# zubair-irshad/HunyuanWorld-Mirror

Hardware: AMD Instinct MI355X
Metric: views/sec (higher is better)
Workload: dtype bf16; 1 GPU; 8-view 518x518 bf16, no priors, camera+depth+pointmap+normal heads, 8 views/GPU, full 1.23B-param arch; views_per_gpu=8, global_views=8, parallelism=view-shard x1, collective=none (1 GPU)

## Files before the change

hunyuanworld-mirror_amd/_lib.py:

```python
from __future__ import annotations

import ctypes as C
import os

import torch

_HERE = os.path.dirname(os.path.abspath(__file__))
LIB_PATH = os.environ.get("WM_HIP_LIB") or os.path.join(_HERE, "libwm_hip.so")

WM_DT = {"bf16": 0, "f16": 1, "fp16": 1, "float16": 1, "bfloat16": 0}
EPI_F32, EPI_T16, EPI_GELU_T16, EPI_RESID = 0, 1, 2, 3


class wm_config(C.Structure):
    _fields_ = [
        ("img_size", C.c_int32), ("patch_size", C.c_int32), ("embed_dim", C.c_int32), ("gs_dim", C.c_int32),
        ("enable_cond", C.c_int32), ("enable_cam", C.c_int32), ("enable_pts", C.c_int32), ("enable_depth", C.c_int32),
        ("enable_norm", C.c_int32), ("enable_gs", C.c_int32),
        ("depth", C.c_int32), ("num_heads", C.c_int32), ("mlp_ratio", C.c_int32), ("num_register_tokens", C.c_int32),
        ("intermediate_idxs", C.c_int32 * 4),
        ("rope_freq", C.c_float),
        ("dino_depth", C.c_int32), ("dino_heads", C.c_int32),
        ("cam_trunk_depth", C.c_int32), ("cam_heads", C.c_int32), ("cam_steps", C.c_int32),
        ("dpt_features", C.c_int32),
        ("dpt_out_channels", C.c_int32 * 4),
        ("backbone_dtype", C.c_int32), ("head_dtype", C.c_int32),
    ]


_FP = C.c_void_p


class wm_outputs(C.Structure):
    _fields_ = [(n, _FP) for n in (
        "camera_params", "camera_poses", "camera_intrs", "depth", "depth_conf", "pts3d", "pts3d_conf",
        "normals", "normals_conf", "gs_depth", "gs_depth_conf", "splat_means", "splat_quats", "splat_scales",
        "splat_opacities", "splat_sh", "splat_weights")] + [("taps", _FP * 4)]


EXPORTS = [
    "wm_create", "wm_destroy", "wm_last_error", "wm_set_weight", "wm_finalize_weights", "wm_host_resample_pos",
    "wm_workspace_bytes", "wm_reserve", "wm_set_workspace", "wm_missing_name", "wm_share_weights", "wm_forward", "wm_forward_sharded", "wm_rccl_unique_id", "wm_comm_init_rccl",
    "wm_local_group_create", "wm_local_group_destroy", "wm_comm_init_local", "wm_allgather", "wm_profile_enable", "wm_profile_read",
    "wm_op_gemm", "wm_op_gemm_resid_ln", "wm_op_gemm_qkv", "wm_op_attention", "wm_op_layernorm", "wm_op_qkv_post", "wm_op_conv", "wm_op_bilinear",
    "wm_op_linear_f32", "wm_host_to_16", "wm_set_tuning", "wm_op_attention_split", "wm_op_attention_ex", "wm_op_attention_flag_count", "wm_op_gs_splat", "wm_op_conv3x3_up", "wm_depth_to_world", "wm_confidence_mask", "wm_confidence_mask_workspace_bytes", "wm_preprocess_image", "wm_preprocess_image_size",
    "wm_preprocess_image_workspace_bytes", "wm_rasterize_splats", "wm_rasterize_workspace_bytes", "wm_prune_gs", "wm_prune_gs_workspace_bytes", "wm_op_up_conv_n32", "wm_op_conv3x3_gemm16", "wm_op_conv_ex", "wm_op_upconv3x3_tap", "wm_op_tconv", "wm_op_upconv_gather",
    "wm_depth_edge", "wm_normals_edge", "wm_point_filter_mask_workspace_bytes", "wm_point_filter_mask",
    "wm_op_im2col", "wm_op_im2col7", "wm_op_dino_tokens", "wm_op_vgt_special", "wm_op_gemm_rowmap", "wm_op_gemm_convt", "wm_op_layernorm_rows",
    "wm_op_bilinear_add", "wm_op_bilinear16", "wm_op_copy2d", "wm_op_small_attention", "wm_op_adaln", "wm_op_cam_update", "wm_op_cam_matrices",
    "wm_op_linear_f32_ex",
]

_lib = None


def lib() -> C.CDLL:
    global _lib
    if _lib is not None:
        return _lib
    if not os.path.exists(LIB_PATH):
        raise RuntimeError(
            f"{LIB_PATH} not found: build it with `python -c 'import __graft_entry__ as g; g.build()'` "
            "(hipcc --offload-arch=gfx950). There is no CPU fallback for the product path.")
    L = C.CDLL(LIB_PATH, mode=C.RTLD_GLOBAL)
    vp, i32, f32 = C.c_void_p, C.c_int, C.c_float
    L.wm_create.argtypes = [C.POINTER(wm_config), i32, C.POINTER(vp)]
    L.wm_destroy.argtypes = [vp]
    L.wm_destroy.restype = None
    L.wm_last_error.argtypes = [vp]
    L.wm_last_error.restype = C.c_char_p
    L.wm_set_weight.argtypes = [vp, C.c_char_p, vp, C.POINTER(C.c_int64), i32]
    L.wm_finalize_weights.argtypes = [vp, C.POINTER(i32)]
    L.wm_host_resample_pos.argtypes = [vp, i32, i32, i32, i32, vp]
    L.wm_host_resample_pos.restype = None
    L.wm_workspace_bytes.argtypes = [vp, i32, i32, i32, i32]
    L.wm_workspace_bytes.restype = C.c_size_t
    L.wm_reserve.argtypes = [vp, i32, i32, i32, i32]
    L.wm_set_workspace.argtypes = [vp, vp, C.c_size_t]
    L.wm_share_weights.argtypes = [vp, vp]
    L.wm_missing_name.argtypes = [vp, i32]
    L.wm_missing_name.restype = C.c_char_p
    L.wm_forward.argtypes = [vp, vp, i32, i32, i32, vp, vp, vp, C.POINTER(C.c_int32), C.POINTER(wm_outputs), vp]
    L.wm_forward_sharded.argtypes = [vp, vp, i32, i32, i32, i32, i32, vp, vp, vp, C.POINTER(C.c_int32),
                                     C.POINTER(wm_outputs), vp]
    L.wm_rccl_unique_id.argtypes = [vp]
    L.wm_comm_init_rccl.argtypes = [vp, vp, i32, i32]
    L.wm_local_group_create.argtypes = [i32]
    L.wm_local_group_create.restype = vp
    L.wm_local_group_destroy.argtypes = [vp]
    L.wm_local_group_destroy.restype = None
    L.wm_comm_init_local.argtypes = [vp, vp, i32]
    L.wm_allgather.argtypes = [vp, vp, vp, C.c_size_t, vp]
    L.wm_profile_enable.argtypes = [vp, i32]
    L.wm_profile_read.argtypes = [vp, i32, C.POINTER(C.c_double), C.POINTER(C.c_int64)]
    L.wm_op_gemm.argtypes = [i32, i32, vp, vp, vp, vp, vp, i32, i32, i32, vp]
    L.wm_op_gemm_resid_ln.argtypes = [i32, vp, vp, vp, vp, vp, vp, vp, f32, vp, vp, vp, i32, i32, i32, C.POINTER(i32), vp]
    L.wm_op_gemm_qkv.argtypes = [i32, vp, vp, vp, vp, vp, vp, vp, vp, vp, vp, vp, vp, i32, i32, i32, i32, i32, i32, f32, vp]
    L.wm_op_attention.argtypes = [i32, vp, vp, vp, vp, i32, i32, i32, i32, i32, vp]
    L.wm_op_attention_split.argtypes = [i32, vp, vp, vp, vp, i32, i32, i32, i32, i32, i32, vp, vp, vp]
    L.wm_op_attention_ex.argtypes = [i32, vp, vp, vp, vp, i32, i32, i32, i32, i32, i32, vp, vp, vp, vp]
    L.wm_op_attention_flag_count.argtypes = [i32, i32, i32]
    L.wm_op_attention_flag_count.restype = C.c_size_t
    L.wm_op_layernorm.argtypes = [vp, vp, vp, vp, i32, i32, f32, i32, i32, vp]
    L.wm_op_qkv_post.argtypes = [i32, vp, vp, vp, vp, vp, vp, vp, vp, vp, vp, i32, i32, i32, i32, i32, f32, vp]
    L.wm_op_conv.argtypes = [i32, vp, vp, vp, vp, vp, vp, i32, i32, i32, i32, i32, i32, i32, i32, i32, i32, vp]
    L.wm_op_bilinear.argtypes = [vp, vp, i32, i32, i32, i32, i32, i32, vp]
    L.wm_op_linear_f32.argtypes = [vp, vp, vp, vp, i32, i32, i32, i32, i32, i32, vp]
    L.wm_host_to_16.argtypes = [vp, vp, C.c_size_t, i32]
    L.wm_host_to_16.restype = None
    L.wm_depth_to_world.argtypes = [vp, vp, vp, vp, vp, vp, i32, i32, i32, f32, vp]
    L.wm_depth_to_world.restype = i32
    L.wm_confidence_mask_workspace_bytes.argtypes = [C.c_size_t]
    L.wm_confidence_mask_workspace_bytes.restype = C.c_size_t
    L.wm_confidence_mask.argtypes = [vp, C.c_size_t, f32, vp, vp, C.c_size_t, vp]
    L.wm_confidence_mask.restype = i32
    L.wm_depth_edge.argtypes = [vp, vp, i32, i32, i32, i32, i32, f32, i32, f32, vp, vp]
    L.wm_depth_edge.restype = i32
    L.wm_normals_edge.argtypes = [vp, vp, i32, i32, i32, i32, C.c_double, vp, vp]
    L.wm_normals_edge.restype = i32
    L.wm_point_filter_mask_workspace_bytes.argtypes = [i32, i32, i32]
    L.wm_point_filter_mask_workspace_bytes.restype = C.c_size_t
    L.wm_point_filter_mask.argtypes = [vp, vp, vp, i32, i32, i32, i32, C.c_double, i32, C.c_double, f32, vp, vp, vp, C.c_size_t, vp]
    L.wm_point_filter_mask.restype = i32
    L.wm_op_up_conv_n32.argtypes = [i32, vp, vp, vp, vp, i32, i32, i32, i32, i32, i32, vp, vp, i32, vp, vp]
    L.wm_op_up_conv_n32.restype = i32
    L.wm_op_conv3x3_gemm16.argtypes = [i32, vp, vp, vp, vp, i32, vp, vp, i32, i32, i32, i32, i32, i32, i32, vp, vp]
    L.wm_op_conv3x3_gemm16.restype = i32
    L.wm_op_conv_ex.argtypes = [i32, vp, i32, vp, vp, vp, vp, vp, i32, i32, i32, i32, i32, i32, i32, i32, i32, vp]
    L.wm_op_conv_ex.restype = i32
    L.wm_op_upconv3x3_tap.argtypes = [i32, vp, vp, vp, vp, i32, i32, i32, i32, i32, i32, i32, vp, vp, vp]
    L.wm_op_upconv3x3_tap.restype = i32
    L.wm_op_tconv.argtypes = [i32, vp, vp, vp, vp, vp, i32, i32, i32, i32, i32, i32, vp, vp]
    L.wm_op_tconv.restype = i32
    L.wm_op_upconv_gather.argtypes = [vp, vp, vp, i32, i32, i32, i32, i32, i32, vp]
    L.wm_op_upconv_gather.restype = i32
    L.wm_prune_gs_workspace_bytes.argtypes = [C.c_size_t]
    L.wm_prune_gs_workspace_bytes.restype = C.c_size_t
    L.wm_prune_gs.argtypes = [vp, vp, vp, vp, vp, vp, i32, f32, vp, vp, vp, vp, vp, C.POINTER(i32), vp, C.c_size_t, vp]
    L.wm_prune_gs.restype = i32
    L.wm_rasterize_workspace_bytes.argtypes = [i32, i32, i32, i32, C.c_size_t]
    L.wm_rasterize_workspace_bytes.restype = C.c_size_t
    L.wm_rasterize_splats.argtypes = [vp, vp, vp, vp, vp, i32, i32, vp, vp, i32, i32, i32, vp, vp, vp, vp, vp, C.c_size_t, C.c_size_t,
                                      C.POINTER(C.c_ulonglong), vp]
    L.wm_rasterize_splats.restype = i32
    L.wm_preprocess_image_size.argtypes = [i32, i32, i32, i32, C.POINTER(i32), C.POINTER(i32)]
    L.wm_preprocess_image_size.restype = i32
    L.wm_preprocess_image_workspace_bytes.argtypes = [i32, i32, i32, i32]
    L.wm_preprocess_image_workspace_bytes.restype = C.c_size_t
    L.wm_preprocess_image.argtypes = [vp, i32, i32, i32, i32, vp, vp, C.c_size_t, vp]
    L.wm_preprocess_image.restype = i32
# ... 41 lines not shown
```

hunyuanworld-mirror_amd/csrc/gemm.hip:

```cpp
#include "wm_common.h"
#include "wm_kernels.h"

#include <cstdlib>
#include <type_traits>

int wm_tuning[WM_TUNE_COUNT] = {-1, -1, -1, -1, -1, -1, -1, -1, -1, -1, -1, -1, -1, -1, -1, -1, -1, -1, -1, -1, -1, -1, -1, -1, -1, -1, -1, -1, -1};

namespace {

#ifndef WM_GEMM_PRIO
#define WM_GEMM_PRIO 0
#endif
constexpr int PRIO = WM_GEMM_PRIO;
constexpr int BK = 64;

typedef __attribute__((address_space(3))) void* lds_vp;
typedef const __attribute__((address_space(1))) void* glb_vp;

__device__ __forceinline__ void stage_piece32(const u16* __restrict__ g, int ld, int row0, int nrows, int k0, char* lds_tile,
                                              int piece, int lane) {
  const int r = piece * 16 + (lane >> 2);
  const int c = (lane & 3) ^ ((r >> 2) & 3);
  int gr = row0 + r;
  gr = gr < nrows ? gr : nrows - 1;
  __builtin_amdgcn_global_load_lds((glb_vp)(g + (size_t)gr * ld + k0 + c * 8), (lds_vp)(lds_tile + piece * 1024), 16, 0, 0);
}
__device__ __forceinline__ s16x8 lds_frag32(const char* tile, int row, int chunk) {
  return *(const s16x8*)(tile + row * 64 + ((chunk ^ ((row >> 2) & 3)) << 4));
}

__device__ __forceinline__ void stage_piece(const u16* __restrict__ g, int ld, int row0, int nrows, int k0, char* lds_tile,
                                            int piece, int lane) {
  const int r = piece * 8 + (lane >> 3);
  const int c = (lane & 7) ^ ((r >> 1) & 7);
  int gr = row0 + r;
  gr = gr < nrows ? gr : nrows - 1;
  __builtin_amdgcn_global_load_lds((glb_vp)(g + (size_t)gr * ld + k0 + c * 8), (lds_vp)(lds_tile + piece * 1024), 16, 0, 0);
}

__device__ __forceinline__ s16x8 lds_frag(const char* tile, int row, int chunk) {
  return *(const s16x8*)(tile + row * 128 + ((chunk ^ ((row >> 1) & 7)) << 4));
}

__device__ __forceinline__ void tile_of(int lid, int ntm, int ntn, int G, int& band, int& nt) {
  if (G <= 1 || ntn <= 4) { band = lid / ntn; nt = lid - band * ntn; return; }
  const int per = G * ntn, sg = lid / per, r = lid - sg * per;
  const int here = ntm - sg * G < G ? ntm - sg * G : G;
  nt = r / here;
  band = sg * G + (r - nt * here);
}

template <int N> __device__ __forceinline__ void wait_vmcnt() { asm volatile("s_waitcnt vmcnt(%0)" ::"n"(N) : "memory"); }

template <int T, int EPI, int WM, int WN, int TM, int TN, int NSTAGE, int ILV, int KT = 64>
__global__ __launch_bounds__(WM * WN * 64) void gemm_nt_kernel(const WmGemmArgs p) {
  constexpr int BK = KT;
  constexpr int NW = WM * WN, BM = WM * TM * 32, BN = WN * TN * 32;
  constexpr int A_BYTES = BM * BK * 2, B_BYTES = BN * BK * 2, STAGE = A_BYTES + B_BYTES;
  constexpr int PA = BM * BK * 2 / 1024, PB = BN * BK * 2 / 1024;
// ... 232 lines not shown
            if (!ok[g]) continue;
            const float4 gm = *(const float4*)(p.gamma + cb + 8 * g);
            const float4 nv = make_float4(old[g].x + gm.x * v[g].x, old[g].y + gm.y * v[g].y, old[g].z + gm.z * v[g].z, old[g].w + gm.w * v[g].w);
            *(float4*)((float*)p.C + orow * p.ldc + cb + 8 * g) = nv;
            if (p.C2) *(float4*)(p.C2 + orow * p.ldc2 + cb + 8 * g) = nv;
          }
        } else if constexpr (EPI == WM_EPI_ROWMAP_ADD) {
#pragma unroll
          for (int g = 0; g < 4; ++g) {
            if (!ok[g]) continue;
            const int col = cb + 8 * g;
            float4 x = v[g];
            if (p.relu) x = make_float4(fmaxf(x.x, 0.f), fmaxf(x.y, 0.f), fmaxf(x.z, 0.f), fmaxf(x.w, 0.f));
            if (p.add) {
              const float4 ad = *(const float4*)(p.add + (size_t)q * p.N + col);
              x.x += ad.x; x.y += ad.y; x.z += ad.z; x.w += ad.w;
            }
            const size_t o = orow * p.ldc + col;
            if (p.out16) {
              uint2 u;
              u.x = (uint32_t)f2t<T>(x.x) | ((uint32_t)f2t<T>(x.y) << 16);
              u.y = (uint32_t)f2t<T>(x.z) | ((uint32_t)f2t<T>(x.w) << 16);
              *(uint2*)((u16*)p.C + o) = u;
            } else {
              float* c = (float*)p.C + o;
              if (p.accumulate) {
                const float4 od = *(const float4*)c;
                x.x += od.x; x.y += od.y; x.z += od.z; x.w += od.w;
              }
              *(float4*)c = x;
            }
          }
        }
      }
    }
  }
}

template <int T, int EPI, int WM, int WN, int TM, int TN, int NSTAGE, int ILV, int KT = 64>
hipError_t launch_cfg(const WmGemmArgs& a, hipStream_t s) {
  constexpr int BM = WM * TM * 32, BN = WN * TN * 32;
  constexpr size_t shm = (size_t)NSTAGE * (BM + BN) * KT * 2;
  const int ntn = (a.N + BN - 1) / BN, ntm = (a.M + BM - 1) / BM;
  static bool attr = false;
  if (!attr) {
    (void)hipFuncSetAttribute((const void*)gemm_nt_kernel<T, EPI, WM, WN, TM, TN, NSTAGE, ILV, KT>, hipFuncAttributeMaxDynamicSharedMemorySize, (int)shm);
    attr = true;
  }
  hipLaunchKernelGGL((gemm_nt_kernel<T, EPI, WM, WN, TM, TN, NSTAGE, ILV, KT>), dim3(ntm * ntn), dim3(WM * WN * 64), shm, s, a);
  return hipGetLastError();
}


template <int T, int EPI, int SM, int SN>
__device__ __forceinline__ void epilogue16(const WmGemmArgs& p, f32x4 (&acc)[SM][SN], int rowb, int colb, int lane, int mlim) {
  const int l15 = lane & 15, lq = lane >> 4;
  if constexpr (EPI == WM_EPI_QKV) {
    static_assert(EPI != WM_EPI_QKV || SN == 4, "QKV epilogue needs 64 columns per wave");
    const WmQkvArgs& q = p.qkv;
    const int D = q.H * 64;
    const int col0 = colb;
    const int which = col0 / D, head = (col0 - which * D) >> 6;
    if (col0 >= p.N) return;
    const float* nw = which == 0 ? q.qn_w : q.kn_w;
    const float* nb = which == 0 ? q.qn_b : q.kn_b;
    const bool do_norm = which < 2 && nw != nullptr, do_rope = which < 2 && q.rope_cos != nullptr;
    u16* dst = (u16*)(which == 0 ? q.q : which == 1 ? q.k : q.v);
    const float sc = which == 0 ? q.q_scale : 1.0f;
    float4 bs4[4], w4[4], b4[4];
#pragma unroll
    for (int j = 0; j < 4; ++j) {
      bs4[j] = p.bias ? *(const float4*)(p.bias + col0 + 16 * j + 4 * lq) : make_float4(0, 0, 0, 0);
      w4[j] = do_norm ? *(const float4*)(nw + 16 * j + 4 * lq) : make_float4(1, 1, 1, 1);
      b4[j] = do_norm ? *(const float4*)(nb + 16 * j + 4 * lq) : make_float4(0, 0, 0, 0);
    }
    auto rope_rows = [&](int i, float4 (&cs)[2], float4 (&sn)[2]) {
      const int row = rowb + i * 16 + l15;
      const int rr = row < mlim ? row : 0;
      const int t = rr - (int)(((float)rr + 0.5f) * q.inv_tpv) * q.tokens_per_view;
      int py = 0, px = 0;
      if (t >= q.patch_start) {
        const int idx = t - q.patch_start;
        py = (int)(((float)idx + 0.5f) * q.inv_gw) + 1;
        px = idx - (py - 1) * q.grid_w + 1;
      }
      cs[0] = *(const float4*)(q.rope_cos + py * 16 + 4 * lq); sn[0] = *(const float4*)(q.rope_sin + py * 16 + 4 * lq);
      cs[1] = *(const float4*)(q.rope_cos + px * 16 + 4 * lq); sn[1] = *(const float4*)(q.rope_sin + px * 16 + 4 * lq);
    };
    float4 csn[2][2], snn[2][2];
    if (do_rope) rope_rows(0, csn[0], snn[0]);
#pragma unroll
    for (int i = 0; i < SM; ++i) {
      if (rowb + i * 16 >= mlim) break;
      const int row = rowb + i * 16 + l15;
      const bool row_ok = row < mlim;
      if (do_rope && i + 1 < SM) rope_rows(i + 1, csn[(i + 1) & 1], snn[(i + 1) & 1]);
      float v[4][4];
#pragma unroll
      for (int j = 0; j < 4; ++j) {
        v[j][0] = acc[i][j][0] + bs4[j].x; v[j][1] = acc[i][j][1] + bs4[j].y; v[j][2] = acc[i][j][2] + bs4[j].z; v[j][3] = acc[i][j][3] + bs4[j].w;
      }
      if (do_norm) {
        float sm = 0.f;
#pragma unroll
        for (int j = 0; j < 4; ++j)
#pragma unroll
          for (int e = 0; e < 4; ++e) sm += v[j][e];
        sm += __shfl_xor(sm, 16);
        const float mean = xhalf_sum(sm) * (1.0f / 64.0f);
        float ss = 0.f;
#pragma unroll
        for (int j = 0; j < 4; ++j)
#pragma unroll
          for (int e = 0; e < 4; ++e) { v[j][e] -= mean; ss += v[j][e] * v[j][e]; }
        ss += __shfl_xor(ss, 16);
        const float rstd = 1.0f / sqrtf(xhalf_sum(ss) * (1.0f / 64.0f) + 1e-5f);
#pragma unroll
        for (int j = 0; j < 4; ++j) {
          v[j][0] = v[j][0] * rstd * w4[j].x + b4[j].x; v[j][1] = v[j][1] * rstd * w4[j].y + b4[j].y;
          v[j][2] = v[j][2] * rstd * w4[j].z + b4[j].z; v[j][3] = v[j][3] * rstd * w4[j].w + b4[j].w;
        }
      }
      if (do_rope) {
#pragma unroll
        for (int hh = 0; hh < 2; ++hh) {
          const float4 cs = csn[i & 1][hh], sn = snn[i & 1][hh];
          const float c4[4] = {cs.x, cs.y, cs.z, cs.w}, s4[4] = {sn.x, sn.y, sn.z, sn.w};
#pragma unroll
          for (int e = 0; e < 4; ++e) {
            const float lo = v[2 * hh][e], hi = v[2 * hh + 1][e];
            v[2 * hh][e] = lo * c4[e] - hi * s4[e];
            v[2 * hh + 1][e] = hi * c4[e] + lo * s4[e];
          }
        }
      }
      uint2 u[4];
#pragma unroll
      for (int j = 0; j < 4; ++j) {
        u[j].x = (uint32_t)f2t<T>(v[j][0] * sc) | ((uint32_t)f2t<T>(v[j][1] * sc) << 16);
        u[j].y = (uint32_t)f2t<T>(v[j][2] * sc) | ((uint32_t)f2t<T>(v[j][3] * sc) << 16);
      }
#pragma unroll
      for (int jp = 0; jp < 2; ++jp) {
        swap16(u[2 * jp].x, u[2 * jp + 1].x);
        swap16(u[2 * jp].y, u[2 * jp + 1].y);
      }
      if (row_ok) {
        u16* o = dst + ((size_t)head * q.head_stride + row) * 64 + 16 * (lq & 1) + 4 * (lq & 2);
#pragma unroll
        for (int jp = 0; jp < 2; ++jp) *(uint4*)(o + 32 * jp) = make_uint4(u[2 * jp].x, u[2 * jp].y, u[2 * jp + 1].x, u[2 * jp + 1].y);
      }
    }
    return;
  } else {
    float4 bs4[SN], gm4[SN];
#pragma unroll
    for (int j = 0; j < SN; ++j) {
      const int col = colb + j * 16 + 4 * lq;
      bs4[j] = (p.bias && col < p.N) ? *(const float4*)(p.bias + col) : make_float4(0, 0, 0, 0);
      if constexpr (EPI == WM_EPI_RESID) gm4[j] = col < p.N ? *(const float4*)(p.gamma + col) : make_float4(0, 0, 0, 0);
    }
    if constexpr ((EPI == WM_EPI_T16 || EPI == WM_EPI_GELU_T16) && SN % 2 == 0) {
      if ((p.N & 7) == 0 && (p.ldc & 7) == 0 && ((uintptr_t)p.C & 15) == 0) {
#pragma unroll
        for (int i = 0; i < SM; ++i) {
          if (rowb + i * 16 >= mlim) break;
          const int row = rowb + i * 16 + l15;
#pragma unroll
          for (int jp = 0; jp < SN / 2; ++jp) {
            uint2 u[2];
#pragma unroll
            for (int h = 0; h < 2; ++h) {
              const int j = 2 * jp + h;
              float4 x = make_float4(acc[i][j][0] + bs4[j].x, acc[i][j][1] + bs4[j].y, acc[i][j][2] + bs4[j].z, acc[i][j][3] + bs4[j].w);
              if constexpr (EPI == WM_EPI_GELU_T16) x = gelu_erf4(x);
              u[h].x = (uint32_t)f2t<T>(x.x) | ((uint32_t)f2t<T>(x.y) << 16);
              u[h].y = (uint32_t)f2t<T>(x.z) | ((uint32_t)f2t<T>(x.w) << 16);
            }
            swap16(u[0].x, u[1].x);
            swap16(u[0].y, u[1].y);
            const int col = colb + (2 * jp + (lq & 1)) * 16 + 4 * (lq & 2);
            if (row < mlim && col < p.N) *(uint4*)((u16*)p.C + (size_t)row * p.ldc + col) = make_uint4(u[0].x, u[0].y, u[1].x, u[1].y);
          }
        }
        return;
      }
    }
    if constexpr (EPI == WM_EPI_RESID) {
      float4 old[2][SN];
      auto load_old = [&](int i, float4 (&o)[SN]) {
        const int row = rowb + i * 16 + l15;
#pragma unroll
        for (int j = 0; j < SN; ++j) {
          const int col = colb + j * 16 + 4 * lq;
          o[j] = (row < mlim && col < p.N) ? *(const float4*)((const float*)p.C + (size_t)row * p.ldc + col) : make_float4(0, 0, 0, 0);
        }
      };
      load_old(0, old[0]);
#pragma unroll
      for (int i = 0; i < SM; ++i) {
        if (rowb + i * 16 >= mlim) break;
        if (i + 1 < SM) load_old(i + 1, old[(i + 1) & 1]);
        const int row = rowb + i * 16 + l15;
#pragma unroll
        for (int j = 0; j < SN; ++j) {
          const int col = colb + j * 16 + 4 * lq;
          const float4 o = old[i & 1][j], gm = gm4[j], bs = bs4[j];
          if (row < mlim && col < p.N) {
            const float4 nv = make_float4(o.x + gm.x * (acc[i][j][0] + bs.x), o.y + gm.y * (acc[i][j][1] + bs.y), o.z + gm.z * (acc[i][j][2] + bs.z), o.w + gm.w * (acc[i][j][3] + bs.w));
            *(float4*)((float*)p.C + (size_t)row * p.ldc + col) = nv;
            if (p.C2) *(float4*)(p.C2 + (size_t)row * p.ldc2 + col) = nv;
          }
        }
      }
      return;
    }
    if constexpr (EPI == WM_EPI_CONV) {
      auto out_row = [&](int row) -> size_t {
        if (p.tc_k <= 0) return (size_t)row;
        const int hw = p.cv_h * p.cv_w, n = row / hw, rem = row - n * hw, ti = rem / p.cv_w, tj = rem - ti * p.cv_w;
        const int ph = colb / 256, a = ph / p.tc_k, b = ph - a * p.tc_k;
        return ((size_t)(n * p.cv_h + ti) * p.tc_k + a) * (size_t)(p.cv_w * p.tc_k) + (size_t)(tj * p.tc_k + b);
      };
      const int cshift = p.tc_k > 0 ? (colb / 256) * 256 : 0;
      float4 rs[2][SN], r2[2][SN];
      auto load_res = [&](int i, float4 (&a)[SN], float4 (&b)[SN]) {
        const int row = rowb + i * 16 + l15;
// ... 8 lines not shown
      load_res(0, rs[0], r2[0]);
#pragma unroll
      for (int i = 0; i < SM; ++i) {
        if (rowb + i * 16 >= mlim) break;
        if (i + 1 < SM) load_res(i + 1, rs[(i + 1) & 1], r2[(i + 1) & 1]);
        const int row = rowb + i * 16 + l15;
        float4 y[SN];
#pragma unroll
        for (int j = 0; j < SN; ++j) {
          float4 a = rs[i & 1][j];
          if (p.cv_resid_relu) a = make_float4(fmaxf(a.x, 0.f), fmaxf(a.y, 0.f), fmaxf(a.z, 0.f), fmaxf(a.w, 0.f));
          const float4 b = r2[i & 1][j], bs = bs4[j];
          y[j] = make_float4(acc[i][j][0] + bs.x + a.x + b.x, acc[i][j][1] + bs.y + a.y + b.y, acc[i][j][2] + bs.z + a.z + b.z, acc[i][j][3] + bs.w + a.w + b.w);
          if (p.relu) y[j] = make_float4(fmaxf(y[j].x, 0.f), fmaxf(y[j].y, 0.f), fmaxf(y[j].z, 0.f), fmaxf(y[j].w, 0.f));
        }
        if (p.out16) {
          if constexpr (SN % 2 == 0) {
#pragma unroll
            for (int jp = 0; jp < SN / 2; ++jp) {
              uint2 u[2];
#pragma unroll
              for (int h = 0; h < 2; ++h) {
                const float4 x = y[2 * jp + h];
                u[h].x = (uint32_t)f2t<T>(x.x) | ((uint32_t)f2t<T>(x.y) << 16);
                u[h].y = (uint32_t)f2t<T>(x.z) | ((uint32_t)f2t<T>(x.w) << 16);
              }
              swap16(u[0].x, u[1].x);
              swap16(u[0].y, u[1].y);
              const int col = colb + (2 * jp + (lq & 1)) * 16 + 4 * (lq & 2);
              if (row < mlim && col < p.N) *(uint4*)((u16*)p.C + out_row(row) * p.ldc + col - cshift) = make_uint4(u[0].x, u[0].y, u[1].x, u[1].y);
            }
          }
        } else {
#pragma unroll
          for (int j = 0; j < SN; ++j) {
            const int col = colb + j * 16 + 4 * lq;
            if (row < mlim && col < p.N) *(float4*)((float*)p.C + out_row(row) * p.ldc + col - cshift) = y[j];
          }
        }
      }
      return;
    }
#pragma unroll
    for (int i = 0; i < SM; ++i) {
      if (rowb + i * 16 >= mlim) break;
      const int row = rowb + i * 16 + l15;
      if (row >= mlim) continue;
#pragma unroll
      for (int j = 0; j < SN; ++j) {
        const int col = colb + j * 16 + 4 * lq;
        if (col >= p.N) continue;
        const float4 bs = bs4[j];
        float4 x = make_float4(acc[i][j][0] + bs.x, acc[i][j][1] + bs.y, acc[i][j][2] + bs.z, acc[i][j][3] + bs.w);
        const size_t o = (size_t)row * p.ldc + col;
        if constexpr (EPI == WM_EPI_F32) {
          *(float4*)((float*)p.C + o) = x;
        } else if constexpr (EPI == WM_EPI_T16 || EPI == WM_EPI_GELU_T16) {
          if constexpr (EPI == WM_EPI_GELU_T16) x = gelu_erf4(x);
          uint2 u;
          u.x = (uint32_t)f2t<T>(x.x) | ((uint32_t)f2t<T>(x.y) << 16);
          u.y = (uint32_t)f2t<T>(x.z) | ((uint32_t)f2t<T>(x.w) << 16);
          *(uint2*)((u16*)p.C + o) = u;
        }
      }
    }
  }
}

template <int T, int EPI, int WM, int WN, int TM, int TN, int NSTAGE>
__global__ __launch_bounds__(WM * WN * 64) void gemm_nt16_kernel(const WmGemmArgs p) {
  constexpr int NW = WM * WN, BM = WM * TM * 32, BN = WN * TN * 32;
  constexpr int SM = TM * 2, SN = TN * 2;
  constexpr int A_BYTES = BM * BK * 2, B_BYTES = BN * BK * 2, STAGE = A_BYTES + B_BYTES;
  constexpr int PA = BM / 8, PB = BN / 8, PPW = (PA + PB) / NW;
  static_assert((PA + PB) % NW == 0, "pieces must divide over waves");
  extern __shared__ __attribute__((aligned(16))) char smem[];
  const int tid = threadIdx.x, lane = tid & 63, wave = __builtin_amdgcn_readfirstlane(tid >> 6);
  const int wm = wave / WN, wn = wave % WN;
  const int ntn = (p.N + BN - 1) / BN, ntm = (p.M + BM - 1) / BM;
  const int lid = xcd_remap(blockIdx.x, ntm * ntn);
  const int m0 = (lid / ntn) * BM, n0 = (lid % ntn) * BN;
  const u16* A = (const u16*)p.A;
  const u16* W = (const u16*)p.W;
  auto stage = [&](int kt, int s) {
    char* base = smem + s * STAGE;
#pragma unroll
    for (int i = 0; i < PPW; ++i) {
      const int pc = wave * PPW + i;
      if (pc < PA) stage_piece(A, p.lda, m0, p.M, kt * BK, base, pc, lane);
      else stage_piece(W, p.ldw, n0, p.N, kt * BK, base + A_BYTES, pc - PA, lane);
    }
  };
  f32x4 acc[SM][SN];
#pragma unroll
  for (int i = 0; i < SM; ++i)
#pragma unroll
    for (int j = 0; j < SN; ++j) acc[i][j] = f32x4{0.f, 0.f, 0.f, 0.f};
  const int nk = p.K / BK;
#pragma unroll
  for (int s = 0; s < NSTAGE - 1; ++s)
    if (s < nk) stage(s, s);
  const int l15 = lane & 15, lq = lane >> 4;
  for (int t = 0; t < nk; ++t) {
    const int ahead = min(nk - 1 - t, NSTAGE - 2);
    if (ahead >= 2) wait_vmcnt<2 * PPW>();
    else if (ahead == 1) wait_vmcnt<PPW>();
// ... 242 lines not shown
      if (__hip_atomic_load((wm_gi32*)(p.ln_sync + band * 2), WM_RLX_AGENT) >= 4) { ok = 1; break; }
      if (++spins > WM_LN_SPIN_LIMIT) break;
      __builtin_amdgcn_s_sleep(1);
    }
    if (!ok) __hip_atomic_store((wm_gi32*)(p.ln_fallback + band), 1, WM_RLX_AGENT);
    *lflag = ok;
  }
  __syncthreads();
  ok = *lflag;
  if (ok) {
    float4 w4[4], b4[4];
#pragma unroll
    for (int j = 0; j < 4; ++j) {
      w4[j] = *(const float4*)(p.ln_w + colb + j * 16 + 4 * lq);
      b4[j] = *(const float4*)(p.ln_b + colb + j * 16 + 4 * lq);
    }
#pragma unroll
    for (int i = 0; i < SM; ++i) {
      if (rowb + i * 16 >= mlim) break;
      const int row = rowb + i * 16 + l15;
      const int rr = row < mlim ? row : mlim - 1;
      float m[4], q[4];
#pragma unroll
      for (int k = 0; k < 4; ++k) {
        const unsigned long long bits = __hip_atomic_load((wm_gu64*)(p.ln_stats + ((size_t)rr * 4 + k) * 2), WM_RLX_AGENT);
        m[k] = __builtin_bit_cast(float, (unsigned)bits); q[k] = __builtin_bit_cast(float, (unsigned)(bits >> 32));
      }
      float mean, M2;
      ln_combine4(m, q, 256.0f, mean, M2);
      const float rstd = 1.0f / sqrtf(__fadd_rn(__fmul_rn(M2, 1.0f / 1024.0f), p.ln_eps));
      uint2 u[4];
#pragma unroll
      for (int j = 0; j < 4; ++j) {
        const float y0 = ln_norm(acc[i][j][0], mean, rstd, w4[j].x, b4[j].x), y1 = ln_norm(acc[i][j][1], mean, rstd, w4[j].y, b4[j].y);
        const float y2 = ln_norm(acc[i][j][2], mean, rstd, w4[j].z, b4[j].z), y3 = ln_norm(acc[i][j][3], mean, rstd, w4[j].w, b4[j].w);
        u[j].x = (uint32_t)f2t<T>(y0) | ((uint32_t)f2t<T>(y1) << 16);
        u[j].y = (uint32_t)f2t<T>(y2) | ((uint32_t)f2t<T>(y3) << 16);
      }
#pragma unroll
      for (int jp = 0; jp < 2; ++jp) {
        swap16(u[2 * jp].x, u[2 * jp + 1].x);
        swap16(u[2 * jp].y, u[2 * jp + 1].y);
        const int col = colb + (2 * jp + (lq & 1)) * 16 + 4 * (lq & 2);
        if (row < mlim) *(uint4*)((u16*)p.ln_out + (size_t)row * p.ln_ld + col) = make_uint4(u[2 * jp].x, u[2 * jp].y, u[2 * jp + 1].x, u[2 * jp + 1].y);
      }
    }
  }
  __syncthreads();
  if (tid == 0) {
    const int d = __hip_atomic_fetch_add((wm_gi32*)(p.ln_sync + band * 2 + 1), 1, WM_RLX_AGENT);
    if (d == 3) {
      __hip_atomic_store((wm_gi32*)(p.ln_sync + band * 2), 0, WM_RLX_AGENT);
      __hip_atomic_store((wm_gi32*)(p.ln_sync + band * 2 + 1), 0, WM_RLX_AGENT);
    }
  }
}

#ifdef WM_GEMM_STAMPS
__device__ int wm_ln_fallback_count;
#endif
template <int T>
__global__ __launch_bounds__(256) void gemm_ln_fallback_kernel(const WmGemmArgs p, int bands, int full_units) {
  const int band = blockIdx.x;
  if (__hip_atomic_load((wm_gi32*)(p.ln_fallback + band), WM_RLX_AGENT) == 0) return;
  int u0, S;
  if (p.sched_bands > 0) {
    u0 = (int)((long long)band * p.sched_units / bands);
    S = (int)((long long)(band + 1) * p.sched_units / bands) - u0;
  } else {
    u0 = band * full_units; S = full_units;
  }
  const int lane = threadIdx.x & 63, wave = threadIdx.x >> 6;
#ifdef WM_GEMM_STAMPS
  if (threadIdx.x == 0) atomicAdd(&wm_ln_fallback_count, 1);
#endif
  const int r1 = (u0 + S) * 16 < p.M ? (u0 + S) * 16 : p.M;
  for (int row = u0 * 16 + wave; row < r1; row += 4) {
    float m[4], q[4];
#pragma unroll
    for (int k = 0; k < 4; ++k) {
      const unsigned long long bits = __hip_atomic_load((wm_gu64*)(p.ln_stats + ((size_t)row * 4 + k) * 2), WM_RLX_AGENT);
      m[k] = __builtin_bit_cast(float, (unsigned)bits); q[k] = __builtin_bit_cast(float, (unsigned)(bits >> 32));
    }
    float mean, M2;
    ln_combine4(m, q, 256.0f, mean, M2);
    const float rstd = 1.0f / sqrtf(__fadd_rn(__fmul_rn(M2, 1.0f / 1024.0f), p.ln_eps));
#pragma unroll
    for (int i = 0; i < 4; ++i) {
      const int c = (i * 64 + lane) * 4;
      const float4 v = *(const float4*)((const float*)p.C + (size_t)row * p.ldc + c);
      const float4 w = *(const float4*)(p.ln_w + c), b = *(const float4*)(p.ln_b + c);
      uint2 u;
      u.x = (uint32_t)f2t<T>(ln_norm(v.x, mean, rstd, w.x, b.x)) | ((uint32_t)f2t<T>(ln_norm(v.y, mean, rstd, w.y, b.y)) << 16);
      u.y = (uint32_t)f2t<T>(ln_norm(v.z, mean, rstd, w.z, b.z)) | ((uint32_t)f2t<T>(ln_norm(v.w, mean, rstd, w.w, b.w)) << 16);
      *(uint2*)((u16*)p.ln_out + (size_t)row * p.ln_ld + c) = u;
    }
  }
  __syncthreads();
  if (threadIdx.x == 0) __hip_atomic_store((wm_gi32*)(p.ln_fallback + band), 0, WM_RLX_AGENT);
}

#ifdef WM_GEMM_STAMPS
__device__ unsigned long long wm_gemm_stamp_buf[8 * 8192];
#endif

template <int T, int EPI, int PRIO, int DBG = 0, int QI = 4, int VER = 2>
// ... 49 lines not shown
    const int lim = (isA ? p.M : p.N) - 1;
    gr = gr < lim ? gr : lim;
    gp[i] = (isA ? (const u16*)p.A + (size_t)gr * p.lda : (const u16*)p.W + (size_t)gr * p.ldw) + c * 8;
    loff[i] = (isA ? 0 : A_BYTES) + pl * 1024;
    if constexpr (CONV) {
      if (isA) {
        const int ai = i < 2 ? i : i - 4;
        const int hw = p.cv_h * p.cv_w, n = gr / hw, rem = gr - n * hw, y = rem / p.cv_w, x = rem - y * p.cv_w;
        cv_pix[ai] = gr;
        cv_fl[ai] = (y == 0 ? 1 : 0) | (y == p.cv_h - 1 ? 2 : 0) | (x == 0 ? 4 : 0) | (x == p.cv_w - 1 ? 8 : 0);
        cv_c8[ai] = c * 8;
      }
    }
  }
  auto dma = [&](int buf, int i0, int i1, bool in_loop = false) {
    if ((DBG == 6 || (DBG >= 16 && (DBG & 1))) && in_loop) return;
#pragma unroll
    for (int i = i0; i < i1; ++i) {
      if ((i == 1 || i == 7) && !two) continue;
      if constexpr (CONV) {
        if (i < 2 || i >= 6) {
          const int ai = i < 2 ? i : i - 4;
          const int tap = cv_tap[ai], cc = cv_cc[ai];
          int dy, dx;
          if (p.tc_k > 0) { const unsigned nb = tc_word >> (4 * tap); dy = (int)(nb & 3) - 1; dx = (int)((nb >> 2) & 3) - 1; }
          else { const int ty = tap / 3; dy = ty - 1; dx = tap - ty * 3 - 1; }
          const int mask = (dy < 0 ? 1 : 0) | (dy > 0 ? 2 : 0) | (dx < 0 ? 4 : 0) | (dx > 0 ? 8 : 0);
          const u16* inside = (const u16*)p.A + ((long long)(cv_pix[ai] + dy * p.cv_w + dx) * p.cv_cin + cc * 64 + cv_c8[ai]);
          const u16* src = (cv_fl[ai] & mask) ? (const u16*)p.cv_zero + cv_c8[ai] : inside;
          __builtin_amdgcn_global_load_lds((glb_vp)src, (lds_vp)(smem + buf * STAGE + loff[i]), 16, 0, 0);
          if (++cv_cc[ai] == cv_nch) { cv_cc[ai] = 0; ++cv_tap[ai]; }
          continue;
        }
      }
      __builtin_amdgcn_global_load_lds((glb_vp)gp[i], (lds_vp)(smem + buf * STAGE + loff[i]), 16, 0, 0);
      gp[i] += 64;
    }
  };
  auto wait2 = [&](auto n2c, auto n1c) {
    if (two) wait_vmcnt<decltype(n2c)::value>(); else wait_vmcnt<decltype(n1c)::value>();
  };
#define WM_W2(a_, b_) wait2(std::integral_constant<int, a_>{}, std::integral_constant<int, b_>{})
  const int sw = (l15 >> 1) & 7;
  const int foff0 = l15 * 128 + ((lq ^ sw) << 4), foff1 = l15 * 128 + (((4 + lq) ^ sw) << 4);
  const int a_base = wr * WROWS * 128, b_base = A_BYTES + wc * 64 * 128;

  f32x4 acc[SM][SN];
#pragma unroll
  for (int i = 0; i < SM; ++i)
#pragma unroll
    for (int j = 0; j < SN; ++j) acc[i][j] = f32x4{0.f, 0.f, 0.f, 0.f};
  s16x8 a[QI][2], b0[2][2], b1[2][2];

  const int nk = CONV && p.tc_k > 0 ? (int)(tc_word >> 16) * cv_nch : p.K / 64;
  dma(0, 0, 8);
  if (nk > 1) dma(1, 0, 8);
  if constexpr (VER == 3) {
    if (nk > 1) WM_W2(10, 7); else WM_W2(2, 1);
  } else {
    if (nk > 1) WM_W2(12, 9); else WM_W2(4, 3);
  }
  __builtin_amdgcn_s_barrier();
  if (VER == 2 && wr == 1) __builtin_amdgcn_s_barrier();

#ifdef WM_GEMM_STAMPS
  const unsigned long long st_loop0 = __builtin_amdgcn_s_memrealtime(), st_cyc0 = __builtin_amdgcn_s_memtime();
#endif
  if constexpr (VER == 3) {
    constexpr int NAY = QI == 4 ? 2 : 1;
    constexpr int CY = 2 * NAY + 4, C0Y = NAY + 2;
    auto lgk0 = [&]() { asm volatile("s_waitcnt lgkmcnt(0)" ::: "memory"); };
    auto bar = [&]() { __builtin_amdgcn_s_barrier(); __builtin_amdgcn_sched_barrier(0); };
    auto mfma_on = [&]() { __builtin_amdgcn_sched_barrier(0); if (PRIO) __builtin_amdgcn_s_setprio(1); };
    auto mfma_off = [&]() { if (PRIO) __builtin_amdgcn_s_setprio(0); __builtin_amdgcn_sched_barrier(0); };
    auto kloop3 = [&](auto nbc) __attribute__((always_inline)) {
      constexpr int NB = decltype(nbc)::value;
      auto rd_a = [&](int t, int q0, int n) {
        const char* tile = smem + (t & 1) * STAGE;
#pragma unroll
        for (int i = 0; i < n; ++i) {
          a[i][0] = *(const s16x8*)(tile + a_base + (q0 + i) * 2048 + foff0);
          a[i][1] = *(const s16x8*)(tile + a_base + (q0 + i) * 2048 + foff1);
        }
      };
      auto rd_b = [&](int t, int j0, s16x8 (&b)[2][2]) {
        const char* tile = smem + (t & 1) * STAGE;
#pragma unroll
        for (int j = 0; j < 2; ++j) {
          b[j][0] = *(const s16x8*)(tile + b_base + (j0 + j) * 2048 + foff0);
          b[j][1] = *(const s16x8*)(tile + b_base + (j0 + j) * 2048 + foff1);
        }
      };
      auto L0 = [&](int t) {
        rd_b(t, 0, b0); rd_a(t, 0, QI);
        if (t >= 1 && t + 1 < nk) dma((t + 1) & 1, 6, 8, true);
      };
      auto L1 = [&](int t) { rd_b(t, 2, b1); };
      auto L2 = [&](int t) {
        rd_a(t, QI, NB);
        if (t + 2 < nk) dma(t & 1, 0, 4, true);
      };
      auto L3 = [&](int t) {
        if (t + 2 < nk) dma(t & 1, 4, 6, true);
      };
      auto mm = [&](int r0, int n, int c0, s16x8 (&b)[2][2]) {
#pragma unroll
        for (int kh = 0; kh < 2; ++kh)
#pragma unroll
          for (int i = 0; i < n; ++i)
#pragma unroll
            for (int j = 0; j < 2; ++j) acc[r0 + i][c0 + j] = mfma16<T>(b[j][kh], a[i][kh], acc[r0 + i][c0 + j]);
      };
      auto M0 = [&](int) { mfma_on(); mm(0, QI, 0, b0); mfma_off(); };
      auto M1 = [&](int) { mfma_on(); mm(0, QI, 2, b1); mfma_off(); };
      auto M2 = [&](int) { mfma_on(); mm(QI, NB, 2, b1); mfma_off(); };
// ... 104 lines not shown
    else if (do_pf) wait_vmcnt<PF>(); else wait_vmcnt<0>();
    stage_end();
#pragma unroll
    for (int kh = 0; kh < 2; ++kh)
#pragma unroll
      for (int i = 0; i < QI; ++i)
#pragma unroll
        for (int j = 0; j < 2; ++j) acc[i][2 + j] = mfma16<T>(b1[j][kh], a[i][kh], acc[i][2 + j]);
    mfma_end();
    if (!NO_RD) {
#pragma unroll
    for (int i = 0; i < NB; ++i) {
      a[i][0] = *(const s16x8*)(tile + a_base + (QI + i) * 2048 + foff0);
      a[i][1] = *(const s16x8*)(tile + a_base + (QI + i) * 2048 + foff1);
    }
    }
    if (n2) dma(buf, 4, 6, true);
    stage_end();
#pragma unroll
    for (int kh = 0; kh < 2; ++kh)
#pragma unroll
      for (int i = 0; i < NB; ++i)
#pragma unroll
        for (int j = 0; j < 2; ++j) acc[QI + i][2 + j] = mfma16<T>(b1[j][kh], a[i][kh], acc[QI + i][2 + j]);
    mfma_end();
    if (n2) { dma(buf, 6, 8, true); WM_W2(12, 9); } else if (n1) { if (do_pf) WM_W2(4 + PF, 3 + PF); else WM_W2(4, 3); }
    stage_end();
#pragma unroll
    for (int kh = 0; kh < 2; ++kh)
#pragma unroll
      for (int i = 0; i < NB; ++i)
#pragma unroll
        for (int j = 0; j < 2; ++j) acc[QI + i][j] = mfma16<T>(b0[j][kh], a[i][kh], acc[QI + i][j]);
    mfma_end();
  }
  };
  if (nB == QI) kloop(std::integral_constant<int, QI>{});
  else if (nB == QI - 1) kloop(std::integral_constant<int, QI - 1>{});
  else kloop(std::integral_constant<int, QI - 2>{});
  }
#undef WM_W2
#ifdef WM_GEMM_STAMPS
  const unsigned long long st_loop1 = __builtin_amdgcn_s_memrealtime(), st_cyc1 = __builtin_amdgcn_s_memtime();
#endif
  if (VER == 2 && wr == 0) __builtin_amdgcn_s_barrier();
  if (DBG == 5 && acc[0][0][0] != 1.2345e-30f) return;
  {
    const int rowb = m0 + (wr ? 16 * S0 : 0), rend = rowb + 16 * Sw;
    if constexpr (EPI == WM_EPI_RESID && DBG == 0 && QI == 3) {
      if (p.ln_out) {
        epilogue_resid_ln<T, SM>(p, acc, smem, tid, lane, wr, wc, band, nt, rowb, n0 + wc * 64, wr ? 16 * S0 : 0, rend < p.M ? rend : p.M);
        return;
      }
    }
    epilogue16<T, EPI, SM, SN>(p, acc, rowb, n0 + wc * 64, lane, rend < p.M ? rend : p.M);
  }
#ifdef WM_GEMM_STAMPS
  asm volatile("s_waitcnt vmcnt(0)" ::: "memory");
  if (wave == 0 && blockIdx.x < 8192) {
    const unsigned long long st_exit = __builtin_amdgcn_s_memrealtime();
    const unsigned hw = __builtin_amdgcn_s_getreg((31 << 11) | 4), xcc = __builtin_amdgcn_s_getreg((31 << 11) | 20);
    if (lane == 0) {
      unsigned long long* o = wm_gemm_stamp_buf + (size_t)blockIdx.x * 8;
      o[0] = st_entry; o[1] = st_loop0; o[2] = st_loop1; o[3] = st_exit; o[4] = st_cyc1 - st_cyc0;
      o[5] = ((unsigned long long)xcc << 32) | hw; o[6] = ((unsigned long long)m0 << 32) | (unsigned)n0; o[7] = 1;
    }
  }
#endif
}

template <int T, int EPI, int DBG = 0, int QI = 4, int VER = 2>
hipError_t launch_pp2(const WmGemmArgs& a, hipStream_t s) {
  constexpr int BM = 64 * QI;
  constexpr size_t shm = (size_t)2 * (BM + 256) * 128 + (EPI == WM_EPI_RESID ? 2048 : 0);
  const int ntn = (a.N + 255) / 256, ntm = a.sched_bands > 0 ? a.sched_bands : (a.M + BM - 1) / BM;
  static bool attr = false;
  if (!attr) {
    (void)hipFuncSetAttribute((const void*)gemm_pp2_kernel<T, EPI, 1, DBG, QI, VER>, hipFuncAttributeMaxDynamicSharedMemorySize, (int)shm);
    attr = true;
  }
  hipLaunchKernelGGL((gemm_pp2_kernel<T, EPI, 1, DBG, QI, VER>), dim3(ntm * ntn), dim3(512), shm, s, a);
  return hipGetLastError();
}

template <int T, int EPI, int QI, int DBG = 0>
hipError_t launch_pp(const WmGemmArgs& a, hipStream_t s) {
  constexpr int BM = 64 * QI, BN = 256;
  constexpr size_t shm = (size_t)2 * (BM + BN) * 128;
  const int ntn = (a.N + BN - 1) / BN, ntm = (a.M + BM - 1) / BM;
  static bool attr = false;
  if (!attr) {
    (void)hipFuncSetAttribute((const void*)gemm_pp_kernel<T, EPI, QI, 1, DBG>, hipFuncAttributeMaxDynamicSharedMemorySize, (int)shm);
    attr = true;
  }
  hipLaunchKernelGGL((gemm_pp_kernel<T, EPI, QI, 1, DBG>), dim3(ntm * ntn), dim3(512), shm, s, a);
  return hipGetLastError();
}

template <int T, int EPI>
hipError_t launch_pp_E(const WmGemmArgs& a, int cfg, hipStream_t s) {
  const int ver = EPI == WM_EPI_CONV ? 2 : wm_tuning[WM_TUNE_GEMM_PP];
  if constexpr (EPI == WM_EPI_CONV) {
    return cfg == 4 ? launch_pp2<T, EPI>(a, s) : launch_pp2<T, EPI, 0, 3>(a, s);
  } else {
    if (ver == 4) return cfg == 4 ? launch_pp2<T, EPI, 0, 4, 3>(a, s) : launch_pp2<T, EPI, 0, 3, 3>(a, s);
    if (ver != 3) return cfg == 4 ? launch_pp2<T, EPI>(a, s) : launch_pp2<T, EPI, 0, 3>(a, s);
    return cfg == 5 ? launch_pp<T, EPI, 3>(a, s) : launch_pp<T, EPI, 4>(a, s);
  }
// ... 90 lines not shown
  return best;
}

void pick_sched(const WmGemmArgs& a, int ncu, int forced_cfg, int& cfg, int& bands) {
  const int U = (a.M + 15) / 16, ntn = (a.N + 255) / 256;
  const float kf = (float)a.K / 1024.0f;
  float best = 1e30f;
  int best_cfg = cfg, best_b = 0;
  for (int c = 4; c <= 5; ++c) {
    if (forced_cfg >= 0 && c != forced_cfg) continue;
    const int full = c == 4 ? 16 : 12;
    const float unit = c == 4 ? 1.43f : 1.5f;
    const int bmin = (U + full - 1) / full;
    for (int k = 0; k < 6; ++k) {
      int B;
      if (k == 0) B = bmin;
      else {
        const long r0 = ((long)bmin * ntn + ncu - 1) / ncu;
        B = (int)(((r0 + k - 1) * ncu) / ntn);
      }
      if (B < bmin) continue;
      if (B > U) B = U;
      const int smax = (U + B - 1) / B;
      if (U / B < full - 4) continue;
      const long rounds = ((long)B * ntn + ncu - 1) / ncu;
      const float loop = kf * (full * unit - 0.5f * (float)(full - smax));
      const float cost = (float)rounds * (1.6f + loop + 0.35f * (float)smax);
      if (cost < best) { best = cost; best_cfg = c; best_b = B; }
    }
  }
  cfg = best_cfg;
  bands = best_b;
}

}

static int wm_ncu() {
  static const int ncu = [] { hipDeviceProp_t pr; int d = 0; (void)hipGetDevice(&d); return hipGetDeviceProperties(&pr, d) == hipSuccess ? pr.multiProcessorCount : 256; }();
  return ncu;
}
static void plan_gemm(const WmGemmArgs& a, int& cfg, int& sched_b, bool& pp2_out);

bool wm_gemm_fuses_ln(const WmGemmArgs& a) {
  if (!a.ln_out || a.epi != WM_EPI_RESID || a.N != 1024 || !a.ln_w || !a.ln_b || !a.ln_stats || !a.ln_sync || !a.ln_fallback || !a.gamma) return false;
  if (wm_tuning[WM_TUNE_LN_FUSE] != 1 || (a.ln_ld & 7) || (a.ldc & 3)) return false;
  int cfg, sched_b; bool pp2;
  plan_gemm(a, cfg, sched_b, pp2);
  if (!pp2 || cfg != 5) return false;
  const int bm = cfg == 4 ? 256 : 192;
  const long bands = sched_b > 0 ? sched_b : (a.M + bm - 1) / bm;
  return bands * 4 <= wm_ncu();
}

hipError_t wm_launch_gemm_ln_fallback(const WmGemmArgs& a, hipStream_t s) {
  if (!wm_gemm_fuses_ln(a)) return hipSuccess;
  int cfg, sched_b; bool pp2;
  plan_gemm(a, cfg, sched_b, pp2);
  const int bm = cfg == 4 ? 256 : 192;
  const int bands = sched_b > 0 ? sched_b : (a.M + bm - 1) / bm;
  WmGemmArgs b = a;
  b.sched_bands = sched_b; b.sched_units = (a.M + 15) / 16;
  if (a.dtype == WM_T_BF16) hipLaunchKernelGGL((gemm_ln_fallback_kernel<WM_T_BF16>), dim3(bands), dim3(256), 0, s, b, bands, bm / 16);
  else hipLaunchKernelGGL((gemm_ln_fallback_kernel<WM_T_F16>), dim3(bands), dim3(256), 0, s, b, bands, bm / 16);
  return hipGetLastError();
}

static void plan_gemm(const WmGemmArgs& a, int& cfg, int& sched_b, bool& pp2_out) {
  cfg = pick_cfg(a);
  sched_b = 0;
  {
    const int ncu = wm_ncu();
    const int pp = wm_tuning[WM_TUNE_GEMM_PP];
    const bool pp2 = (cfg == 4 || cfg == 5) && (pp < 0 || pp == 1 || pp == 2 || pp == 4 || a.epi == WM_EPI_CONV) && (a.epi == WM_EPI_F32 || a.epi == WM_EPI_T16 || a.epi == WM_EPI_GELU_T16 || a.epi == WM_EPI_RESID || a.epi == WM_EPI_QKV || a.epi == WM_EPI_CONV);
    const int ts = wm_tuning[WM_TUNE_GEMM_SCHED];
    if (pp2 && ts != 0) {
      const long legacy_tiles = (long)((a.M + (cfg == 4 ? 255 : 191)) / (cfg == 4 ? 256 : 192)) * ((a.N + 255) / 256);
      if (ts > 0) sched_b = ts;
      else if (legacy_tiles <= 3L * ncu && a.M <= 16384) pick_sched(a, ncu, wm_tuning[WM_TUNE_GEMM_CFG], cfg, sched_b);
      const int U = (a.M + 15) / 16, full = cfg == 4 ? 16 : 12;
      if (sched_b > U) sched_b = U;
      if (sched_b <= 0 || (U + sched_b - 1) / sched_b > full || U / sched_b < full - 4) sched_b = 0;
    }
    pp2_out = pp2 && wm_tuning[WM_TUNE_GEMM_PP] != 0;
    static const int pp_env = [] { const char* e = wm_env("WM_GEMM_PP"); return e ? atoi(e) : 1; }();
    if (wm_tuning[WM_TUNE_GEMM_PP] < 0 && !pp_env) pp2_out = false;
    if (a.epi == WM_EPI_CONV) pp2_out = true;
  }
}

hipError_t wm_launch_gemm(const WmGemmArgs& a, hipStream_t s) {
  if (a.M <= 0 || a.N <= 0) return hipSuccess;
  if (a.K <= 0 || a.K % 64 != 0 || a.N % 4 != 0) return hipErrorInvalidValue;
  if ((a.lda & 7) || (a.ldw & 7)) return hipErrorInvalidValue;
  if (a.epi == WM_EPI_CONVT && (a.ct_cout & 3)) return hipErrorInvalidValue;
  if (a.epi != WM_EPI_CONVT && a.epi != WM_EPI_QKV && (a.ldc & 3)) return hipErrorInvalidValue;
  if (a.epi == WM_EPI_QKV && (a.N % 64 || a.N != 3 * a.qkv.H * 64)) return hipErrorInvalidValue;
  if (a.epi == WM_EPI_CONV && a.tc_k <= 0 && (a.cv_h <= 0 || a.cv_w <= 0 || a.cv_cin % 64 || a.K != 9 * a.cv_cin || a.M % (a.cv_h * a.cv_w) || !a.cv_zero || (a.N & 7))) return hipErrorInvalidValue;
  if (a.epi == WM_EPI_CONV && a.tc_k > 0 && (a.cv_h <= 0 || a.cv_w <= 0 || a.cv_cin % 64 || a.K != 4 * a.cv_cin || a.M % (a.cv_h * a.cv_w) || !a.cv_zero || a.tc_k > 4 ||
                                             a.N != a.tc_k * a.tc_k * 256 || a.ldc != 256 || a.cv_resid || a.cv_resid2))
    return hipErrorInvalidValue;
  int cfg, sched_b;
  bool is_pp2;
  plan_gemm(a, cfg, sched_b, is_pp2);
  const bool fuse_ln = wm_gemm_fuses_ln(a);
  const int gb = wm_tuning[WM_TUNE_GEMM_GROUP] >= 0 ? wm_tuning[WM_TUNE_GEMM_GROUP] : 6;
  if (a.epi == WM_EPI_QKV) {
    if (a.qkv.tokens_per_view <= 0 || a.qkv.grid_w <= 0 || a.M >= (1 << 20) || a.qkv.tokens_per_view >= (1 << 16)) return hipErrorInvalidValue;
    WmGemmArgs b = a;
    b.group_bands = gb;
    b.sched_bands = sched_b; b.sched_units = (a.M + 15) / 16;
    b.qkv.inv_tpv = 1.0f / (float)a.qkv.tokens_per_view;
    b.qkv.inv_gw = 1.0f / (float)a.qkv.grid_w;
    return b.dtype == WM_T_BF16 ? launch_T<WM_T_BF16>(b, cfg, s) : launch_T<WM_T_F16>(b, cfg, s);
  }
  WmGemmArgs c = a;
  c.group_bands = gb;
  c.sched_bands = sched_b; c.sched_units = (a.M + 15) / 16;
  c.pf_c = a.epi == WM_EPI_RESID && wm_tuning[WM_TUNE_RESID_PREFETCH] == 1 ? 1 : 0;
  if (!fuse_ln) c.ln_out = nullptr;
  return c.dtype == WM_T_BF16 ? launch_T<WM_T_BF16>(c, cfg, s) : launch_T<WM_T_F16>(c, cfg, s);
}

#ifdef WM_GEMM_STAMPS
extern "C" int wm_debug_gemm_stamps(unsigned long long* host_out, int nblocks) {
  if (nblocks > 8192) nblocks = 8192;
  return hipMemcpyFromSymbol(host_out, HIP_SYMBOL(wm_gemm_stamp_buf), (size_t)nblocks * 8 * sizeof(unsigned long long)) == hipSuccess ? 0 : 1;
}
extern "C" int wm_debug_ln_fallback_count() {
  int v = -1, z = 0;
  if (hipMemcpyFromSymbol(&v, HIP_SYMBOL(wm_ln_fallback_count), 4) != hipSuccess) return -1;
  (void)hipMemcpyToSymbol(HIP_SYMBOL(wm_ln_fallback_count), &z, 4);
  return v;
}
extern "C" int wm_debug_gemm_stamps_clear() {
  void* d = nullptr;
  if (hipGetSymbolAddress(&d, HIP_SYMBOL(wm_gemm_stamp_buf)) != hipSuccess) return 1;
  return hipMemset(d, 0, sizeof(unsigned long long) * 8 * 8192) == hipSuccess ? 0 : 1;
}
#endif
```

hunyuanworld-mirror_amd/csrc/wm_kernels.h:

```cpp
#pragma once
#include <hip/hip_runtime.h>
#include <stdint.h>
#include <stddef.h>

#include <cstdlib>
inline const char* wm_env(const char* name) {
#ifdef WM_DIAG_ENV
  return getenv(name);
#else
  (void)name;
  return nullptr;
#endif
}


enum {
  WM_EPI_F32 = 0,
  WM_EPI_T16 = 1,
  WM_EPI_GELU_T16 = 2,
  WM_EPI_RESID = 3,
  WM_EPI_ROWMAP_ADD = 4,
  WM_EPI_CONVT = 5,
  WM_EPI_QKV = 6,
  WM_EPI_CONV = 7,
};

struct WmQkvArgs {
  const float* qkv; void* q; void* k; void* v;
  const float* qn_w; const float* qn_b; const float* kn_w; const float* kn_b;
  const float* rope_cos; const float* rope_sin;
  int M, H, head_stride;
  int tokens_per_view, patch_start, grid_w;
  float inv_tpv, inv_gw;
  float q_scale; int dtype;
};

struct WmGemmArgs {
  const void* A; const void* W; void* C;
  const float* bias; const float* gamma; const float* add;
  float* C2; int ldc2;
  int M, N, K, lda, ldw, ldc;
  int dtype, epi;
  int group_bands;
  int pf_c;
  int sched_bands, sched_units;
  int rows_per_group, out_group, out_off, accumulate, out16, relu;
  int ct_k, ct_cout, ct_gh, ct_gw;
  WmQkvArgs qkv;
  int cv_h, cv_w, cv_cin;
  const void* cv_zero;
  const float* cv_resid; const float* cv_resid2;
  int cv_resid_relu;
  int tc_k;
  unsigned tc_list[16];
  void* ln_out; int ln_ld;
  const float* ln_w; const float* ln_b; float ln_eps;
  float* ln_stats;
  int* ln_sync;
  int* ln_fallback;
};
hipError_t wm_launch_gemm(const WmGemmArgs& a, hipStream_t s);
bool wm_gemm_fuses_ln(const WmGemmArgs& a);
hipError_t wm_launch_gemm_ln_fallback(const WmGemmArgs& a, hipStream_t s);

#define WM_ATTN_MAX_SPLITS_C 8
struct WmAttnArgs {
  const void* Q; const void* K; const void* V;
  void* O;
  int H;
  int q_rows;
  int seq_len;
  int q_head_stride;
  int kv_head_stride;
  int kv_chunks;
  long long kv_chunk_stride;
  int kv_rows_per_chunk;
  int dtype;
  int kv_splits, max_splits;
  int full_units;
  float* part_o; float* part_ml;
  int* unit_flags;
  const int* only_if;
  int* unit_hint;
  int* unit_stat;
  int force_partial, part_slot0;
};
hipError_t wm_launch_attention_combine(const WmAttnArgs& a, int slots, hipStream_t s);
hipError_t wm_launch_attention(const WmAttnArgs& a, hipStream_t s);
int wm_attention_variant(const WmAttnArgs& a);
void wm_attention_geometry(const WmAttnArgs& a, int* unit_rows, int* blocks_per_cu);
hipError_t wm_launch_attention_v3(const WmAttnArgs& a, int grid, int* flags, int minw, hipStream_t s);
hipError_t wm_launch_attention_v4(const WmAttnArgs& a, int grid, int* flags, hipStream_t s);
inline size_t wm_attention_max_blocks(int q_rows, int seq_len, int H) {
  const size_t nseq = (size_t)(q_rows / (seq_len > 0 ? seq_len : 1));
  return ((size_t)(seq_len + 127) / 128 + 1) * nseq * (size_t)H * WM_ATTN_MAX_SPLITS_C;
}
constexpr int WM_ATTN_MAX_SPLITS = 8;
constexpr int WM_ATTN_HINT_TTL = 15;

struct WmLnArgs {
  const float* x; void* y; const float* w; const float* b;
  int D, ld_in, ld_out; float eps;
  int groups, rows_per_group, in_group, in_off, out_group, out_off;
  int out_f32, dtype;
};
hipError_t wm_launch_layernorm(const WmLnArgs& a, hipStream_t s);

hipError_t wm_launch_qkv_post(const WmQkvArgs& a, hipStream_t s);

hipError_t wm_launch_im2col(const float* img, void* out, int N, int C, int H, int W, int ps, int Kpad,
                            int normalize, int dtype, hipStream_t s);
hipError_t wm_launch_im2col7(const float* img, void* out, int N, int H, int W, int Kpad, int dtype, hipStream_t s);
hipError_t wm_launch_gs_splat(const float* gp, const float* img, const float* depth, const float* cam, float* means, float* quats,
                              float* scales, float* opac, float* sh, float* wts, int N, int H, int W, hipStream_t s);
// ... 35 lines not shown
  const float* resid2;
  float* y;
  int N, Hi, Wi, Cin, Ho, Wo, Cout, ksize, stride, pad;
  int relu_in, resid_relu, relu_out, dtype;
  int up_hs, up_ws;
  const float* up_addx; const float* up_addy;
  int out16;
  int in16;
  int dbg;
};
bool wm_conv3x3_applicable(const WmConvArgs& a);
bool wm_conv_force_generic();
bool wm_conv3x3_out16_ok(const WmConvArgs& a);
struct WmConvN32Args {
  const uint16_t* x; const uint16_t* w; const float* bias; float* y; const uint16_t* zero;
  int N, H, W, Cin, relu_out, dtype;
  const float* tail_w; const float* tail_b; float* tail_attr; float* tail_conf; int tail_C, tail_act;
};
hipError_t wm_launch_conv3x3_n32_in16(const WmConvN32Args& a, hipStream_t s);
hipError_t wm_launch_bilinear16(const float* in, void* out16, int N, int Hi, int Wi, int Ho, int Wo, int C, const float* addx,
                                const float* addy, int dtype, hipStream_t s);
hipError_t wm_launch_conv(const WmConvArgs& a, hipStream_t s);
hipError_t wm_launch_f32_to_16_2d(const float* src, int ld_src, void* dst16, int ld_dst, int rows, int cols, int dtype, hipStream_t s);
hipError_t wm_launch_tconv_border(float* out, const float* bmiss, int N, int H, int W, int F, hipStream_t s);
hipError_t wm_launch_repack_tap_major(const void* w16, void* wt16, int Co, int C, hipStream_t s);
hipError_t wm_launch_upconv_gather(const void* y16, const float* bias, float* out, int N, int Hi, int Wi, int Ho, int Wo, int Co, hipStream_t s);

hipError_t wm_launch_linear_f32(const float* X, const float* W, const float* b, float* Y, int M, int N, int K,
                                int ldx, int ldy, int pre_act, int post_act, const float* gamma, int accumulate,
                                hipStream_t s);
hipError_t wm_launch_small_attention(const float* qkv, float* out, int S, int heads, int hd, hipStream_t s);
hipError_t wm_launch_adaln(const float* tok, const float* mod, float* h, int S, int D, float eps, hipStream_t s);
hipError_t wm_launch_cam_update(float* pred, const float* delta, float* out, int S, int first, hipStream_t s);
hipError_t wm_launch_cam_matrices(const float* params, float* poses, float* intrs, int S, int H, int W, hipStream_t s);

struct WmRasterArgs {
  const float* means; const float* quats; const float* scales; const float* opacities;
  const float* colors; int is_sh;
  int N;
  const float* viewmats; const float* Ks; int C;
  int width, height;
  float* out_rgb; float* out_depth; float* out_alpha;
  int* radii_out;
  void* workspace; size_t workspace_bytes; size_t max_isects;
};
size_t wm_raster_workspace_bytes(int N, int C, int width, int height, size_t max_isects);
hipError_t wm_launch_rasterize(const WmRasterArgs& a, hipStream_t s, unsigned long long* n_isects_out);

size_t wm_prune_workspace_bytes(size_t N);
hipError_t wm_launch_prune_gs(const float* means, const float* quats, const float* scales, const float* opac, const float* sh,
                              const float* weights, int N, float voxel, float* o_means, float* o_quats, float* o_scales, float* o_opac,
                              float* o_sh, int* K_out, void* workspace, size_t ws_bytes, hipStream_t s);

enum { WM_TUNE_GEMM_CFG = 0, WM_TUNE_GEMM_PP, WM_TUNE_GEMM_MFMA16, WM_TUNE_ATTN_QB, WM_TUNE_OP_LDPAD, WM_TUNE_ATTN_SPLITS, WM_TUNE_CONV_FUSE_UP, WM_TUNE_CONV_NARROW, WM_TUNE_CONV_BN, WM_TUNE_CONV_RS, WM_TUNE_LIN_MFMA, WM_TUNE_CONV_TPX, WM_TUNE_ATTN_TAIL, WM_TUNE_GEMM_GROUP, WM_TUNE_COMM_OVERLAP, WM_TUNE_HEADS_CONC, WM_TUNE_RCU_MID16, WM_TUNE_GEMM_SCHED, WM_TUNE_FORCE_GATHER, WM_TUNE_ATTN_OP_POLICY, WM_TUNE_COMM_P2P, WM_TUNE_LN_RPW, WM_TUNE_LN_FUSE, WM_TUNE_HEADS_MAIN, WM_TUNE_CONV_GEMM, WM_TUNE_RESID_PREFETCH, WM_TUNE_UP1_GATHER, WM_TUNE_TCONV, WM_TUNE_UP1_COMP, WM_TUNE_COUNT };
extern int wm_tuning[WM_TUNE_COUNT];
```

hunyuanworld-mirror_amd/csrc/wm_model.cpp:

```cpp
#include <hip/hip_runtime.h>
#include <rccl/rccl.h>
#include <pthread.h>

#include <algorithm>
#include <cmath>
#include <cstdio>
#include <cstdlib>
#include <cstring>
#include <map>
#include <string>
#include <unordered_map>
#include <vector>

#include "../../include/wm_hip.h"
#include "wm_kernels.h"

namespace {

inline int ru(int x, int m) { return (x + m - 1) / m * m; }

inline uint16_t h_f2bf(float f) {
  uint32_t u;
  memcpy(&u, &f, 4);
  if ((u & 0x7fffffffu) > 0x7f800000u) return (uint16_t)((u >> 16) | 0x40);
  return (uint16_t)((u + 0x7fffu + ((u >> 16) & 1u)) >> 16);
}
inline uint16_t h_f2h(float f) {
  _Float16 h = (_Float16)f;
  uint16_t r;
  memcpy(&r, &h, 2);
  return r;
}
inline uint16_t h_to16(float f, int dt) { return dt == WM_DT_BF16 ? h_f2bf(f) : h_f2h(f); }

struct Weight {
  std::vector<int64_t> shape;
  float* f32 = nullptr;
  void* w16 = nullptr;
  int k16 = 0;
  bool tap_major = false;
  std::vector<float> host;
  bool set = false;
  bool owned = true;
};

struct TconvPack {
  void* w16 = nullptr;
  float* bias_rep = nullptr;
  float* bmiss = nullptr;
  unsigned list[16] = {0};
  int k = 0, cin = 0;
};
static void free_tconv(TconvPack& t) {
  if (t.w16) (void)hipFree(t.w16);
  if (t.bias_rep) (void)hipFree(t.bias_rep);
  if (t.bmiss) (void)hipFree(t.bmiss);
  t = TconvPack();
}

static hipError_t build_tconv(int dt, int k, int Cin, int Cm, int F_, const float* wct, const float* bct, const float* wrn, TconvPack& out, hipStream_t s);
struct Up1Comp {
  void* w16 = nullptr;
  float* bias = nullptr;
  int co = 0;
};
static void free_up1comp(Up1Comp& u) {
  if (u.w16) (void)hipFree(u.w16);
  if (u.bias) (void)hipFree(u.bias);
  u = Up1Comp();
}
static hipError_t build_up1comp(int dt, int F_, int Co, const float* woc1, const float* wout, const float* bout, Up1Comp& out, hipStream_t s);

struct EvPair { hipEvent_t a, b; };

struct Comm {
  int kind = 0;
  int rank = 0, world = 1;
  ncclComm_t nccl = nullptr;
  wm_local_group* grp = nullptr;
};

}

struct wm_local_group {
  int world;
  pthread_barrier_t bar;
  std::vector<void*> recv;
};

struct wm_handle {
  wm_config cfg;
  int device = 0;
  std::string err;
  std::unordered_map<std::string, Weight> w;
  std::map<std::string, std::vector<int64_t>> spec;
  bool finalized = false;
  Comm comm;
  char* arena = nullptr;
  size_t arena_bytes = 0;
  bool arena_owned = true;
  int plan_n = -1, plan_nt = -1, plan_H = -1, plan_W = -1;
  std::map<std::string, TconvPack> tconv;
  bool tconv_valid = false;
  std::map<std::string, Up1Comp> up1comp;
  std::vector<std::string> missing;
  std::map<std::string, void*> buf;
  hipStream_t hstream[4] = {nullptr, nullptr, nullptr, nullptr};
  hipEvent_t hfork = nullptr, hjoin[4] = {nullptr, nullptr, nullptr, nullptr};
  hipStream_t cstream = nullptr;
  hipEvent_t cfork = nullptr, cjoin = nullptr;
  hipStream_t camstream = nullptr;
  hipEvent_t camjoin = nullptr;
  int* att_stat_host = nullptr;
  int att_stat_n = 0;
  std::vector<int> att_seen, att_general_ttl;
  bool prof = false;
  static constexpr int NKIND = 13;
  std::vector<EvPair> ev[NKIND];
  size_t ev_used[NKIND] = {};
};

namespace {

wm_status fail(wm_handle* h, wm_status st, const std::string& msg) {
  if (h) h->err = msg;
  return st;
}
#define HIPCHK(h, e)                                                                                   \
  do {                                                                                                 \
    hipError_t _e = (e);                                                                               \
    if (_e != hipSuccess)                                                                              \
      return fail(h, WM_ERR_HIP, std::string(hipGetErrorString(_e)) + " at " + __FILE__ + ":" + std::to_string(__LINE__)); \
  } while (0)

bool ends_with(const std::string& s, const char* suf) {
  const size_t n = strlen(suf);
  return s.size() >= n && s.compare(s.size() - n, n, suf) == 0;
}
bool starts_with(const std::string& s, const char* p) { return s.compare(0, strlen(p), p) == 0; }

enum WKind { WK_F32, WK_LIN16_BACKBONE, WK_LIN16_HEAD, WK_CONV16_HEAD, WK_CONVT16_HEAD };

WKind classify(const std::string& n, int ndim) {
  const bool vgt = starts_with(n, "visual_geometry_transformer.");
  if (vgt && ndim >= 2) {
    if (ends_with(n, "attn.qkv.weight") || ends_with(n, "attn.proj.weight") || ends_with(n, "mlp.fc1.weight") ||
        ends_with(n, "mlp.fc2.weight") || ends_with(n, "patch_embed.proj.weight") || ends_with(n, "depth_embed.proj.2.fc1.weight") ||
        ends_with(n, "depth_embed.proj.2.fc2.weight"))
      return WK_LIN16_BACKBONE;
    return WK_F32;
  }
  const bool head = starts_with(n, "pts_head.") || starts_with(n, "depth_head.") || starts_with(n, "norm_head.") || starts_with(n, "gs_head.");
  if (head && ndim == 4 && ends_with(n, ".weight")) {
    if (ends_with(n, "scratch.output_conv2.2.weight")) return WK_F32;
    if (n.find("input_merger") != std::string::npos) return WK_LIN16_HEAD;
    if (n.find("resize_layers.0.") != std::string::npos || n.find("resize_layers.1.") != std::string::npos) return WK_CONVT16_HEAD;
// ... 237 lines not shown
  if (x < 1.0) return ((a + 2.0) * x - (a + 3.0)) * x * x + 1.0;
  if (x < 2.0) return (((x - 5.0) * x + 8.0) * x - 4.0) * a;
  return 0.0;
}
void aa_weights(int in, int out, std::vector<int>& xmin, std::vector<int>& xsize, std::vector<float>& wts, int& maxk) {
  const double scale = (double)in / out;
  const double support = scale >= 1.0 ? 2.0 * scale : 2.0;
  const double invscale = scale >= 1.0 ? 1.0 / scale : 1.0;
  maxk = (int)std::ceil(support) * 2 + 1;
  xmin.resize(out); xsize.resize(out); wts.assign((size_t)out * maxk, 0.f);
  for (int i = 0; i < out; ++i) {
    const double center = scale * (i + 0.5);
    const int lo = std::max(0, (int)(center - support + 0.5));
    const int hi = std::min(in, (int)(center + support + 0.5));
    xmin[i] = lo; xsize[i] = hi - lo;
    double tot = 0;
    std::vector<double> w(hi - lo);
    for (int j = 0; j < hi - lo; ++j) { w[j] = cubic_aa((j + lo - center + 0.5) * invscale); tot += w[j]; }
    for (int j = 0; j < hi - lo; ++j) wts[(size_t)i * maxk + j] = (float)(w[j] / tot);
  }
}

}

extern "C" void wm_host_resample_pos(const float* in, int gs, int D, int gh, int gw, float* out) {
  std::vector<int> xm, xs, ym, ys;
  std::vector<float> xw, yw;
  int kx, ky;
  aa_weights(gs, gw, xm, xs, xw, kx);
  aa_weights(gs, gh, ym, ys, yw, ky);
  std::vector<float> tmp((size_t)gs * gw * D);
  for (int y = 0; y < gs; ++y)
    for (int x = 0; x < gw; ++x) {
      float* o = &tmp[((size_t)y * gw + x) * D];
      for (int c = 0; c < D; ++c) o[c] = 0.f;
      for (int j = 0; j < xs[x]; ++j) {
        const float w = xw[(size_t)x * kx + j];
        const float* s = in + ((size_t)y * gs + xm[x] + j) * D;
        for (int c = 0; c < D; ++c) o[c] += w * s[c];
      }
    }
  for (int y = 0; y < gh; ++y)
    for (int x = 0; x < gw; ++x) {
      float* o = out + ((size_t)y * gw + x) * D;
      for (int c = 0; c < D; ++c) o[c] = 0.f;
      for (int j = 0; j < ys[y]; ++j) {
        const float w = yw[(size_t)y * ky + j];
        const float* s = &tmp[((size_t)(ym[y] + j) * gw + x) * D];
        for (int c = 0; c < D; ++c) o[c] += w * s[c];
      }
    }
}

extern "C" int wm_set_tuning(const char* key, int value) {
  static const char* keys[WM_TUNE_COUNT] = {"gemm_cfg", "gemm_pp", "gemm_mfma16", "attn_qb", "op_ldpad", "attn_splits", "conv_fuse_up", "conv_narrow", "conv_bn", "conv_rs", "lin_mfma", "conv_tpx", "attn_tail", "gemm_group", "comm_overlap", "heads_concurrent", "rcu_mid16", "gemm_sched", "force_gather", "attn_op_policy", "comm_p2p", "ln_rpw", "ln_fuse", "heads_main", "conv_gemm", "resid_prefetch", "up1_gather", "tconv", "up1_comp"};
  for (int i = 0; i < WM_TUNE_COUNT; ++i)
    if (key && strcmp(key, keys[i]) == 0) { wm_tuning[i] = value; return 0; }
  return -1;
}

extern "C" void wm_host_to_16(const float* in, uint16_t* out, size_t n, int dtype) {
  for (size_t i = 0; i < n; ++i) out[i] = h_to16(in[i], dtype);
}

extern "C" wm_status wm_create(const wm_config* cfg, int device, wm_handle** out) {
  if (!cfg || !out) return WM_ERR_INVALID;
  wm_handle* h = new wm_handle();
  h->cfg = *cfg;
  h->device = device;
  *out = h;
  if (cfg->embed_dim / cfg->num_heads != 64 || cfg->embed_dim / cfg->dino_heads != 64)
    return fail(h, WM_ERR_INVALID, "backbone head_dim must be 64 (reference: 1024/16)");
  if (cfg->embed_dim % 64) return fail(h, WM_ERR_INVALID, "embed_dim must be a multiple of 64");
  if (hipSetDevice(device) != hipSuccess) return fail(h, WM_ERR_HIP, "hipSetDevice failed");
  return WM_OK;
}

extern "C" void wm_destroy(wm_handle* h) {
  if (!h) return;
  (void)hipSetDevice(h->device);
  for (auto& kv : h->tconv) free_tconv(kv.second);
  for (auto& kv : h->up1comp) free_up1comp(kv.second);
  for (auto& kv : h->w) {
    if (!kv.second.owned) continue;
    if (kv.second.f32) (void)hipFree(kv.second.f32);
    if (kv.second.w16) (void)hipFree(kv.second.w16);
  }
  if (h->arena && h->arena_owned) (void)hipFree(h->arena);
  for (int i = 0; i < 4; ++i) {
    if (h->hstream[i]) (void)hipStreamDestroy(h->hstream[i]);
    if (h->hjoin[i]) (void)hipEventDestroy(h->hjoin[i]);
  }
  if (h->att_stat_host) (void)hipHostFree(h->att_stat_host);
  if (h->hfork) (void)hipEventDestroy(h->hfork);
  if (h->camstream) (void)hipStreamDestroy(h->camstream);
  if (h->camjoin) (void)hipEventDestroy(h->camjoin);
  if (h->cstream) (void)hipStreamDestroy(h->cstream);
  if (h->cfork) (void)hipEventDestroy(h->cfork);
  if (h->cjoin) (void)hipEventDestroy(h->cjoin);
  for (int k = 0; k < wm_handle::NKIND; ++k)
    for (auto& e : h->ev[k]) { (void)hipEventDestroy(e.a); (void)hipEventDestroy(e.b); }
  if (h->comm.kind == 1 && h->comm.nccl) ncclCommDestroy(h->comm.nccl);
  delete h;
}

extern "C" const char* wm_last_error(const wm_handle* h) { return h ? h->err.c_str() : "null handle"; }

extern "C" wm_status wm_set_weight(wm_handle* h, const char* name, const float* host, const int64_t* shape, int ndim) {
  if (!h || !name || !host || !shape) return WM_ERR_INVALID;
  HIPCHK(h, hipSetDevice(h->device));
  const std::string n(name);
  auto& spec = h->spec;
  if (spec.empty())
    for (auto& kv : param_spec(h->cfg)) spec[kv.first] = kv.second;
  auto it = spec.find(n);
  if (it == spec.end()) return WM_OK;
  std::vector<int64_t> sh(shape, shape + ndim);
  if (sh != it->second) return fail(h, WM_ERR_INVALID, "shape mismatch for " + n);
  size_t numel = 1;
  for (auto s : sh) numel *= (size_t)s;
  Weight& w = h->w[n];
  h->plan_n = -1;
  h->tconv_valid = false;
  if (w.owned) {
    if (w.f32) (void)hipFree(w.f32);
    if (w.w16) (void)hipFree(w.w16);
  }
  w.f32 = nullptr; w.w16 = nullptr; w.owned = true; w.tap_major = false;
  w.shape = sh;
  w.set = true;
  const WKind k = classify(n, ndim);
  if (k == WK_F32) {
    HIPCHK(h, hipMalloc((void**)&w.f32, std::max<size_t>(numel, 4) * 4));
    HIPCHK(h, hipMemcpy(w.f32, host, numel * 4, hipMemcpyHostToDevice));
    if (ends_with(n, "pos_embed") || ends_with(n, "init_token")) w.host.assign(host, host + numel);
    if (n.find(".resize_layers.0.bias") != std::string::npos || n.find(".resize_layers.1.bias") != std::string::npos ||
        ends_with(n, ".scratch.refinenet1.out_conv.bias"))
      w.host.assign(host, host + numel);
    return WM_OK;
  }
  if (n.find(".resize_layers.0.weight") != std::string::npos || n.find(".resize_layers.1.weight") != std::string::npos ||
      ends_with(n, ".scratch.layer1_rn.weight") || ends_with(n, ".scratch.layer2_rn.weight") ||
      ends_with(n, ".scratch.refinenet1.out_conv.weight") || ends_with(n, ".scratch.output_conv1.weight"))
    w.host.assign(host, host + numel);
  const int dt = k == WK_LIN16_BACKBONE ? h->cfg.backbone_dtype : h->cfg.head_dtype;
  std::vector<uint16_t> r;
  if (k == WK_LIN16_BACKBONE || k == WK_LIN16_HEAD) {
    const int N = (int)sh[0];
    const int K = (int)(numel / N);
    const int Kp = ru(K, 64);
    r.assign((size_t)N * Kp, 0);
    for (int i = 0; i < N; ++i)
      for (int j = 0; j < K; ++j) r[(size_t)i * Kp + j] = h_to16(host[(size_t)i * K + j], dt);
    w.k16 = Kp;
  } else if (k == WK_CONV16_HEAD) {
    const int Co = (int)sh[0], Ci = (int)sh[1], kh = (int)sh[2], kw = (int)sh[3];
    r.resize(numel);
    for (int o = 0; o < Co; ++o)
      for (int c = 0; c < Ci; ++c)
        for (int y = 0; y < kh; ++y)
          for (int x = 0; x < kw; ++x)
            r[(((size_t)o * kh + y) * kw + x) * Ci + c] = h_to16(host[(((size_t)o * Ci + c) * kh + y) * kw + x], dt);
    w.k16 = kh * kw * Ci;
    if (kh == 3 && kw == 3 && ends_with(n, "output_conv1.weight")) {
      r.resize(2 * numel);
      for (int o = 0; o < Co; ++o)
        for (int t = 0; t < 9; ++t)
          for (int c = 0; c < Ci; ++c) r[numel + ((size_t)t * Co + o) * Ci + c] = r[((size_t)o * 9 + t) * Ci + c];
      w.tap_major = true;
    }
  } else {
    const int Ci = (int)sh[0], Co = (int)sh[1], kk = (int)sh[2];
    r.resize(numel);
    for (int c = 0; c < Ci; ++c)
      for (int o = 0; o < Co; ++o)
        for (int i = 0; i < kk; ++i)
          for (int j = 0; j < kk; ++j)
            r[((size_t)(i * kk + j) * Co + o) * Ci + c] = h_to16(host[(((size_t)c * Co + o) * kk + i) * kk + j], dt);
    w.k16 = Ci;
  }
  HIPCHK(h, hipMalloc(&w.w16, r.size() * 2));
  HIPCHK(h, hipMemcpy(w.w16, r.data(), r.size() * 2, hipMemcpyHostToDevice));
  return WM_OK;
}

static float init_value_of(const std::string& n) {
  const bool norm = n.find(".norm1.") != std::string::npos || n.find(".norm2.") != std::string::npos || n.find(".norm.") != std::string::npos ||
                    n.find("q_norm.") != std::string::npos || n.find("k_norm.") != std::string::npos || n.find("token_norm.") != std::string::npos ||
                    n.find("out_norm.") != std::string::npos;
  if (norm) return ends_with(n, ".weight") ? 1.0f : 0.0f;
  if (ends_with(n, ".gamma")) return n.find(".patch_embed.") != std::string::npos ? 1.0f : 0.01f;
  return 0.0f;
}

extern "C" wm_status wm_finalize_weights(wm_handle* h, int* missing) {
  if (!h) return WM_ERR_INVALID;
  HIPCHK(h, hipSetDevice(h->device));
  h->missing.clear();
  for (auto& kv : param_spec(h->cfg)) {
    auto it = h->w.find(kv.first);
    if (it != h->w.end() && it->second.set) continue;
    h->missing.push_back(kv.first);
    size_t numel = 1;
    for (auto s : kv.second) numel *= (size_t)s;
    std::vector<float> z(numel, init_value_of(kv.first));
    wm_status st = wm_set_weight(h, kv.first.c_str(), z.data(), kv.second.data(), (int)kv.second.size());
    if (st != WM_OK) return st;
    h->w[kv.first].set = false;
  }
  if (missing) *missing = (int)h->missing.size();
  h->finalized = true;
  return WM_OK;
}

extern "C" wm_status wm_share_weights(wm_handle* dst, const wm_handle* src) {
  if (!dst || !src || dst == src) return WM_ERR_INVALID;
  if (!src->finalized) return fail(dst, WM_ERR_STATE, "source weights not finalized");
  if (memcmp(&dst->cfg, &src->cfg, sizeof(wm_config)) != 0 || dst->device != src->device)
    return fail(dst, WM_ERR_INVALID, "wm_share_weights: configuration or device differs");
  for (auto& kv : dst->w) {
    if (!kv.second.owned) continue;
    if (kv.second.f32) (void)hipFree(kv.second.f32);
    if (kv.second.w16) (void)hipFree(kv.second.w16);
  }
  dst->w = src->w;
  for (auto& kv : dst->w) kv.second.owned = false;
  dst->spec = src->spec;
  dst->missing = src->missing;
  dst->finalized = true;
  dst->plan_n = -1;
  dst->tconv_valid = false;
  return WM_OK;
}

extern "C" const char* wm_missing_name(const wm_handle* h, int i) {
  return (h && i >= 0 && (size_t)i < h->missing.size()) ? h->missing[i].c_str() : nullptr;
}

extern "C" size_t wm_workspace_bytes(const wm_handle* h, int n_local, int n_total, int H, int W) {
  if (!h) return 0;
  const Dims d = make_dims(h, n_local, n_total, H, W);
  size_t tot = 0;
  for (auto& kv : arena_layout(h, d)) tot += kv.second;
  return tot;
}

namespace {

wm_status plan(wm_handle* h, const Dims& d) {
  if (h->plan_n == d.n && h->plan_nt == d.nt && h->plan_H == d.H && h->plan_W == d.W) return WM_OK;
  const wm_config& c = h->cfg;
  auto L = arena_layout(h, d);
  size_t tot = 0;
  for (auto& kv : L) tot += kv.second;
  HIPCHK(h, hipDeviceSynchronize());
  if (tot > h->arena_bytes) {
    if (!h->arena_owned)
      return fail(h, WM_ERR_STATE, "caller workspace too small: " + std::to_string(h->arena_bytes) + " < " + std::to_string(tot) + " bytes (wm_workspace_bytes)");
    if (h->arena) HIPCHK(h, hipFree(h->arena));
    h->arena = nullptr;
    h->arena_bytes = 0;
    HIPCHK(h, hipMalloc((void**)&h->arena, tot));
    h->arena_bytes = tot;
  }
  h->buf.clear();
  size_t off = 0;
  for (auto& kv : L) { h->buf[kv.first] = h->arena + off; off += kv.second; }

  {
    const int np = std::max(d.gh, d.gw) + 1;
    std::vector<float> cs((size_t)np * 16), sn((size_t)np * 16);
    for (int p = 0; p < np; ++p)
      for (int i = 0; i < 16; ++i) {
        const float expo = (float)(2 * i) / 32.0f;
        const float inv = 1.0f / std::pow(c.rope_freq, expo);
        const float ang = (float)p * inv;
        cs[(size_t)p * 16 + i] = std::cos(ang);
        sn[(size_t)p * 16 + i] = std::sin(ang);
      }
    HIPCHK(h, hipMemcpy(h->buf["rope_cos"], cs.data(), cs.size() * 4, hipMemcpyHostToDevice));
    HIPCHK(h, hipMemcpy(h->buf["rope_sin"], sn.data(), sn.size() * 4, hipMemcpyHostToDevice));
  }
  {
    const int n = (c.dino_depth + 2 * c.depth) * 3;
    if (h->att_stat_n != n) {
      if (h->att_stat_host) HIPCHK(h, hipHostFree(h->att_stat_host));
      h->att_stat_host = nullptr;
      HIPCHK(h, hipHostMalloc((void**)&h->att_stat_host, (size_t)n * 4, hipHostMallocDefault));
      h->att_stat_n = n;
    }
    memset(h->att_stat_host, 0, (size_t)n * 4);
    h->att_seen.assign(n, 0);
    h->att_general_ttl.assign(n, 0);
    HIPCHK(h, hipMemset(h->buf["ATT_STAT"], 0, (size_t)n * 4));
  }
  HIPCHK(h, hipMemset(h->buf["LN_SYNC"], 0, ((size_t)d.Mx / 16 + 2) * 3 * 4));
  HIPCHK(h, hipMemset(h->buf["ATT_HINT"], 0, (size_t)(c.dino_depth + 2 * c.depth) * 3 * wm_attention_max_blocks((int)d.Mx, d.P < d.Td ? d.P : d.Td, d.heads) * 4));
  {
    const Weight* pe = W(h, "visual_geometry_transformer.patch_embed.pos_embed");
    if (!pe || pe->host.empty()) return fail(h, WM_ERR_STATE, "pos_embed not set");
    const int g = c.img_size / c.patch_size, D = d.D;
    if (d.gh == g && d.gw == g) {
      HIPCHK(h, hipMemcpy(h->buf["dino_pos"], pe->host.data(), (size_t)(1 + d.hw) * D * 4, hipMemcpyHostToDevice));
    } else {
      std::vector<float> r((size_t)(1 + d.hw) * D);
      memcpy(r.data(), pe->host.data(), (size_t)D * 4);
      wm_host_resample_pos(pe->host.data() + D, g, D, d.gh, d.gw, r.data() + D);
      HIPCHK(h, hipMemcpy(h->buf["dino_pos"], r.data(), r.size() * 4, hipMemcpyHostToDevice));
    }
  }
  {
    const double aspect = (double)d.W / (double)d.H;
    std::vector<float> tx, ty;
    for (int i = 0; i < 4; ++i) {
      const int C = c.dpt_out_channels[i];
      uv_tables(d.gw, d.gh, C, aspect, tx, ty);
      std::vector<float> full((size_t)d.hw * C);
      for (int y = 0; y < d.gh; ++y)
        for (int x = 0; x < d.gw; ++x)
          for (int k = 0; k < C; ++k)
            full[((size_t)y * d.gw + x) * C + k] = k < C / 2 ? tx[(size_t)x * (C / 2) + k] : ty[(size_t)y * (C / 2) + k - C / 2];
      HIPCHK(h, hipMemcpy(h->buf["dpt_pos" + std::to_string(i)], full.data(), full.size() * 4, hipMemcpyHostToDevice));
    }
    uv_tables(d.W, d.H, c.dpt_features / 2, aspect, tx, ty);
    HIPCHK(h, hipMemcpy(h->buf["dpt_posx"], tx.data(), tx.size() * 4, hipMemcpyHostToDevice));
    HIPCHK(h, hipMemcpy(h->buf["dpt_posy"], ty.data(), ty.size() * 4, hipMemcpyHostToDevice));
    if (c.enable_gs) {
      uv_tables(d.W, d.H, c.gs_dim / 2, aspect, tx, ty);
      HIPCHK(h, hipMemcpy(h->buf["gs_posx"], tx.data(), tx.size() * 4, hipMemcpyHostToDevice));
      HIPCHK(h, hipMemcpy(h->buf["gs_posy"], ty.data(), ty.size() * 4, hipMemcpyHostToDevice));
    }
  }
  if (!h->tconv_valid) {
    for (auto& kv : h->tconv) free_tconv(kv.second);
  for (auto& kv : h->up1comp) free_up1comp(kv.second);
    h->tconv.clear();
    std::vector<std::string> heads;
    if (c.enable_pts) heads.push_back("pts_head.");
    if (c.enable_depth) heads.push_back("depth_head.");
    if (c.enable_norm) heads.push_back("norm_head.");
    if (c.dpt_features == 256)
      for (const std::string& p : heads)
        for (int i = 0; i < 2; ++i) {
          const Weight* wct = W(h, p + "resize_layers." + std::to_string(i) + ".weight");
          const Weight* bct = W(h, p + "resize_layers." + std::to_string(i) + ".bias");
          const Weight* wrn = W(h, p + "scratch.layer" + std::to_string(i + 1) + "_rn.weight");
          const int k = i == 0 ? 4 : 2, oc = c.dpt_out_channels[i];
          if (!wct || !bct || !wrn || wct->host.empty() || bct->host.empty() || wrn->host.empty() || oc % 64) continue;
          if (wct->host.size() != (size_t)oc * oc * k * k || bct->host.size() != (size_t)oc || wrn->host.size() != (size_t)256 * oc * 9) continue;
          HIPCHK(h, build_tconv(c.head_dtype, k, oc, oc, 256, wct->host.data(), bct->host.data(), wrn->host.data(), h->tconv[p + std::to_string(i)], nullptr));
        }
    h->up1comp.clear();
    if (c.head_dtype == WM_DT_F16)
      for (const std::string& p : heads) {
        const Weight* w1 = W(h, p + "scratch.output_conv1.weight");
        const Weight* wo = W(h, p + "scratch.refinenet1.out_conv.weight");
        const Weight* bo = W(h, p + "scratch.refinenet1.out_conv.bias");
        const int F_ = c.dpt_features;
        if (!w1 || !wo || !bo || w1->host.empty() || wo->host.empty() || bo->host.empty() || F_ % 64 || w1->shape.size() != 4) continue;
        const int Co = (int)w1->shape[0];
        if ((Co != 128 && Co != 64 && Co != 32) || w1->host.size() != (size_t)Co * F_ * 9 || wo->host.size() != (size_t)F_ * F_ || bo->host.size() != (size_t)F_) continue;
        HIPCHK(h, build_up1comp(c.head_dtype, F_, Co, w1->host.data(), wo->host.data(), bo->host.data(), h->up1comp[p], nullptr));
      }
    h->tconv_valid = true;
  }
  if (c.enable_cam) {
    const Weight* it = W(h, "cam_head.init_token");
    std::vector<float> v((size_t)d.nt * 12, 0.f);
    if (it && !it->host.empty())
      for (int i = 0; i < d.nt; ++i)
        for (int k = 0; k < 9; ++k) v[(size_t)i * 12 + k] = it->host[k];
    HIPCHK(h, hipMemcpy(h->buf["cam_init"], v.data(), v.size() * 4, hipMemcpyHostToDevice));
  }
  h->plan_n = d.n; h->plan_nt = d.nt; h->plan_H = d.H; h->plan_W = d.W;
  return WM_OK;
}

struct ProfScope {
  wm_handle* h; int kind; hipStream_t s; EvPair* e = nullptr;
  ProfScope(wm_handle* h_, int k, hipStream_t s_) : h(h_), kind(k), s(s_) {
    if (!h->prof) return;
    auto& v = h->ev[kind];
    if (h->ev_used[kind] == v.size()) {
      EvPair p;
// ... 15 lines not shown
      for (int r = 0; r < cm.world; ++r) {
        if (r == cm.rank) continue;
        if (ncclSend(send, bytes, ncclInt8, r, cm.nccl, s) != ncclSuccess) return fail(h, WM_ERR_COMM, "ncclSend failed");
        if (ncclRecv((char*)recv + (size_t)r * bytes, bytes, ncclInt8, r, cm.nccl, s) != ncclSuccess) return fail(h, WM_ERR_COMM, "ncclRecv failed");
      }
      if (ncclGroupEnd() != ncclSuccess) return fail(h, WM_ERR_COMM, "ncclGroupEnd failed");
      HIPCHK(h, hipMemcpyAsync((char*)recv + (size_t)cm.rank * bytes, send, bytes, hipMemcpyDeviceToDevice, s));
      return WM_OK;
    }
    if (ncclAllGather(send, recv, bytes, ncclInt8, cm.nccl, s) != ncclSuccess) return fail(h, WM_ERR_COMM, "ncclAllGather failed");
    return WM_OK;
  }
  if (cm.kind == 2) {
    wm_local_group* g = cm.grp;
    g->recv[cm.rank] = recv;
    HIPCHK(h, hipStreamSynchronize(s));
    pthread_barrier_wait(&g->bar);
    for (int r = 0; r < g->world; ++r)
      HIPCHK(h, hipMemcpyAsync((char*)g->recv[r] + (size_t)cm.rank * bytes, send, bytes, hipMemcpyDeviceToDevice, s));
    HIPCHK(h, hipStreamSynchronize(s));
    pthread_barrier_wait(&g->bar);
    return WM_OK;
  }
  return fail(h, WM_ERR_COMM, "sharded forward without a communicator");
}

struct Ctx {
  wm_handle* h; Dims d; hipStream_t s; int bdt, hdt;
  int attn_site = 0;
};

#define LCHK(c, e)                                                                                            \
  do {                                                                                                        \
    hipError_t _e = (e);                                                                                      \
    if (_e != hipSuccess)                                                                                     \
      return fail((c).h, WM_ERR_HIP, std::string(hipGetErrorString(_e)) + " at " + __FILE__ + ":" + std::to_string(__LINE__)); \
  } while (0)

wm_status gemm(Ctx& c, int dt, int epi, const void* A, int lda, const void* Wp, int ldw, void* C, int ldc, const float* bias,
               const float* gamma, int M, int N, int K, WmGemmArgs* extra = nullptr, int prof_kind = -1, bool* ln_fused = nullptr) {
  WmGemmArgs a;
  if (extra) a = *extra; else memset(&a, 0, sizeof(a));
  a.A = A; a.W = Wp; a.C = C; a.bias = bias; a.gamma = gamma;
  a.M = M; a.N = N; a.K = K; a.lda = lda; a.ldw = ldw; a.ldc = ldc; a.dtype = dt; a.epi = epi;
  ProfScope ps(c.h, prof_kind >= 0 ? prof_kind : epi == WM_EPI_QKV ? 5 : epi == WM_EPI_RESID ? 6 : epi == WM_EPI_GELU_T16 ? 7 : 2, c.s);
  const bool fuse = a.ln_out != nullptr && wm_gemm_fuses_ln(a);
  if (!fuse) a.ln_out = nullptr;
  if (ln_fused) *ln_fused = fuse;
  LCHK(c, wm_launch_gemm(a, c.s));
  if (fuse) LCHK(c, wm_launch_gemm_ln_fallback(a, c.s));
  return WM_OK;
}

wm_status layernorm(Ctx& c, const float* x, int ld_in, void* y, int ld_out, const float* w, const float* b, int D, float eps,
                    int groups, int rpg, int in_group, int in_off, int out_group, int out_off, int out_f32, int dt) {
  WmLnArgs a;
  a.x = x; a.y = y; a.w = w; a.b = b; a.D = D; a.ld_in = ld_in; a.ld_out = ld_out; a.eps = eps;
  a.groups = groups; a.rows_per_group = rpg; a.in_group = in_group; a.in_off = in_off; a.out_group = out_group; a.out_off = out_off;
  a.out_f32 = out_f32; a.dtype = dt;
  LCHK(c, wm_launch_layernorm(a, c.s));
  return WM_OK;
}

wm_status backbone_block(Ctx& c, const std::string& p, float* X, int M, int seq_len, int heads, float eps, bool qk_norm,
                         bool rope, int tokens_per_view, int patch_start, bool is_global, float* tap_half = nullptr,
                         bool ln1_done = false, const std::string& next_norm1 = std::string(), bool* ln1_ready = nullptr) {
  wm_handle* h = c.h;
  const Dims& d = c.d;
  const int D = d.D, dt = c.bdt;
  uint16_t* A16 = B<uint16_t>(h, "A16");
  char* QKV16 = B<char>(h, "QKV16");
  const size_t hsz = (size_t)M * D * 2;
  void* Q16 = QKV16; void* K16 = QKV16 + hsz; void* V16 = QKV16 + 2 * hsz;
  void* O16 = B<void>(h, "O16");
  void* H16 = B<void>(h, "H16");
  wm_status st;
  if (ln1_ready) *ln1_ready = false;
  if (!ln1_done) {
    st = layernorm(c, X, D, A16, D, F(h, p + "norm1.weight"), F(h, p + "norm1.bias"), D, eps, 1, M, 0, 0, 0, 0, 0, dt);
    if (st) return st;
  }
  auto fuse_args = [&](WmGemmArgs& ex, const float* w, const float* b) {
    ex.ln_out = A16; ex.ln_ld = D; ex.ln_w = w; ex.ln_b = b; ex.ln_eps = eps;
    ex.ln_stats = B<float>(h, "LN_STATS");
    int* sync = B<int>(h, "LN_SYNC");
    ex.ln_sync = sync; ex.ln_fallback = sync + ((size_t)d.Mx / 16 + 2) * 2;
  };
  {
    WmGemmArgs ex;
    memset(&ex, 0, sizeof(ex));
    WmQkvArgs& a = ex.qkv;
    a.q = Q16; a.k = K16; a.v = V16;
    if (qk_norm) {
      a.qn_w = F(h, p + "attn.q_norm.weight"); a.qn_b = F(h, p + "attn.q_norm.bias");
      a.kn_w = F(h, p + "attn.k_norm.weight"); a.kn_b = F(h, p + "attn.k_norm.bias");
    }
    if (rope) { a.rope_cos = B<float>(h, "rope_cos"); a.rope_sin = B<float>(h, "rope_sin"); }
    a.M = M; a.H = heads; a.head_stride = M; a.tokens_per_view = tokens_per_view; a.patch_start = patch_start; a.grid_w = d.gw;
    a.q_scale = 0.125f * 1.4426950408889634f; a.dtype = dt;
    st = gemm(c, dt, WM_EPI_QKV, A16, D, W16(h, p + "attn.qkv.weight"), D, nullptr, 0, F(h, p + "attn.qkv.bias"), nullptr, M, 3 * D, D, &ex);
    if (st) return st;
  }
  {
    WmAttnArgs a;
    memset(&a, 0, sizeof(a));
    a.Q = Q16; a.O = O16; a.H = heads; a.q_rows = M; a.q_head_stride = M; a.dtype = dt;
    const bool force_gather = wm_tuning[WM_TUNE_FORCE_GATHER] > 0;
    static const bool overlap_env = [] { const char* e = wm_env("WM_COMM_OVERLAP"); return e && atoi(e) != 0; }();
    a.part_o = B<float>(h, "ATT_PO"); a.part_ml = B<float>(h, "ATT_ML"); a.max_splits = WM_ATTN_MAX_SPLITS;
    a.unit_flags = B<int>(h, "ATT_FLAGS");
    const size_t hint_n = wm_attention_max_blocks((int)d.Mx, d.P < d.Td ? d.P : d.Td, d.heads);
    const int site = c.attn_site++;
    int* const hint0 = B<int>(h, "ATT_HINT") + (size_t)site * 3 * hint_n;
    int* const stat0 = B<int>(h, "ATT_STAT") + (size_t)site * 3;
    a.unit_hint = hint0; a.unit_stat = stat0;
    bool general_only = false;
    if (site * 3 < h->att_stat_n) {
      const int cur = h->att_stat_host[site * 3], delta = cur - h->att_seen[site * 3];
      h->att_seen[site * 3] = cur;
      const long units = (long)((seq_len + 511) / 512) * (M / (seq_len > 0 ? seq_len : 1)) * heads;
      if (delta > 0 && (long)delta * 4 >= units) h->att_general_ttl[site * 3] = WM_ATTN_HINT_TTL;
      if (h->att_general_ttl[site * 3] > 0) { --h->att_general_ttl[site * 3]; general_only = true; }
    }
    const bool sharded = is_global && (d.world > 1 || (force_gather && h->comm.kind != 0));
    const int ntpc = (M + 63) / 64;
    const bool overlap = wm_tuning[WM_TUNE_COMM_OVERLAP] >= 0 ? wm_tuning[WM_TUNE_COMM_OVERLAP] != 0 : overlap_env;
    bool overlap_ok = sharded && overlap && d.world > 1 && ntpc >= 16;
    if (overlap_ok) {
      WmAttnArgs t = a;
      t.force_partial = 1; t.K = K16; t.V = V16; t.seq_len = M; t.kv_head_stride = M; t.kv_chunks = 1;
      overlap_ok = wm_attention_variant(t) >= 0;
      t.kv_chunks = d.world - 1 > 1 ? d.world - 1 : 2; t.kv_rows_per_chunk = M; t.kv_chunk_stride = (long long)(2 * hsz / 2);
      overlap_ok = overlap_ok && wm_attention_variant(t) >= 0;
    }
    if (overlap_ok) {
      if (!h->cstream) {
        LCHK(c, hipStreamCreateWithFlags(&h->cstream, hipStreamNonBlocking));
        LCHK(c, hipEventCreateWithFlags(&h->cfork, hipEventDisableTiming));
        LCHK(c, hipEventCreateWithFlags(&h->cjoin, hipEventDisableTiming));
      }
      char* KVG = B<char>(h, "KVG");
      const int rank = h->comm.rank, world = d.world;
      LCHK(c, hipEventRecord(h->cfork, c.s));
      static const int ncu = [] { hipDeviceProp_t pr; int dv = 0; (void)hipGetDevice(&dv); return hipGetDeviceProperties(&pr, dv) == hipSuccess ? pr.multiProcessorCount : 256; }();
      auto pick = [&](int chunks, int smax) {
        WmAttnArgs g = a;
        g.force_partial = 1; g.seq_len = M; g.kv_head_stride = M;
        if (chunks <= 1) { g.K = K16; g.V = V16; g.kv_chunks = 1; }
        else { g.K = B<char>(h, "KVG"); g.V = g.K; g.kv_chunks = chunks; g.kv_rows_per_chunk = M; g.kv_chunk_stride = (long long)(2 * hsz / 2); }
        int unit_rows = 256, per_cu = 2;
        wm_attention_geometry(g, &unit_rows, &per_cu);
        const int ntiles = (chunks < 1 ? 1 : chunks) * ntpc;
        const long slots = (long)per_cu * ncu, units = (long)((M + unit_rows - 1) / unit_rows) * heads;
        int best = 1; long best_cost = -1;
        for (int S = 1; S <= smax && S * 8 <= ntiles; ++S) {
          const long cost = ((units * S + slots - 1) / slots) * ((ntiles + S - 1) / S) + 6L * S;
          if (best_cost < 0 || cost < best_cost) { best_cost = cost; best = S; }
        }
        return best;
      };
      const int nb = rank, nc = world - 1 - rank;
      const int sa = pick(1, 2);
      const int sb = nb > 0 ? pick(nb, nc > 0 ? 3 : 6) : 0, sc = nc > 0 ? pick(nc, WM_ATTN_MAX_SPLITS - sa - sb) : 0;
      a.force_partial = 1;
      a.K = K16; a.V = V16; a.seq_len = M; a.kv_head_stride = M; a.kv_chunks = 1; a.kv_chunk_stride = 0; a.kv_rows_per_chunk = 0;
      a.kv_splits = sa; a.part_slot0 = 0;
      {
        ProfScope ps(h, 0, c.s);
        LCHK(c, wm_launch_attention(a, c.s));
      }
      LCHK(c, hipStreamWaitEvent(h->cstream, h->cfork, 0));
      st = comm_allgather(h, K16, KVG, 2 * hsz, h->cstream);
      if (st) return st;
      LCHK(c, hipEventRecord(h->cjoin, h->cstream));
      LCHK(c, hipStreamWaitEvent(c.s, h->cjoin, 0));
      ProfScope ps(h, 0, c.s);
      a.seq_len = M; a.kv_head_stride = M; a.kv_chunk_stride = (long long)(2 * hsz / 2); a.kv_rows_per_chunk = M;
      if (nb > 0) {
        a.K = KVG; a.V = KVG + hsz; a.kv_chunks = nb; a.kv_splits = sb; a.part_slot0 = sa; a.unit_hint = hint0 + hint_n; a.unit_stat = stat0 + 1;
        LCHK(c, wm_launch_attention(a, c.s));
      }
      if (nc > 0) {
        char* base = KVG + (size_t)(rank + 1) * 2 * hsz;
        a.K = base; a.V = base + hsz; a.kv_chunks = nc; a.kv_splits = sc; a.part_slot0 = sa + sb; a.unit_hint = hint0 + 2 * hint_n; a.unit_stat = stat0 + 2;
        LCHK(c, wm_launch_attention(a, c.s));
      }
      LCHK(c, wm_launch_attention_combine(a, sa + sb + sc, c.s));
    } else {
      if (sharded) {
        char* KVG = B<char>(h, "KVG");
        st = comm_allgather(h, K16, KVG, 2 * hsz, c.s);
        if (st) return st;
        a.K = KVG; a.V = KVG + hsz; a.seq_len = M; a.kv_head_stride = M; a.kv_chunks = d.world;
        a.kv_chunk_stride = (long long)(2 * hsz / 2); a.kv_rows_per_chunk = M;
      } else {
        a.K = K16; a.V = V16; a.seq_len = seq_len; a.kv_head_stride = M; a.kv_chunks = 1; a.kv_chunk_stride = 0; a.kv_rows_per_chunk = 0;
      }
      if (general_only) { a.unit_flags = nullptr; a.unit_hint = nullptr; a.unit_stat = nullptr; }
      ProfScope ps(h, is_global ? 0 : 1, c.s);
      LCHK(c, wm_launch_attention(a, c.s));
    }
  }
  {
    WmGemmArgs ex;
    memset(&ex, 0, sizeof(ex));
    fuse_args(ex, F(h, p + "norm2.weight"), F(h, p + "norm2.bias"));
    bool fused = false;
    st = gemm(c, dt, WM_EPI_RESID, O16, D, W16(h, p + "attn.proj.weight"), D, X, D, F(h, p + "attn.proj.bias"), F(h, p + "ls1.gamma"), M, D, D, &ex, -1, &fused);
    if (st) return st;
    if (!fused) {
      st = layernorm(c, X, D, A16, D, F(h, p + "norm2.weight"), F(h, p + "norm2.bias"), D, eps, 1, M, 0, 0, 0, 0, 0, dt);
      if (st) return st;
    }
  }
  const int Hd = c.h->cfg.mlp_ratio * D;
  st = gemm(c, dt, WM_EPI_GELU_T16, A16, D, W16(h, p + "mlp.fc1.weight"), D, H16, Hd, F(h, p + "mlp.fc1.bias"), nullptr, M, Hd, D);
  if (st) return st;
  WmGemmArgs ex;
  memset(&ex, 0, sizeof(ex));
  ex.C2 = tap_half; ex.ldc2 = 2 * D;
  bool fused = false;
  if (!next_norm1.empty()) fuse_args(ex, F(h, next_norm1 + "norm1.weight"), F(h, next_norm1 + "norm1.bias"));
  st = gemm(c, dt, WM_EPI_RESID, H16, Hd, W16(h, p + "mlp.fc2.weight"), Hd, X, D, F(h, p + "mlp.fc2.bias"), F(h, p + "ls2.gamma"), M, D, Hd, &ex, -1, &fused);
  if (ln1_ready) *ln1_ready = fused;
  return st;
}

wm_status linear32(Ctx& c, const float* X, int ldx, const std::string& name, float* Y, int ldy, int M, int pre, int post,
                   const float* gamma = nullptr, int accumulate = 0) {
  const Weight* w = W(c.h, name + ".weight");
  if (!w || !w->f32) return fail(c.h, WM_ERR_STATE, "missing fp32 weight " + name);
  const int N = (int)w->shape[0];
  int K = 1;
  for (size_t i = 1; i < w->shape.size(); ++i) K *= (int)w->shape[i];
  LCHK(c, wm_launch_linear_f32(X, w->f32, F(c.h, name + ".bias"), Y, M, N, K, ldx, ldy, pre, post, gamma, accumulate, c.s));
  return WM_OK;
}

wm_status camera_head(Ctx& c, float* out_params) {
  wm_handle* h = c.h;
  const Dims& d = c.d;
  const wm_config& cf = h->cfg;
  const int D2 = 2 * d.D, S = d.nt;
  const std::string ch = "cam_head.";
  float* tok = B<float>(h, "cam_tok");
  wm_status st;
  float* tok_local = d.world > 1 ? B<float>(h, "cam_tok_local") : tok;
  st = layernorm(c, B<float>(h, "tap3"), D2, tok_local, D2, F(h, ch + "token_norm.weight"), F(h, ch + "token_norm.bias"), D2, 1e-5f,
                 d.n, 1, d.P, 0, 1, 0, 1, 0);
  if (st) return st;
  if (d.world > 1) {
    st = comm_allgather(h, tok_local, tok, (size_t)d.n * D2 * 4, c.s);
    if (st) return st;
  }
  float *e = B<float>(h, "cam_e"), *mod = B<float>(h, "cam_mod"), *hh = B<float>(h, "cam_h"), *a = B<float>(h, "cam_a");
  float *qkv = B<float>(h, "cam_qkv"), *o = B<float>(h, "cam_o"), *f = B<float>(h, "cam_f");
  float *pred = B<float>(h, "cam_pred"), *delta = B<float>(h, "cam_delta"), *init = B<float>(h, "cam_init");
  LCHK(c, hipMemsetAsync(pred, 0, (size_t)S * 12 * 4, c.s));
  LCHK(c, hipMemsetAsync(delta, 0, (size_t)S * 12 * 4, c.s));
  for (int step = 0; step < cf.cam_steps; ++step) {
    st = linear32(c, step == 0 ? init : pred, 12, ch + "param_embed", e, D2, S, 0, 0);
    if (st) return st;
    st = linear32(c, e, D2, ch + "adapt_norm_gen.1", mod, 3 * D2, S, 1, 0);
    if (st) return st;
    LCHK(c, wm_launch_adaln(tok, mod, hh, S, D2, 1e-6f, c.s));
    for (int b = 0; b < cf.cam_trunk_depth; ++b) {
      const std::string p = ch + "refine_net." + std::to_string(b) + ".";
      st = layernorm(c, hh, D2, a, D2, F(h, p + "norm1.weight"), F(h, p + "norm1.bias"), D2, 1e-5f, 1, S, 0, 0, 0, 0, 1, 0);
      if (st) return st;
      st = linear32(c, a, D2, p + "attn.qkv", qkv, 3 * D2, S, 0, 0);
      if (st) return st;
      LCHK(c, wm_launch_small_attention(qkv, o, S, cf.cam_heads, D2 / cf.cam_heads, c.s));
      st = linear32(c, o, D2, p + "attn.proj", hh, D2, S, 0, 0, F(h, p + "ls1.gamma"), 1);
      if (st) return st;
      st = layernorm(c, hh, D2, a, D2, F(h, p + "norm2.weight"), F(h, p + "norm2.bias"), D2, 1e-5f, 1, S, 0, 0, 0, 0, 1, 0);
      if (st) return st;
      st = linear32(c, a, D2, p + "mlp.fc1", f, 4 * D2, S, 0, 2);
// ... 329 lines not shown
      memset(&ex, 0, sizeof(ex));
      ex.rows_per_group = (int)npix; ex.accumulate = 1; ex.relu = 1;
      st = gemm(c, c.hdt, WM_EPI_ROWMAP_ADD, col, 192, W16(h, p + "input_merger.0.weight"), 192, fused, F_ / 2,
                F(h, p + "input_merger.0.bias"), nullptr, (int)npix, F_ / 2, 192, &ex);
      if (st) return st;
      float* X = others[0];
      float* gp = others[2];
      st = conv(c, fused, "gs_renderer.gs_head.0", false, nullptr, false, nullptr, X, n, Ho, Wo, 3, 1, 1, false);
      if (st) return st;
      st = conv(c, X, "gs_renderer.gs_head.2", true, nullptr, false, nullptr, gp, n, Ho, Wo, 1, 1, 0, true);
      if (st) return st;
      LCHK(c, wm_launch_gs_splat(gp, img_c, out_attr + voff, B<float>(h, "cam_params") + (size_t)(first_view + v0) * 9,
                                 out->splat_means + voff * 3, out->splat_quats + voff * 4, out->splat_scales + voff * 3,
                                 out->splat_opacities + voff, out->splat_sh + voff * 3, out->splat_weights + voff, n, Ho, Wo, c.s));
    }
  }
  return WM_OK;
}

wm_status forward_impl(wm_handle* h, const float* img, int n, int first_view, int nt, int H, int W_, const float* pose7,
                       const float* depth, const float* ray4, const int32_t* flags, const wm_outputs* out, hipStream_t s) {
  if (!h || !img || !out) return WM_ERR_INVALID;
  if (!h->finalized) return fail(h, WM_ERR_STATE, "weights not finalized");
  const wm_config& cf = h->cfg;
  if (n <= 0 || nt < n || nt % n) return fail(h, WM_ERR_INVALID, "n_total must be a positive multiple of n_local");
  if (H % cf.patch_size || W_ % cf.patch_size) return fail(h, WM_ERR_INVALID, "H and W must be multiples of patch_size");
  if (nt / n > 1 && (h->comm.kind == 0 || h->comm.world != nt / n)) return fail(h, WM_ERR_COMM, "communicator world size mismatch");
  HIPCHK(h, hipSetDevice(h->device));
  Ctx c{h, make_dims(h, n, nt, H, W_), s, cf.backbone_dtype, cf.head_dtype};
  const Dims& d = c.d;
  if (!(h->plan_n == d.n && h->plan_nt == d.nt && h->plan_H == d.H && h->plan_W == d.W))
    return fail(h, WM_ERR_STATE, "no workspace for this shape: call wm_reserve(h, n_local, n_total, H, W) first (and again after loading weights)");
  wm_status st = WM_OK;
  for (int k = 0; k < wm_handle::NKIND; ++k) h->ev_used[k] = 0;
  ProfScope whole(h, 4, s);
  HIPCHK(h, hipMemsetAsync(B<char>(h, "ZERO256"), 0, 256, s));
  const int D = d.D;
  const std::string v = "visual_geometry_transformer.", dn = v + "patch_embed.";
  float* Xd = B<float>(h, "Xd");
  float* Xv = B<float>(h, "Xv");
  void* A16 = B<void>(h, "A16");

  LCHK(c, wm_launch_im2col(img, A16, n, 3, H, W_, cf.patch_size, d.kpad_patch, 1, c.bdt, s));
  {
    WmGemmArgs ex;
    memset(&ex, 0, sizeof(ex));
    ex.rows_per_group = d.hw; ex.out_group = d.Td; ex.out_off = 1 + d.R; ex.add = B<float>(h, "dino_pos") + D;
    st = gemm(c, c.bdt, WM_EPI_ROWMAP_ADD, A16, d.kpad_patch, W16(h, dn + "patch_embed.proj.weight"), d.kpad_patch, Xd, D,
              F(h, dn + "patch_embed.proj.bias"), nullptr, n * d.hw, D, d.kpad_patch, &ex);
    if (st) return st;
  }
  LCHK(c, wm_launch_dino_tokens(nullptr, F(h, dn + "cls_token"), F(h, dn + "register_tokens"), B<float>(h, "dino_pos"), Xd, n, d.hw, d.R, D, s));
  {
    bool ln1 = false;
    for (int i = 0; i < cf.dino_depth; ++i) {
      const std::string nxt = i + 1 < cf.dino_depth ? dn + "blocks." + std::to_string(i + 1) + "." : std::string();
      st = backbone_block(c, dn + "blocks." + std::to_string(i) + ".", Xd, d.Md, d.Td, cf.dino_heads, 1e-6f, false, false, d.Td, 0, false, nullptr, ln1, nxt, &ln1);
      if (st) return st;
    }
  }
  st = layernorm(c, Xd, D, Xv, D, F(h, dn + "norm.weight"), F(h, dn + "norm.bias"), D, 1e-6f, n, d.hw, d.Td, 1 + d.R, d.P, d.psi, 1, 0);
  if (st) return st;

  const float* pose_tok = nullptr; const float* ray_tok = nullptr;
  if (cf.enable_cond) {
    float* pin = B<float>(h, "pr_in"); float* ph = B<float>(h, "pr_h");
    if (flags && flags[0] == 1 && pose7) {
      LCHK(c, hipMemcpy2DAsync(pin, 8 * 4, pose7, 7 * 4, 7 * 4, n, hipMemcpyDeviceToDevice, s));
      st = linear32(c, pin, 8, v + "pose_embed.0", ph, D, n, 0, 1);
      if (st) return st;
      st = linear32(c, ph, D, v + "pose_embed.2", B<float>(h, "pose_tok"), D, n, 0, 0);
      if (st) return st;
      pose_tok = B<float>(h, "pose_tok");
    }
    if (flags && flags[2] == 1 && ray4) {
      st = linear32(c, ray4, 4, v + "ray_embed.0", ph, D, n, 0, 1);
      if (st) return st;
      st = linear32(c, ph, D, v + "ray_embed.2", B<float>(h, "ray_tok"), D, n, 0, 0);
      if (st) return st;
      ray_tok = B<float>(h, "ray_tok");
    }
    if (flags && flags[1] == 1 && depth) {
      LCHK(c, wm_launch_im2col(depth, A16, n, 1, H, W_, cf.patch_size, d.kpad_depth, 0, c.bdt, s));
      void* H16 = B<void>(h, "H16");
      st = gemm(c, c.bdt, WM_EPI_GELU_T16, A16, d.kpad_depth, W16(h, v + "depth_embed.proj.2.fc1.weight"), d.kpad_depth, H16, 4 * D,
                F(h, v + "depth_embed.proj.2.fc1.bias"), nullptr, n * d.hw, 4 * D, d.kpad_depth);
      if (st) return st;
      WmGemmArgs ex;
      memset(&ex, 0, sizeof(ex));
      ex.rows_per_group = d.hw; ex.out_group = d.P; ex.out_off = d.psi; ex.accumulate = 1;
      st = gemm(c, c.bdt, WM_EPI_ROWMAP_ADD, H16, 4 * D, W16(h, v + "depth_embed.proj.2.fc2.weight"), 4 * D, Xv, D,
                F(h, v + "depth_embed.proj.2.fc2.bias"), nullptr, n * d.hw, D, 4 * D, &ex);
      if (st) return st;
    }
  }
  LCHK(c, wm_launch_vgt_special(Xv, F(h, v + "cam_token"), F(h, v + "reg_token"), pose_tok, ray_tok, n, d.P, d.R, D, cf.enable_cond, first_view, s));

  int tap_i = 0;
  bool vgt_ln1 = false;
  for (int i = 0; i < cf.depth; ++i) {
    const bool is_tap = tap_i < 4 && i == cf.intermediate_idxs[tap_i];
    float* tap = is_tap ? B<float>(h, ("tap" + std::to_string(tap_i)).c_str()) : nullptr;
    const std::string gname = v + "global_blocks." + std::to_string(i) + ".";
    const std::string fnext = i + 1 < cf.depth ? v + "frame_blocks." + std::to_string(i + 1) + "." : std::string();
    st = backbone_block(c, v + "frame_blocks." + std::to_string(i) + ".", Xv, d.Mv, d.P, cf.num_heads, 1e-5f, true, true, d.P, d.psi, false, tap,
                        vgt_ln1, gname, &vgt_ln1);
    if (st) return st;
    st = backbone_block(c, gname, Xv, d.Mv, d.Mv, cf.num_heads, 1e-5f, true, true, d.P, d.psi, true, tap ? tap + D : nullptr, vgt_ln1, fnext, &vgt_ln1);
    if (st) return st;
    if (is_tap) {
      if (out->taps[tap_i]) LCHK(c, hipMemcpyAsync(out->taps[tap_i], tap, (size_t)d.Mv * 2 * D * 4, hipMemcpyDeviceToDevice, s));
      ++tap_i;
    }
  }

  if (h->att_stat_host) LCHK(c, hipMemcpyAsync(h->att_stat_host, B<int>(h, "ATT_STAT"), (size_t)h->att_stat_n * 4, hipMemcpyDeviceToHost, s));

  static const bool conc_env = [] { const char* e = wm_env("WM_HEADS_CONCURRENT"); return !e || atoi(e) != 0; }();
  const bool serial = !(wm_tuning[WM_TUNE_HEADS_CONC] >= 0 ? wm_tuning[WM_TUNE_HEADS_CONC] != 0 : conc_env) || h->prof;
  if (!h->hfork) LCHK(c, hipEventCreateWithFlags(&h->hfork, hipEventDisableTiming));
  if (!serial) LCHK(c, hipEventRecord(h->hfork, s));
  bool cam_async = false;
  if (cf.enable_cam && out->camera_params) {
    Ctx cc = c;
    if (!serial) {
      if (!h->camstream) {
        LCHK(c, hipStreamCreateWithFlags(&h->camstream, hipStreamNonBlocking));
        LCHK(c, hipEventCreateWithFlags(&h->camjoin, hipEventDisableTiming));
      }
      cc.s = h->camstream;
      LCHK(c, hipStreamWaitEvent(cc.s, h->hfork, 0));
      cam_async = true;
    }
    st = camera_head(cc, B<float>(h, "cam_params"));
    if (st) return st;
    LCHK(c, hipMemcpyAsync(out->camera_params, B<float>(h, "cam_params"), (size_t)nt * 9 * 4, hipMemcpyDeviceToDevice, cc.s));
    if (out->camera_poses && out->camera_intrs)
      LCHK(c, wm_launch_cam_matrices(B<float>(h, "cam_params"), out->camera_poses, out->camera_intrs, nt, H, W_, cc.s));
    if (cam_async) LCHK(c, hipEventRecord(h->camjoin, cc.s));
  }
  {
    struct HeadJob { const char* p; int F; int od; int act; bool gs; float* attr; float* conf; };
    std::vector<HeadJob> jobs;
    if (cf.enable_depth && out->depth && out->depth_conf) jobs.push_back({"depth_head.", cf.dpt_features, 2, WM_ACT_EXP, false, out->depth, out->depth_conf});
    if (cf.enable_pts && out->pts3d && out->pts3d_conf) jobs.push_back({"pts_head.", cf.dpt_features, 4, WM_ACT_INV_LOG, false, out->pts3d, out->pts3d_conf});
    if (cf.enable_norm && out->normals && out->normals_conf) jobs.push_back({"norm_head.", cf.dpt_features, 4, WM_ACT_NORM, false, out->normals, out->normals_conf});
    if (cf.enable_gs && out->gs_depth && out->gs_depth_conf) {
      if (out->splat_means && !(out->splat_quats && out->splat_scales && out->splat_opacities && out->splat_sh && out->splat_weights))
        return fail(h, WM_ERR_INVALID, "splat outputs must be given together");
      if (out->splat_means && !(cf.enable_cam && out->camera_params)) return fail(h, WM_ERR_INVALID, "splats need the camera head");
      jobs.push_back({"gs_head.", cf.gs_dim, 2, WM_ACT_EXP, true, out->gs_depth, out->gs_depth_conf});
    }
// ... 101 lines not shown
  if (!h || !g || rank < 0 || rank >= g->world) return WM_ERR_INVALID;
  h->comm.kind = 2; h->comm.rank = rank; h->comm.world = g->world; h->comm.grp = g;
  return WM_OK;
}

extern "C" wm_status wm_allgather(wm_handle* h, const void* send, void* recv, size_t bytes_per_rank, void* stream) {
  if (!h || !send || !recv || bytes_per_rank == 0) return WM_ERR_INVALID;
  return comm_allgather(h, send, recv, bytes_per_rank, (hipStream_t)stream);
}

extern "C" wm_status wm_profile_enable(wm_handle* h, int on) {
  if (!h) return WM_ERR_INVALID;
  h->prof = on != 0;
  return WM_OK;
}
extern "C" wm_status wm_profile_read(wm_handle* h, int kind, double* total_ms, int64_t* launches) {
  if (!h || kind < 0 || kind >= wm_handle::NKIND) return WM_ERR_INVALID;
  double tot = 0;
  for (size_t i = 0; i < h->ev_used[kind]; ++i) {
    float ms = 0;
    HIPCHK(h, hipEventSynchronize(h->ev[kind][i].b));
    HIPCHK(h, hipEventElapsedTime(&ms, h->ev[kind][i].a, h->ev[kind][i].b));
    tot += ms;
  }
  if (total_ms) *total_ms = tot;
  if (launches) *launches = (int64_t)h->ev_used[kind];
  return WM_OK;
}

extern "C" wm_status wm_op_gemm(int dtype, int epi, const void* A, const void* Wp, void* C, const float* bias, const float* gamma,
                                int M, int N, int K, void* stream) {
  WmGemmArgs a;
  memset(&a, 0, sizeof(a));
  a.A = A; a.W = Wp; a.C = C; a.bias = bias; a.gamma = gamma; a.M = M; a.N = N; a.K = K; a.lda = K; a.ldw = K; a.ldc = N;
  if (wm_tuning[WM_TUNE_OP_LDPAD] > 0) a.lda = a.ldw = K + wm_tuning[WM_TUNE_OP_LDPAD];
  a.dtype = dtype; a.epi = epi;
  return wm_launch_gemm(a, (hipStream_t)stream) == hipSuccess ? WM_OK : WM_ERR_HIP;
}
extern "C" wm_status wm_op_gemm_resid_ln(int dtype, const void* A, const void* Wp, float* X, const float* bias, const float* gamma, const float* ln_w,
                                         const float* ln_b, float ln_eps, void* ln_out, float* stats, int* sync, int M, int N, int K, int* fused_out,
                                         void* stream) {
  WmGemmArgs a;
  memset(&a, 0, sizeof(a));
  a.A = A; a.W = Wp; a.C = X; a.bias = bias; a.gamma = gamma; a.M = M; a.N = N; a.K = K; a.lda = K; a.ldw = K; a.ldc = N;
  a.dtype = dtype; a.epi = WM_EPI_RESID;
  a.ln_out = ln_out; a.ln_ld = N; a.ln_w = ln_w; a.ln_b = ln_b; a.ln_eps = ln_eps; a.ln_stats = stats; a.ln_sync = sync;
  a.ln_fallback = sync + ((size_t)M / 16 + 2) * 2;
  const bool fuse = wm_gemm_fuses_ln(a);
  if (fused_out) *fused_out = fuse ? 1 : 0;
  if (!fuse) a.ln_out = nullptr;
  if (wm_launch_gemm(a, (hipStream_t)stream) != hipSuccess) return WM_ERR_HIP;
  if (fuse && wm_launch_gemm_ln_fallback(a, (hipStream_t)stream) != hipSuccess) return WM_ERR_HIP;
  return WM_OK;
}
extern "C" wm_status wm_op_gemm_qkv(int dtype, const void* A, const void* Wp, const float* bias, void* q, void* k, void* v,
                                    const float* qn_w, const float* qn_b, const float* kn_w, const float* kn_b, const float* rope_cos,
                                    const float* rope_sin, int M, int H, int K, int tokens_per_view, int patch_start, int grid_w,
                                    float q_scale, void* stream) {
  WmGemmArgs a;
  memset(&a, 0, sizeof(a));
  a.A = A; a.W = Wp; a.bias = bias; a.M = M; a.N = 3 * H * 64; a.K = K; a.lda = K; a.ldw = K; a.dtype = dtype; a.epi = WM_EPI_QKV;
  a.qkv.q = q; a.qkv.k = k; a.qkv.v = v; a.qkv.qn_w = qn_w; a.qkv.qn_b = qn_b; a.qkv.kn_w = kn_w; a.qkv.kn_b = kn_b;
  a.qkv.rope_cos = rope_cos; a.qkv.rope_sin = rope_sin; a.qkv.M = M; a.qkv.H = H; a.qkv.head_stride = M;
  a.qkv.tokens_per_view = tokens_per_view; a.qkv.patch_start = patch_start; a.qkv.grid_w = grid_w; a.qkv.q_scale = q_scale; a.qkv.dtype = dtype;
  return wm_launch_gemm(a, (hipStream_t)stream) == hipSuccess ? WM_OK : WM_ERR_HIP;
}
extern "C" wm_status wm_op_attention(int dtype, const void* Q, const void* K, const void* V, void* O, int H, int q_rows, int seq_len,
                                     int kv_chunks, int kv_rows_per_chunk, void* stream) {
  WmAttnArgs a;
  memset(&a, 0, sizeof(a));
  a.Q = Q; a.K = K; a.V = V; a.O = O; a.H = H; a.q_rows = q_rows; a.seq_len = seq_len; a.q_head_stride = q_rows;
  a.kv_chunks = kv_chunks; a.dtype = dtype;
  if (kv_chunks > 1) {
    a.kv_head_stride = kv_rows_per_chunk; a.kv_rows_per_chunk = kv_rows_per_chunk; a.kv_chunk_stride = (long long)H * kv_rows_per_chunk * 64;
  } else {
    a.kv_head_stride = q_rows;
  }
  return wm_launch_attention(a, (hipStream_t)stream) == hipSuccess ? WM_OK : WM_ERR_HIP;
}
extern "C" wm_status wm_op_attention_split(int dtype, const void* Q, const void* K, const void* V, void* O, int H, int q_rows, int seq_len,
                                           int kv_chunks, int kv_rows_per_chunk, int kv_splits, float* part_o, float* part_ml, void* stream) {
  WmAttnArgs a;
  memset(&a, 0, sizeof(a));
  a.Q = Q; a.K = K; a.V = V; a.O = O; a.H = H; a.q_rows = q_rows; a.seq_len = seq_len; a.q_head_stride = q_rows;
  a.kv_chunks = kv_chunks; a.dtype = dtype; a.kv_splits = kv_splits; a.max_splits = WM_ATTN_MAX_SPLITS; a.part_o = part_o; a.part_ml = part_ml;
  if (kv_chunks > 1) {
    a.kv_head_stride = kv_rows_per_chunk; a.kv_rows_per_chunk = kv_rows_per_chunk; a.kv_chunk_stride = (long long)H * kv_rows_per_chunk * 64;
  } else {
    a.kv_head_stride = q_rows;
  }
  return wm_launch_attention(a, (hipStream_t)stream) == hipSuccess ? WM_OK : WM_ERR_HIP;
}
extern "C" wm_status wm_op_attention_ex(int dtype, const void* Q, const void* K, const void* V, void* O, int H, int q_rows, int seq_len,
                                        int kv_chunks, int kv_rows_per_chunk, int kv_splits, float* part_o, float* part_ml, int* unit_flags,
                                        void* stream) {
  WmAttnArgs a;
  memset(&a, 0, sizeof(a));
  a.Q = Q; a.K = K; a.V = V; a.O = O; a.H = H; a.q_rows = q_rows; a.seq_len = seq_len; a.q_head_stride = q_rows;
  a.kv_chunks = kv_chunks; a.dtype = dtype; a.kv_splits = kv_splits; a.max_splits = WM_ATTN_MAX_SPLITS; a.part_o = part_o; a.part_ml = part_ml;
  a.unit_flags = unit_flags;
  if (unit_flags) {
    const size_t nb = wm_attention_max_blocks(q_rows, seq_len, H);
    a.unit_hint = unit_flags + nb;
    a.unit_stat = unit_flags + 2 * nb;
    const bool policy = wm_tuning[WM_TUNE_ATTN_OP_POLICY] == 1;
    static int* mirror = nullptr;
// ... 406 lines not shown
```

include/wm_hip.h:

```cpp
#ifndef WM_HIP_H
#define WM_HIP_H
#include <stddef.h>
#include <stdint.h>

#ifdef __cplusplus
extern "C" {
#endif

typedef struct wm_handle wm_handle;

typedef enum { WM_OK = 0, WM_ERR_INVALID = 1, WM_ERR_HIP = 2, WM_ERR_STATE = 3, WM_ERR_COMM = 4 } wm_status;
typedef enum { WM_DT_BF16 = 0, WM_DT_F16 = 1 } wm_dtype;

typedef struct {
  int32_t img_size, patch_size, embed_dim, gs_dim;
  int32_t enable_cond, enable_cam, enable_pts, enable_depth, enable_norm, enable_gs;
  int32_t depth, num_heads, mlp_ratio, num_register_tokens;
  int32_t intermediate_idxs[4];
  float rope_freq;
  int32_t dino_depth, dino_heads;
  int32_t cam_trunk_depth, cam_heads, cam_steps;
  int32_t dpt_features;
  int32_t dpt_out_channels[4];
  int32_t backbone_dtype;
// ... 9 lines not shown
  float* pts3d;
  float* pts3d_conf;
  float* normals;
  float* normals_conf;
  float* gs_depth;
  float* gs_depth_conf;
  float* splat_means;
  float* splat_quats;
  float* splat_scales;
  float* splat_opacities;
  float* splat_sh;
  float* splat_weights;
  float* taps[4];
} wm_outputs;

wm_status wm_create(const wm_config* cfg, int device, wm_handle** out);
void wm_destroy(wm_handle* h);
const char* wm_last_error(const wm_handle* h);
wm_status wm_set_weight(wm_handle* h, const char* name, const float* host, const int64_t* shape, int ndim);
wm_status wm_finalize_weights(wm_handle* h, int* missing);
const char* wm_missing_name(const wm_handle* h, int i);
wm_status wm_share_weights(wm_handle* dst, const wm_handle* src);
void wm_host_resample_pos(const float* in, int gs, int D, int gh, int gw, float* out);

size_t wm_workspace_bytes(const wm_handle* h, int n_local, int n_total, int H, int W);
wm_status wm_reserve(wm_handle* h, int n_local, int n_total, int H, int W);
wm_status wm_set_workspace(wm_handle* h, void* device_ptr, size_t bytes);
wm_status wm_forward(wm_handle* h, const float* img, int N, int H, int W, const float* pose7, const float* depth,
                     const float* ray4, const int32_t cond_flags[3], const wm_outputs* out, void* stream);
wm_status wm_forward_sharded(wm_handle* h, const float* img, int n_local, int first_view, int n_total, int H, int W,
                             const float* pose7, const float* depth, const float* ray4, const int32_t cond_flags[3],
                             const wm_outputs* out, void* stream);

#define WM_RCCL_ID_BYTES 128
wm_status wm_rccl_unique_id(uint8_t id[WM_RCCL_ID_BYTES]);
wm_status wm_comm_init_rccl(wm_handle* h, const uint8_t id[WM_RCCL_ID_BYTES], int rank, int world);
typedef struct wm_local_group wm_local_group;
wm_local_group* wm_local_group_create(int world);
void wm_local_group_destroy(wm_local_group* g);
wm_status wm_comm_init_local(wm_handle* h, wm_local_group* g, int rank);
wm_status wm_allgather(wm_handle* h, const void* send, void* recv, size_t bytes_per_rank, void* stream);

wm_status wm_profile_enable(wm_handle* h, int on);
wm_status wm_profile_read(wm_handle* h, int kind, double* total_ms, int64_t* launches);

wm_status wm_op_gemm(int dtype, int epi, const void* A, const void* W, void* C, const float* bias, const float* gamma,
                     int M, int N, int K, void* stream);
wm_status wm_op_gemm_qkv(int dtype, const void* A, const void* W, const float* bias, void* q, void* k, void* v, const float* qn_w,
                         const float* qn_b, const float* kn_w, const float* kn_b, const float* rope_cos, const float* rope_sin, int M,
                         int H, int K, int tokens_per_view, int patch_start, int grid_w, float q_scale, void* stream);
wm_status wm_op_gemm_resid_ln(int dtype, const void* A, const void* W, float* X, const float* bias, const float* gamma, const float* ln_w,
                              const float* ln_b, float ln_eps, void* ln_out, float* stats, int* sync, int M, int N, int K, int* fused_out,
                              void* stream);
wm_status wm_op_attention(int dtype, const void* Q, const void* K, const void* V, void* O, int H, int q_rows, int seq_len,
                          int kv_chunks, int kv_rows_per_chunk, void* stream);
wm_status wm_op_attention_split(int dtype, const void* Q, const void* K, const void* V, void* O, int H, int q_rows, int seq_len,
                                int kv_chunks, int kv_rows_per_chunk, int kv_splits, float* part_o, float* part_ml, void* stream);
wm_status wm_op_attention_ex(int dtype, const void* Q, const void* K, const void* V, void* O, int H, int q_rows, int seq_len,
                             int kv_chunks, int kv_rows_per_chunk, int kv_splits, float* part_o, float* part_ml, int* unit_flags,
                             void* stream);
size_t wm_op_attention_flag_count(int q_rows, int seq_len, int H);
wm_status wm_op_gs_splat(const float* gp, const float* img, const float* depth, const float* cam, float* means, float* quats,
                         float* scales, float* opac, float* sh, float* wts, int N, int H, int W, void* stream);
wm_status wm_op_layernorm(const float* x, void* y, const float* w, const float* b, int rows, int D, float eps, int out_f32,
                          int dtype, void* stream);
wm_status wm_op_qkv_post(int dtype, const float* qkv, void* q, void* k, void* v, const float* qn_w, const float* qn_b,
                         const float* kn_w, const float* kn_b, const float* rope_cos, const float* rope_sin, int M, int H,
                         int tokens_per_view, int patch_start, int grid_w, float q_scale, void* stream);
wm_status wm_op_conv(int dtype, const float* x, const void* w16, const float* bias, const float* resid, const float* resid2,
                     float* y, int N, int Hi, int Wi, int Cin, int Cout, int ksize, int stride, int pad, int relu_in,
                     int resid_relu, void* stream);
wm_status wm_op_conv3x3_up(int dtype, const float* x, const void* w16, const float* bias, float* y, int N, int Hs, int Ws, int Hi, int Wi,
                           int Cin, int Cout, const float* addx, const float* addy, void* stream);
wm_status wm_op_bilinear(const float* in, float* out, int N, int Hi, int Wi, int Ho, int Wo, int C, void* stream);
wm_status wm_op_linear_f32(const float* X, const float* W, const float* b, float* Y, int M, int N, int K, int ldx, int pre_act,
                           int post_act, void* stream);

wm_status wm_op_im2col(int dtype, const float* img, void* out, int N, int C, int H, int W, int ps, int Kpad, int normalize, void* stream);
wm_status wm_op_im2col7(int dtype, const float* img, void* out, int N, int H, int W, int Kpad, void* stream);
wm_status wm_op_dino_tokens(const float* patch, const float* cls, const float* reg, const float* pos, float* X, int N, int hw, int R, int D,
                            void* stream);
wm_status wm_op_vgt_special(float* X, const float* cam_tok, const float* reg_tok, const float* pose_tok, const float* ray_tok, int N, int P,
                            int R, int D, int cond, int first_view_global, void* stream);
wm_status wm_op_gemm_rowmap(int dtype, const void* A, const void* W, void* C, const float* bias, const float* add, int M, int N, int K,
                            int ldc, int rows_per_group, int out_group, int out_off, int accumulate, int out16, int relu, void* stream);
wm_status wm_op_gemm_convt(int dtype, const void* A, const void* W, float* C, const float* bias, int M, int N, int K, int ct_k, int ct_cout,
                           int ct_gh, int ct_gw, void* stream);
wm_status wm_op_layernorm_rows(const float* x, void* y, const float* w, const float* b, int D, int ld_in, int ld_out, float eps, int groups,
                               int rows_per_group, int in_group, int in_off, int out_group, int out_off, int out_f32, int dtype, void* stream);
wm_status wm_op_bilinear_add(const float* in, float* out, int N, int Hi, int Wi, int Ho, int Wo, int C, const float* addx, const float* addy,
                             void* stream);
wm_status wm_op_bilinear16(int dtype, const float* in, void* out16, int N, int Hi, int Wi, int Ho, int Wo, int C, const float* addx,
                           const float* addy, void* stream);
wm_status wm_op_copy2d(const float* src, float* dst, int rows, int cols, int ld_src, int ld_dst, void* stream);
wm_status wm_op_small_attention(const float* qkv, float* out, int S, int heads, int hd, void* stream);
wm_status wm_op_adaln(const float* tok, const float* mod, float* h, int S, int D, float eps, void* stream);
wm_status wm_op_cam_update(float* pred, const float* delta, float* out, int S, int first, void* stream);
wm_status wm_op_cam_matrices(const float* params, float* poses, float* intrs, int S, int H, int W, void* stream);
wm_status wm_op_linear_f32_ex(const float* X, const float* W, const float* b, float* Y, int M, int N, int K, int ldx, int ldy, int pre_act,
                              int post_act, const float* gamma, int accumulate, void* stream);
wm_status wm_depth_to_world(const float* depth, const float* extrinsic, const float* intrinsic, float* world, float* cam,
                            unsigned char* mask, int B, int H, int W, float eps, void* stream);

wm_status wm_preprocess_image_size(int H, int W, int mode, int output_size, int* out_h, int* out_w);
size_t wm_preprocess_image_workspace_bytes(int H, int W, int mode, int output_size);
wm_status wm_preprocess_image(const unsigned char* rgb, int H, int W, int mode, int output_size, float* out, void* workspace,
// ... 54 lines not shown
```

Before: 160.6 views/s.

## Defer LayerNorm into consumer GEMM epilogues via folded weights and row stats

Adds a deferred-LayerNorm path. The LN scale is folded into the following GEMM's bf16 weights, with per-column sum and bias vectors precomputed. The residual GEMM epilogue writes a bf16 copy of the unnormalized residual plus per-row partial mean/variance stats. The consumer GEMMs (QKV, fc1) then apply mean and rstd in their epilogue, so the standalone layernorm launch and its extra pass over activations are removed. The path is gated behind a new tuning flag, and applying normalization after the matmul on unnormalized bf16 inputs may change numerical accuracy.

```diff
diff --git a/hunyuanworld-mirror_amd/_lib.py b/hunyuanworld-mirror_amd/_lib.py
--- a/hunyuanworld-mirror_amd/_lib.py
+++ b/hunyuanworld-mirror_amd/_lib.py
@@ -49,6 +49,7 @@
     "wm_op_im2col", "wm_op_im2col7", "wm_op_dino_tokens", "wm_op_vgt_special", "wm_op_gemm_rowmap", "wm_op_gemm_convt", "wm_op_layernorm_rows",
     "wm_op_bilinear_add", "wm_op_bilinear16", "wm_op_copy2d", "wm_op_small_attention", "wm_op_adaln", "wm_op_cam_update", "wm_op_cam_matrices",
     "wm_op_linear_f32_ex",
+    "wm_op_fold_ln", "wm_op_gemm_resid_defer", "wm_op_gemm_deferred_ln", "wm_op_gemm_qkv_deferred_ln", "wm_layernorm_launch_count",
 ]
 
 _lib = None
@@ -96,6 +97,12 @@
     L.wm_op_gemm.argtypes = [i32, i32, vp, vp, vp, vp, vp, i32, i32, i32, vp]
     L.wm_op_gemm_resid_ln.argtypes = [i32, vp, vp, vp, vp, vp, vp, vp, f32, vp, vp, vp, i32, i32, i32, C.POINTER(i32), vp]
     L.wm_op_gemm_qkv.argtypes = [i32, vp, vp, vp, vp, vp, vp, vp, vp, vp, vp, vp, vp, i32, i32, i32, i32, i32, i32, f32, vp]
+    L.wm_op_fold_ln.argtypes = [vp, vp, vp, vp, vp, vp, vp, i32, i32, vp]
+    L.wm_op_gemm_resid_defer.argtypes = [i32, vp, vp, vp, vp, vp, vp, vp, vp, i32, i32, i32, C.POINTER(i32), vp]
+    L.wm_op_gemm_deferred_ln.argtypes = [i32, i32, vp, vp, vp, vp, vp, vp, f32, i32, i32, i32, vp]
+    L.wm_op_gemm_qkv_deferred_ln.argtypes = [i32, vp, vp, vp, vp, vp, f32, vp, vp, vp, vp, vp, vp, vp, vp, vp, i32, i32, i32, i32, i32, i32, f32, vp]
+    L.wm_layernorm_launch_count.argtypes = [i32]
+    L.wm_layernorm_launch_count.restype = C.c_longlong
     L.wm_op_attention.argtypes = [i32, vp, vp, vp, vp, i32, i32, i32, i32, i32, vp]
     L.wm_op_attention_split.argtypes = [i32, vp, vp, vp, vp, i32, i32, i32, i32, i32, i32, vp, vp, vp]
     L.wm_op_attention_ex.argtypes = [i32, vp, vp, vp, vp, i32, i32, i32, i32, i32, i32, vp, vp, vp, vp]
diff --git a/hunyuanworld-mirror_amd/csrc/gemm.hip b/hunyuanworld-mirror_amd/csrc/gemm.hip
--- a/hunyuanworld-mirror_amd/csrc/gemm.hip
+++ b/hunyuanworld-mirror_amd/csrc/gemm.hip
@@ -4,7 +4,7 @@
 #include <cstdlib>
 #include <type_traits>
 
-int wm_tuning[WM_TUNE_COUNT] = {-1, -1, -1, -1, -1, -1, -1, -1, -1, -1, -1, -1, -1, -1, -1, -1, -1, -1, -1, -1, -1, -1, -1, -1, -1, -1, -1, -1, -1};
+int wm_tuning[WM_TUNE_COUNT] = {-1, -1, -1, -1, -1, -1, -1, -1, -1, -1, -1, -1, -1, -1, -1, -1, -1, -1, -1, -1, -1, -1, -1, -1, -1, -1, -1, -1, -1, -1};
 
 namespace {
 
@@ -343,9 +343,18 @@
 }
 
 
+__device__ __forceinline__ float ln_lin(float a, float mean, float rstd, float s, float c) {
+  return __builtin_fmaf(rstd, __fsub_rn(a, __fmul_rn(mean, s)), c);
+}
+__device__ __forceinline__ float4 ln_lin4(const f32x4& a, float mean, float rstd, const float4& s, const float4& c) {
+  return make_float4(ln_lin(a[0], mean, rstd, s.x, c.x), ln_lin(a[1], mean, rstd, s.y, c.y), ln_lin(a[2], mean, rstd, s.z, c.z), ln_lin(a[3], mean, rstd, s.w, c.w));
+}
+
 template <int T, int EPI, int SM, int SN>
-__device__ __forceinline__ void epilogue16(const WmGemmArgs& p, f32x4 (&acc)[SM][SN], int rowb, int colb, int lane, int mlim) {
+__device__ __forceinline__ void epilogue16(const WmGemmArgs& p, f32x4 (&acc)[SM][SN], int rowb, int colb, int lane, int mlim,
+                                           const float* lnm = nullptr, const float* lnr = nullptr) {
   const int l15 = lane & 15, lq = lane >> 4;
+  const bool def = lnm != nullptr && p.ln_s != nullptr;
   if constexpr (EPI == WM_EPI_QKV) {
     static_assert(EPI != WM_EPI_QKV || SN == 4, "QKV epilogue needs 64 columns per wave");
     const WmQkvArgs& q = p.qkv;
@@ -358,10 +367,16 @@
     const bool do_norm = which < 2 && nw != nullptr, do_rope = which < 2 && q.rope_cos != nullptr;
     u16* dst = (u16*)(which == 0 ? q.q : which == 1 ? q.k : q.v);
     const float sc = which == 0 ? q.q_scale : 1.0f;
-    float4 bs4[4], w4[4], b4[4];
+    float4 bs4[4], w4[4], b4[4], s4[4];
 #pragma unroll
     for (int j = 0; j < 4; ++j) {
-      bs4[j] = p.bias ? *(const float4*)(p.bias + col0 + 16 * j + 4 * lq) : make_float4(0, 0, 0, 0);
+      if (def) {
+        bs4[j] = *(const float4*)(p.ln_c + col0 + 16 * j + 4 * lq);
+        s4[j] = *(const float4*)(p.ln_s + col0 + 16 * j + 4 * lq);
+      } else {
+        bs4[j] = p.bias ? *(const float4*)(p.bias + col0 + 16 * j + 4 * lq) : make_float4(0, 0, 0, 0);
+        s4[j] = make_float4(0, 0, 0, 0);
+      }
       w4[j] = do_norm ? *(const float4*)(nw + 16 * j + 4 * lq) : make_float4(1, 1, 1, 1);
       b4[j] = do_norm ? *(const float4*)(nb + 16 * j + 4 * lq) : make_float4(0, 0, 0, 0);
     }
@@ -389,7 +404,12 @@
       float v[4][4];
 #pragma unroll
       for (int j = 0; j < 4; ++j) {
-        v[j][0] = acc[i][j][0] + bs4[j].x; v[j][1] = acc[i][j][1] + bs4[j].y; v[j][2] = acc[i][j][2] + bs4[j].z; v[j][3] = acc[i][j][3] + bs4[j].w;
+        if (def) {
+          const float4 x = ln_lin4(acc[i][j], lnm[i], lnr[i], s4[j], bs4[j]);
+          v[j][0] = x.x; v[j][1] = x.y; v[j][2] = x.z; v[j][3] = x.w;
+        } else {
+          v[j][0] = acc[i][j][0] + bs4[j].x; v[j][1] = acc[i][j][1] + bs4[j].y; v[j][2] = acc[i][j][2] + bs4[j].z; v[j][3] = acc[i][j][3] + bs4[j].w;
+        }
       }
       if (do_norm) {
         float sm = 0.f;
@@ -444,11 +464,15 @@
     }
     return;
   } else {
-    float4 bs4[SN], gm4[SN];
+    float4 bs4[SN], gm4[SN], s4[SN];
 #pragma unroll
     for (int j = 0; j < SN; ++j) {
       const int col = colb + j * 16 + 4 * lq;
       bs4[j] = (p.bias && col < p.N) ? *(const float4*)(p.bias + col) : make_float4(0, 0, 0, 0);
+      s4[j] = make_float4(0, 0, 0, 0);
+      if constexpr (EPI == WM_EPI_F32 || EPI == WM_EPI_GELU_T16) {
+        if (def && col < p.N) { bs4[j] = *(const float4*)(p.ln_c + col); s4[j] = *(const float4*)(p.ln_s + col); }
+      }
       if constexpr (EPI == WM_EPI_RESID) gm4[j] = col < p.N ? *(const float4*)(p.gamma + col) : make_float4(0, 0, 0, 0);
     }
     if constexpr ((EPI == WM_EPI_T16 || EPI == WM_EPI_GELU_T16) && SN % 2 == 0) {
@@ -464,6 +488,7 @@
             for (int h = 0; h < 2; ++h) {
               const int j = 2 * jp + h;
               float4 x = make_float4(acc[i][j][0] + bs4[j].x, acc[i][j][1] + bs4[j].y, acc[i][j][2] + bs4[j].z, acc[i][j][3] + bs4[j].w);
+              if (def) x = ln_lin4(acc[i][j], lnm[i], lnr[i], s4[j], bs4[j]);
               if constexpr (EPI == WM_EPI_GELU_T16) x = gelu_erf4(x);
               u[h].x = (uint32_t)f2t<T>(x.x) | ((uint32_t)f2t<T>(x.y) << 16);
               u[h].y = (uint32_t)f2t<T>(x.z) | ((uint32_t)f2t<T>(x.w) << 16);
@@ -578,6 +603,9 @@
         if (col >= p.N) continue;
         const float4 bs = bs4[j];
         float4 x = make_float4(acc[i][j][0] + bs.x, acc[i][j][1] + bs.y, acc[i][j][2] + bs.z, acc[i][j][3] + bs.w);
+        if constexpr (EPI == WM_EPI_F32 || EPI == WM_EPI_GELU_T16) {
+          if (def) x = ln_lin4(acc[i][j], lnm[i], lnr[i], s4[j], bs);
+        }
         const size_t o = (size_t)row * p.ldc + col;
         if constexpr (EPI == WM_EPI_F32) {
           *(float4*)((float*)p.C + o) = x;
@@ -926,6 +954,84 @@
     if (d == 3) {
       __hip_atomic_store((wm_gi32*)(p.ln_sync + band * 2), 0, WM_RLX_AGENT);
       __hip_atomic_store((wm_gi32*)(p.ln_sync + band * 2 + 1), 0, WM_RLX_AGENT);
+    }
+  }
+}
+
+template <int T, int SM>
+__device__ __forceinline__ void epilogue_resid_defer(const WmGemmArgs& p, f32x4 (&acc)[SM][4], char* smem, int lane, int wc, int nt, int rowb, int colb,
+                                                     int rl0, int mlim) {
+  const int l15 = lane & 15, lq = lane >> 4;
+  float4 bs4[4], gm4[4];
+#pragma unroll
+  for (int j = 0; j < 4; ++j) {
+    const int col = colb + j * 16 + 4 * lq;
+    bs4[j] = p.bias ? *(const float4*)(p.bias + col) : make_float4(0, 0, 0, 0);
+    gm4[j] = *(const float4*)(p.gamma + col);
+  }
+  float4 old[2][4];
+  auto load_old = [&](int i, float4 (&o)[4]) {
+    const int row = rowb + i * 16 + l15;
+#pragma unroll
+    for (int j = 0; j < 4; ++j) o[j] = row < mlim ? *(const float4*)((const float*)p.C + (size_t)row * p.ldc + colb + j * 16 + 4 * lq) : make_float4(0, 0, 0, 0);
+  };
+  load_old(0, old[0]);
+#pragma unroll
+  for (int i = 0; i < SM; ++i) {
+    if (rowb + i * 16 >= mlim) break;
+    if (i + 1 < SM) load_old(i + 1, old[(i + 1) & 1]);
+    const int row = rowb + i * 16 + l15;
+    uint2 u[4];
+#pragma unroll
+    for (int j = 0; j < 4; ++j) {
+      const float4 o = old[i & 1][j], gm = gm4[j], bs = bs4[j];
+      acc[i][j] = f32x4{o.x + gm.x * (acc[i][j][0] + bs.x), o.y + gm.y * (acc[i][j][1] + bs.y), o.z + gm.z * (acc[i][j][2] + bs.z), o.w + gm.w * (acc[i][j][3] + bs.w)};
+      u[j].x = (uint32_t)f2t<T>(acc[i][j][0]) | ((uint32_t)f2t<T>(acc[i][j][1]) << 16);
+      u[j].y = (uint32_t)f2t<T>(acc[i][j][2]) | ((uint32_t)f2t<T>(acc[i][j][3]) << 16);
+      if (row < mlim) {
+        const float4 nv = make_float4(acc[i][j][0], acc[i][j][1], acc[i][j][2], acc[i][j][3]);
+        *(float4*)((float*)p.C + (size_t)row * p.ldc + colb + j * 16 + 4 * lq) = nv;
+        if (p.C2) *(float4*)(p.C2 + (size_t)row * p.ldc2 + colb + j * 16 + 4 * lq) = nv;
+      }
+    }
+#pragma unroll
+    for (int jp = 0; jp < 2; ++jp) {
+      swap16(u[2 * jp].x, u[2 * jp + 1].x);
+      swap16(u[2 * jp].y, u[2 * jp + 1].y);
+      const int col = colb + (2 * jp + (lq & 1)) * 16 + 4 * (lq & 2);
+      if (row < mlim) *(uint4*)((u16*)p.a16_out + (size_t)row * p.a16_ld + col) = make_uint4(u[2 * jp].x, u[2 * jp].y, u[2 * jp + 1].x, u[2 * jp + 1].y);
+    }
+  }
+  float2* lst = (float2*)smem;
+  __syncthreads();
+#pragma unroll
+  for (int i = 0; i < SM; ++i) {
+    if (rowb + i * 16 >= mlim) break;
+    float s1 = 0.f;
+#pragma unroll
+    for (int j = 0; j < 4; ++j) s1 += (acc[i][j][0] + acc[i][j][1]) + (acc[i][j][2] + acc[i][j][3]);
+    s1 += __shfl_xor(s1, 16);
+    const float mw = __fmul_rn(xhalf_sum(s1), 1.0f / 64.0f);
+    float s2 = 0.f;
+#pragma unroll
+    for (int j = 0; j < 4; ++j)
+#pragma unroll
+      for (int e = 0; e < 4; ++e) { const float d = acc[i][j][e] - mw; s2 = __builtin_fmaf(d, d, s2); }
+    s2 += __shfl_xor(s2, 16);
+    s2 = xhalf_sum(s2);
+    if (lq == 0) lst[(rl0 + i * 16 + l15) * 4 + wc] = make_float2(mw, s2);
+  }
+  __syncthreads();
+  if (wc == 0 && lq == 0) {
+#pragma unroll
+    for (int i = 0; i < SM; ++i) {
+      if (rowb + i * 16 >= mlim) break;
+      const float4 a0 = *(const float4*)(lst + (rl0 + i * 16 + l15) * 4), a1 = *(const float4*)(lst + (rl0 + i * 16 + l15) * 4 + 2);
+      const float m[4] = {a0.x, a0.z, a1.x, a1.z}, q[4] = {a0.y, a0.w, a1.y, a1.w};
+      float tmean, tm2;
+      ln_combine4(m, q, 64.0f, tmean, tm2);
+      const int row = rowb + i * 16 + l15;
+      if (row < mlim) *(float2*)(p.ln_stats + ((size_t)row * 4 + nt) * 2) = make_float2(tmean, tm2);
     }
   }
 }
@@ -1081,6 +1187,21 @@
     for (int j = 0; j < SN; ++j) acc[i][j] = f32x4{0.f, 0.f, 0.f, 0.f};
   s16x8 a[QI][2], b0[2][2], b1[2][2];
 
+  constexpr bool DEFC = (EPI == WM_EPI_F32 || EPI == WM_EPI_GELU_T16 || EPI == WM_EPI_QKV) && DBG == 0;
+  float lnm[SM], lnr[SM];
+  float4 lnst[DEFC ? SM : 1][2];
+  if constexpr (DEFC) {
+    if (p.ln_s) {
+      const int rowb0 = m0 + (wr ? 16 * S0 : 0);
+#pragma unroll
+      for (int i = 0; i < SM; ++i) {
+        int row = rowb0 + i * 16 + l15;
+        row = row < p.M ? row : p.M - 1;
+        const float4* sp = (const float4*)(p.ln_stats + (size_t)row * 8);
+        lnst[i][0] = sp[0]; lnst[i][1] = sp[1];
+      }
+    }
+  }
   const int nk = CONV && p.tc_k > 0 ? (int)(tc_word >> 16) * cv_nch : p.K / 64;
   dma(0, 0, 8);
   if (nk > 1) dma(1, 0, 8);
@@ -1090,6 +1211,19 @@
     if (nk > 1) WM_W2(12, 9); else WM_W2(4, 3);
   }
   __builtin_amdgcn_s_barrier();
+  if constexpr (DEFC) {
+#pragma unroll
+    for (int i = 0; i < SM; ++i) { lnm[i] = 0.f; lnr[i] = 1.f; }
+    if (p.ln_s) {
+#pragma unroll
+      for (int i = 0; i < SM; ++i) {
+        const float m[4] = {lnst[i][0].x, lnst[i][0].z, lnst[i][1].x, lnst[i][1].z}, q[4] = {lnst[i][0].y, lnst[i][0].w, lnst[i][1].y, lnst[i][1].w};
+        float M2;
+        ln_combine4(m, q, 256.0f, lnm[i], M2);
+        lnr[i] = 1.0f / sqrtf(__fadd_rn(__fmul_rn(M2, 1.0f / 1024.0f), p.ln_eps));
+      }
+    }
+  }
   if (VER == 2 && wr == 1) __builtin_amdgcn_s_barrier();
 
 #ifdef WM_GEMM_STAMPS
@@ -1300,8 +1434,13 @@
         epilogue_resid_ln<T, SM>(p, acc, smem, tid, lane, wr, wc, band, nt, rowb, n0 + wc * 64, wr ? 16 * S0 : 0, rend < p.M ? rend : p.M);
         return;
       }
-    }
-    epilogue16<T, EPI, SM, SN>(p, acc, rowb, n0 + wc * 64, lane, rend < p.M ? rend : p.M);
+      if (p.a16_out) {
+        epilogue_resid_defer<T, SM>(p, acc, smem, lane, wc, nt, rowb, n0 + wc * 64, wr ? 16 * S0 : 0, rend < p.M ? rend : p.M);
+        return;
+      }
+    }
+    if constexpr (DEFC) epilogue16<T, EPI, SM, SN>(p, acc, rowb, n0 + wc * 64, lane, rend < p.M ? rend : p.M, lnm, lnr);
+    else epilogue16<T, EPI, SM, SN>(p, acc, rowb, n0 + wc * 64, lane, rend < p.M ? rend : p.M);
   }
 #ifdef WM_GEMM_STAMPS
   asm volatile("s_waitcnt vmcnt(0)" ::: "memory");
@@ -1498,6 +1637,54 @@
   return bands * 4 <= wm_ncu();
 }
 
+bool wm_gemm_defers_ln(const WmGemmArgs& a) {
+  if (!a.a16_out || a.epi != WM_EPI_RESID || a.dtype != WM_T_BF16 || a.N != 1024 || !a.ln_stats || !a.gamma || (a.a16_ld & 7) || (a.ldc & 3)) return false;
+  if (((uintptr_t)a.a16_out & 15) || ((uintptr_t)a.ln_stats & 15)) return false;
+  if (wm_tuning[WM_TUNE_LN_DEFER] != 1 || wm_tuning[WM_TUNE_LN_FUSE] == 1) return false;
+  int cfg, sched_b; bool pp2;
+  plan_gemm(a, cfg, sched_b, pp2);
+  return pp2 && cfg == 5;
+}
+
+bool wm_gemm_takes_deferred_ln(const WmGemmArgs& a) {
+  if (a.epi != WM_EPI_F32 && a.epi != WM_EPI_GELU_T16 && a.epi != WM_EPI_QKV) return false;
+  if (a.dtype != WM_T_BF16 || a.K != 1024 || (a.N & 3) || !a.ln_stats || !a.ln_s || !a.ln_c || ((uintptr_t)a.ln_stats & 15)) return false;
+  int cfg, sched_b; bool pp2;
+  plan_gemm(a, cfg, sched_b, pp2);
+  return pp2 && (cfg == 4 || cfg == 5);
+}
+
+namespace {
+__global__ __launch_bounds__(256) void fold_ln_kernel(const float* __restrict__ W, const float* __restrict__ lw, const float* __restrict__ lb,
+                                                      const float* __restrict__ bias, u16* __restrict__ wg, float* __restrict__ so, float* __restrict__ co, int K) {
+  __shared__ float red[2][4];
+  const int j = blockIdx.x, tid = threadIdx.x, lane = tid & 63, wave = tid >> 6;
+  float s = 0.f, c = 0.f;
+  for (int k = tid; k < K; k += 256) {
+    const float w = W[(size_t)j * K + k];
+    const u16 r = f2t<WM_T_BF16>(__fmul_rn(lw[k], w));
+    wg[(size_t)j * K + k] = r;
+    s += __builtin_bit_cast(float, (uint32_t)r << 16);
+    c = __builtin_fmaf(lb[k], w, c);
+  }
+#pragma unroll
+  for (int o = 32; o > 0; o >>= 1) { s += __shfl_xor(s, o); c += __shfl_xor(c, o); }
+  if (lane == 0) { red[0][wave] = s; red[1][wave] = c; }
+  __syncthreads();
+  if (tid == 0) {
+    so[j] = (red[0][0] + red[0][1]) + (red[0][2] + red[0][3]);
+    co[j] = (bias ? bias[j] : 0.f) + ((red[1][0] + red[1][1]) + (red[1][2] + red[1][3]));
+  }
+}
+}
+
+hipError_t wm_launch_fold_ln(const float* W32, const float* ln_w, const float* ln_b, const float* bias, void* wg16, float* s, float* c, int N, int K,
+                             hipStream_t st) {
+  if (N <= 0 || K <= 0 || !W32 || !ln_w || !ln_b || !wg16 || !s || !c) return hipErrorInvalidValue;
+  hipLaunchKernelGGL(fold_ln_kernel, dim3(N), dim3(256), 0, st, W32, ln_w, ln_b, bias, (u16*)wg16, s, c, K);
+  return hipGetLastError();
+}
+
 hipError_t wm_launch_gemm_ln_fallback(const WmGemmArgs& a, hipStream_t s) {
   if (!wm_gemm_fuses_ln(a)) return hipSuccess;
   int cfg, sched_b; bool pp2;
@@ -1549,6 +1736,7 @@
   bool is_pp2;
   plan_gemm(a, cfg, sched_b, is_pp2);
   const bool fuse_ln = wm_gemm_fuses_ln(a);
+  if (a.ln_s && !wm_gemm_takes_deferred_ln(a)) return hipErrorInvalidValue;
   const int gb = wm_tuning[WM_TUNE_GEMM_GROUP] >= 0 ? wm_tuning[WM_TUNE_GEMM_GROUP] : 6;
   if (a.epi == WM_EPI_QKV) {
     if (a.qkv.tokens_per_view <= 0 || a.qkv.grid_w <= 0 || a.M >= (1 << 20) || a.qkv.tokens_per_view >= (1 << 16)) return hipErrorInvalidValue;
@@ -1564,6 +1752,7 @@
   c.sched_bands = sched_b; c.sched_units = (a.M + 15) / 16;
   c.pf_c = a.epi == WM_EPI_RESID && wm_tuning[WM_TUNE_RESID_PREFETCH] == 1 ? 1 : 0;
   if (!fuse_ln) c.ln_out = nullptr;
+  if (fuse_ln || !wm_gemm_defers_ln(a)) c.a16_out = nullptr;
   return c.dtype == WM_T_BF16 ? launch_T<WM_T_BF16>(c, cfg, s) : launch_T<WM_T_F16>(c, cfg, s);
 }
 
diff --git a/hunyuanworld-mirror_amd/csrc/wm_kernels.h b/hunyuanworld-mirror_amd/csrc/wm_kernels.h
--- a/hunyuanworld-mirror_amd/csrc/wm_kernels.h
+++ b/hunyuanworld-mirror_amd/csrc/wm_kernels.h
@@ -58,8 +58,14 @@
   float* ln_stats;
   int* ln_sync;
   int* ln_fallback;
+  void* a16_out; int a16_ld;
+  const float* ln_s; const float* ln_c;
 };
 hipError_t wm_launch_gemm(const WmGemmArgs& a, hipStream_t s);
+bool wm_gemm_defers_ln(const WmGemmArgs& a);
+bool wm_gemm_takes_deferred_ln(const WmGemmArgs& a);
+hipError_t wm_launch_fold_ln(const float* W32, const float* ln_w, const float* ln_b, const float* bias, void* wg16, float* s, float* c, int N, int K,
+                             hipStream_t st);
 bool wm_gemm_fuses_ln(const WmGemmArgs& a);
 hipError_t wm_launch_gemm_ln_fallback(const WmGemmArgs& a, hipStream_t s);
 
@@ -201,5 +207,5 @@
                               const float* weights, int N, float voxel, float* o_means, float* o_quats, float* o_scales, float* o_opac,
                               float* o_sh, int* K_out, void* workspace, size_t ws_bytes, hipStream_t s);
 
-enum { WM_TUNE_GEMM_CFG = 0, WM_TUNE_GEMM_PP, WM_TUNE_GEMM_MFMA16, WM_TUNE_ATTN_QB, WM_TUNE_OP_LDPAD, WM_TUNE_ATTN_SPLITS, WM_TUNE_CONV_FUSE_UP, WM_TUNE_CONV_NARROW, WM_TUNE_CONV_BN, WM_TUNE_CONV_RS, WM_TUNE_LIN_MFMA, WM_TUNE_CONV_TPX, WM_TUNE_ATTN_TAIL, WM_TUNE_GEMM_GROUP, WM_TUNE_COMM_OVERLAP, WM_TUNE_HEADS_CONC, WM_TUNE_RCU_MID16, WM_TUNE_GEMM_SCHED, WM_TUNE_FORCE_GATHER, WM_TUNE_ATTN_OP_POLICY, WM_TUNE_COMM_P2P, WM_TUNE_LN_RPW, WM_TUNE_LN_FUSE, WM_TUNE_HEADS_MAIN, WM_TUNE_CONV_GEMM, WM_TUNE_RESID_PREFETCH, WM_TUNE_UP1_GATHER, WM_TUNE_TCONV, WM_TUNE_UP1_COMP, WM_TUNE_COUNT };
+enum { WM_TUNE_GEMM_CFG = 0, WM_TUNE_GEMM_PP, WM_TUNE_GEMM_MFMA16, WM_TUNE_ATTN_QB, WM_TUNE_OP_LDPAD, WM_TUNE_ATTN_SPLITS, WM_TUNE_CONV_FUSE_UP, WM_TUNE_CONV_NARROW, WM_TUNE_CONV_BN, WM_TUNE_CONV_RS, WM_TUNE_LIN_MFMA, WM_TUNE_CONV_TPX, WM_TUNE_ATTN_TAIL, WM_TUNE_GEMM_GROUP, WM_TUNE_COMM_OVERLAP, WM_TUNE_HEADS_CONC, WM_TUNE_RCU_MID16, WM_TUNE_GEMM_SCHED, WM_TUNE_FORCE_GATHER, WM_TUNE_ATTN_OP_POLICY, WM_TUNE_COMM_P2P, WM_TUNE_LN_RPW, WM_TUNE_LN_FUSE, WM_TUNE_HEADS_MAIN, WM_TUNE_CONV_GEMM, WM_TUNE_RESID_PREFETCH, WM_TUNE_UP1_GATHER, WM_TUNE_TCONV, WM_TUNE_UP1_COMP, WM_TUNE_LN_DEFER, WM_TUNE_COUNT };
 extern int wm_tuning[WM_TUNE_COUNT];
diff --git a/hunyuanworld-mirror_amd/csrc/wm_model.cpp b/hunyuanworld-mirror_amd/csrc/wm_model.cpp
--- a/hunyuanworld-mirror_amd/csrc/wm_model.cpp
+++ b/hunyuanworld-mirror_amd/csrc/wm_model.cpp
@@ -8,6 +8,7 @@
 #include <cstdlib>
 #include <cstring>
 #include <map>
+#include <memory>
 #include <string>
 #include <unordered_map>
 #include <vector>
@@ -42,7 +43,18 @@
   std::vector<float> host;
   bool set = false;
   bool owned = true;
+  void* wg16 = nullptr;
+  float* ln_sc = nullptr;
+  bool fold_owned = false;
+  std::shared_ptr<const std::vector<float>> host32;
 };
+static void drop_fold(Weight& w) {
+  if (w.fold_owned) {
+    if (w.wg16) (void)hipFree(w.wg16);
+    if (w.ln_sc) (void)hipFree(w.ln_sc);
+  }
+  w.wg16 = nullptr; w.ln_sc = nullptr; w.fold_owned = false;
+}
 
 struct TconvPack {
   void* w16 = nullptr;
@@ -102,6 +114,7 @@
   int plan_n = -1, plan_nt = -1, plan_H = -1, plan_W = -1;
   std::map<std::string, TconvPack> tconv;
   bool tconv_valid = false;
+  bool fold_valid = false;
   std::map<std::string, Up1Comp> up1comp;
   std::vector<std::string> missing;
   std::map<std::string, void*> buf;
@@ -445,8 +458,61 @@
     }
 }
 
+static bool fold_enabled(const wm_config& c) { return c.backbone_dtype == WM_DT_BF16 && c.embed_dim == 1024; }
+static std::string fold_target(const std::string& n) {
+  if (!starts_with(n, "visual_geometry_transformer.")) return std::string();
+  static const char* const suf[8] = {"norm1.weight", "norm1.bias", "attn.qkv.weight", "attn.qkv.bias", "norm2.weight", "norm2.bias", "mlp.fc1.weight", "mlp.fc1.bias"};
+  for (int i = 0; i < 8; ++i)
+    if (ends_with(n, suf[i]) && n.size() > strlen(suf[i]) && n[n.size() - strlen(suf[i]) - 1] == '.' && (n.find(".blocks.") != std::string::npos || n.find("_blocks.") != std::string::npos))
+      return n.substr(0, n.size() - strlen(suf[i])) + (i < 4 ? "attn.qkv.weight" : "mlp.fc1.weight");
+  return std::string();
+}
+static wm_status build_folds(wm_handle* h) {
+  if (h->fold_valid) return WM_OK;
+  if (!fold_enabled(h->cfg)) { h->fold_valid = true; return WM_OK; }
+  const wm_config& c = h->cfg;
+  const std::string v = "visual_geometry_transformer.";
+  std::vector<std::string> blocks;
+  for (int i = 0; i < c.dino_depth; ++i) blocks.push_back(v + "patch_embed.blocks." + std::to_string(i) + ".");
+  for (int i = 0; i < c.depth; ++i) { blocks.push_back(v + "frame_blocks." + std::to_string(i) + "."); blocks.push_back(v + "global_blocks." + std::to_string(i) + "."); }
+  float* tmp = nullptr;
+  size_t tmp_n = 0;
+  wm_status st = WM_OK;
+  for (const std::string& b : blocks) {
+    for (int which = 0; which < 2 && st == WM_OK; ++which) {
+      auto it = h->w.find(b + (which ? "mlp.fc1.weight" : "attn.qkv.weight"));
+      if (it == h->w.end() || it->second.wg16 || !it->second.host32 || it->second.shape.size() != 2 || it->second.shape[1] != 1024) continue;
+      Weight& lw = it->second;
+      const float* nw = F(h, b + (which ? "norm2.weight" : "norm1.weight"));
+      const float* nb = F(h, b + (which ? "norm2.bias" : "norm1.bias"));
+      const float* bias = F(h, b + (which ? "mlp.fc1.bias" : "attn.qkv.bias"));
+      if (!nw || !nb || !bias) continue;
+      const int N = (int)lw.shape[0], K = 1024;
+      const size_t numel = (size_t)N * K;
+      if (lw.host32->size() != numel) continue;
+      if (numel > tmp_n) {
+        if (tmp) (void)hipFree(tmp);
+        tmp = nullptr; tmp_n = 0;
+        if (hipMalloc((void**)&tmp, numel * 4) != hipSuccess) { st = fail(h, WM_ERR_HIP, "hipMalloc failed (LayerNorm fold)"); break; }
+        tmp_n = numel;
+      }
+      bool ok = hipMemcpy(tmp, lw.host32->data(), numel * 4, hipMemcpyHostToDevice) == hipSuccess;
+      ok = ok && hipMalloc(&lw.wg16, numel * 2) == hipSuccess;
+      lw.fold_owned = true;
+      ok = ok && hipMalloc((void**)&lw.ln_sc, (size_t)2 * N * 4) == hipSuccess;
+      ok = ok && wm_launch_fold_ln(tmp, nw, nb, bias, lw.wg16, lw.ln_sc, lw.ln_sc + N, N, K, nullptr) == hipSuccess;
+      ok = ok && hipDeviceSynchronize() == hipSuccess;
+      if (!ok) { drop_fold(lw); st = fail(h, WM_ERR_HIP, "building the folded LayerNorm weights failed for " + it->first); }
+    }
+    if (st != WM_OK) break;
+  }
+  if (tmp) (void)hipFree(tmp);
+  if (st == WM_OK) h->fold_valid = true;
+  return st;
+}
+
 extern "C" int wm_set_tuning(const char* key, int value) {
-  static const char* keys[WM_TUNE_COUNT] = {"gemm_cfg", "gemm_pp", "gemm_mfma16", "attn_qb", "op_ldpad", "attn_splits", "conv_fuse_up", "conv_narrow", "conv_bn", "conv_rs", "lin_mfma", "conv_tpx", "attn_tail", "gemm_group", "comm_overlap", "heads_concurrent", "rcu_mid16", "gemm_sched", "force_gather", "attn_op_policy", "comm_p2p", "ln_rpw", "ln_fuse", "heads_main", "conv_gemm", "resid_prefetch", "up1_gather", "tconv", "up1_comp"};
+  static const char* keys[WM_TUNE_COUNT] = {"gemm_cfg", "gemm_pp", "gemm_mfma16", "attn_qb", "op_ldpad", "attn_splits", "conv_fuse_up", "conv_narrow", "conv_bn", "conv_rs", "lin_mfma", "conv_tpx", "attn_tail", "gemm_group", "comm_overlap", "heads_concurrent", "rcu_mid16", "gemm_sched", "force_gather", "attn_op_policy", "comm_p2p", "ln_rpw", "ln_fuse", "heads_main", "conv_gemm", "resid_prefetch", "up1_gather", "tconv", "up1_comp", "ln_defer"};
   for (int i = 0; i < WM_TUNE_COUNT; ++i)
     if (key && strcmp(key, keys[i]) == 0) { wm_tuning[i] = value; return 0; }
   return -1;
@@ -475,6 +541,7 @@
   for (auto& kv : h->tconv) free_tconv(kv.second);
   for (auto& kv : h->up1comp) free_up1comp(kv.second);
   for (auto& kv : h->w) {
+    drop_fold(kv.second);
     if (!kv.second.owned) continue;
     if (kv.second.f32) (void)hipFree(kv.second.f32);
     if (kv.second.w16) (void)hipFree(kv.second.w16);
@@ -515,11 +582,20 @@
   Weight& w = h->w[n];
   h->plan_n = -1;
   h->tconv_valid = false;
+  {
+    const std::string lin = fold_target(n);
+    if (!lin.empty()) {
+      auto fi = h->w.find(lin);
+      if (fi != h->w.end()) drop_fold(fi->second);
+      h->fold_valid = false;
+    }
+  }
   if (w.owned) {
     if (w.f32) (void)hipFree(w.f32);
     if (w.w16) (void)hipFree(w.w16);
   }
   w.f32 = nullptr; w.w16 = nullptr; w.owned = true; w.tap_major = false;
+  w.host32.reset();
   w.shape = sh;
   w.set = true;
   const WKind k = classify(n, ndim);
@@ -537,6 +613,7 @@
       ends_with(n, ".scratch.refinenet1.out_conv.weight") || ends_with(n, ".scratch.output_conv1.weight"))
     w.host.assign(host, host + numel);
   const int dt = k == WK_LIN16_BACKBONE ? h->cfg.backbone_dtype : h->cfg.head_dtype;
+  if (fold_enabled(h->cfg) && fold_target(n) == n) w.host32 = std::make_shared<const std::vector<float>>(host, host + numel);
   std::vector<uint16_t> r;
   if (k == WK_LIN16_BACKBONE || k == WK_LIN16_HEAD) {
     const int N = (int)sh[0];
@@ -603,7 +680,7 @@
   }
   if (missing) *missing = (int)h->missing.size();
   h->finalized = true;
-  return WM_OK;
+  return build_folds(h);
 }
 
 extern "C" wm_status wm_share_weights(wm_handle* dst, const wm_handle* src) {
@@ -612,18 +689,20 @@
   if (memcmp(&dst->cfg, &src->cfg, sizeof(wm_config)) != 0 || dst->device != src->device)
     return fail(dst, WM_ERR_INVALID, "wm_share_weights: configuration or device differs");
   for (auto& kv : dst->w) {
+    drop_fold(kv.second);
     if (!kv.second.owned) continue;
     if (kv.second.f32) (void)hipFree(kv.second.f32);
     if (kv.second.w16) (void)hipFree(kv.second.w16);
   }
   dst->w = src->w;
-  for (auto& kv : dst->w) kv.second.owned = false;
+  for (auto& kv : dst->w) { kv.second.owned = false; kv.second.fold_owned = false; }
+  dst->fold_valid = false;
   dst->spec = src->spec;
   dst->missing = src->missing;
   dst->finalized = true;
   dst->plan_n = -1;
   dst->tconv_valid = false;
-  return WM_OK;
+  return build_folds(dst);
 }
 
 extern "C" const char* wm_missing_name(const wm_handle* h, int i) {
@@ -723,6 +802,10 @@
       HIPCHK(h, hipMemcpy(h->buf["gs_posx"], tx.data(), tx.size() * 4, hipMemcpyHostToDevice));
       HIPCHK(h, hipMemcpy(h->buf["gs_posy"], ty.data(), ty.size() * 4, hipMemcpyHostToDevice));
     }
+  }
+  {
+    const wm_status fst = build_folds(h);
+    if (fst != WM_OK) return fst;
   }
   if (!h->tconv_valid) {
     for (auto& kv : h->tconv) free_tconv(kv.second);
@@ -844,6 +927,8 @@
   return WM_OK;
 }
 
+long long g_ln_launches = 0;
+
 wm_status layernorm(Ctx& c, const float* x, int ld_in, void* y, int ld_out, const float* w, const float* b, int D, float eps,
                     int groups, int rpg, int in_group, int in_off, int out_group, int out_off, int out_f32, int dt) {
   WmLnArgs a;
@@ -854,9 +939,10 @@
   return WM_OK;
 }
 
+enum { LN1_NONE = 0, LN1_FUSED = 1, LN1_DEFERRED = 2 };
 wm_status backbone_block(Ctx& c, const std::string& p, float* X, int M, int seq_len, int heads, float eps, bool qk_norm,
                          bool rope, int tokens_per_view, int patch_start, bool is_global, float* tap_half = nullptr,
-                         bool ln1_done = false, const std::string& next_norm1 = std::string(), bool* ln1_ready = nullptr) {
+                         int ln1_done = LN1_NONE, const std::string& next_norm1 = std::string(), int* ln1_ready = nullptr) {
   wm_handle* h = c.h;
   const Dims& d = c.d;
   const int D = d.D, dt = c.bdt;
@@ -867,8 +953,23 @@
   void* O16 = B<void>(h, "O16");
   void* H16 = B<void>(h, "H16");
   wm_status st;
-  if (ln1_ready) *ln1_ready = false;
+  if (ln1_ready) *ln1_ready = LN1_NONE;
+  auto defer_consumer = [&](WmGemmArgs& ex, const Weight* lw, float ceps) {
+    ex.ln_stats = B<float>(h, "LN_STATS"); ex.ln_s = lw->ln_sc; ex.ln_c = lw->ln_sc + lw->shape[0]; ex.ln_eps = ceps;
+  };
+  auto can_defer = [&](const std::string& lin_name, int epi, int Kp) -> const Weight* {
+    const Weight* lw = W(h, lin_name);
+    if (!lw || !lw->wg16 || !lw->ln_sc || dt != WM_DT_BF16 || D != 1024) return nullptr;
+    WmGemmArgs pa, ca;
+    memset(&pa, 0, sizeof(pa)); memset(&ca, 0, sizeof(ca));
+    pa.epi = WM_EPI_RESID; pa.dtype = dt; pa.M = M; pa.N = D; pa.K = Kp; pa.lda = Kp; pa.ldw = Kp; pa.ldc = D; pa.C = X; pa.gamma = F(h, p + "ls1.gamma");
+    pa.a16_out = A16; pa.a16_ld = D; pa.ln_stats = B<float>(h, "LN_STATS");
+    ca.epi = epi; ca.dtype = dt; ca.M = M; ca.N = (int)lw->shape[0]; ca.K = D; ca.lda = D; ca.ldw = D; ca.ldc = ca.N;
+    defer_consumer(ca, lw, eps);
+    return wm_gemm_defers_ln(pa) && wm_gemm_takes_deferred_ln(ca) ? lw : nullptr;
+  };
   if (!ln1_done) {
+    ++g_ln_launches;
     st = layernorm(c, X, D, A16, D, F(h, p + "norm1.weight"), F(h, p + "norm1.bias"), D, eps, 1, M, 0, 0, 0, 0, 0, dt);
     if (st) return st;
   }
@@ -890,7 +991,14 @@
     if (rope) { a.rope_cos = B<float>(h, "rope_cos"); a.rope_sin = B<float>(h, "rope_sin"); }
     a.M = M; a.H = heads; a.head_stride = M; a.tokens_per_view = tokens_per_view; a.patch_start = patch_start; a.grid_w = d.gw;
     a.q_scale = 0.125f * 1.4426950408889634f; a.dtype = dt;
-    st = gemm(c, dt, WM_EPI_QKV, A16, D, W16(h, p + "attn.qkv.weight"), D, nullptr, 0, F(h, p + "attn.qkv.bias"), nullptr, M, 3 * D, D, &ex);
+    const Weight* qw = W(h, p + "attn.qkv.weight");
+    if (ln1_done == LN1_DEFERRED) {
+      if (!qw || !qw->wg16) return fail(h, WM_ERR_STATE, "deferred LayerNorm without folded weights: " + p + "attn.qkv.weight");
+      defer_consumer(ex, qw, eps);
+      st = gemm(c, dt, WM_EPI_QKV, A16, D, qw->wg16, D, nullptr, 0, nullptr, nullptr, M, 3 * D, D, &ex);
+    } else {
+      st = gemm(c, dt, WM_EPI_QKV, A16, D, W16(h, p + "attn.qkv.weight"), D, nullptr, 0, F(h, p + "attn.qkv.bias"), nullptr, M, 3 * D, D, &ex);
+    }
     if (st) return st;
   }
   {
@@ -993,28 +1101,44 @@
       LCHK(c, wm_launch_attention(a, c.s));
     }
   }
+  const Weight* fc1_def = nullptr;
   {
     WmGemmArgs ex;
     memset(&ex, 0, sizeof(ex));
     fuse_args(ex, F(h, p + "norm2.weight"), F(h, p + "norm2.bias"));
+    fc1_def = can_defer(p + "mlp.fc1.weight", WM_EPI_GELU_T16, D);
+    if (fc1_def) { ex.a16_out = A16; ex.a16_ld = D; }
     bool fused = false;
     st = gemm(c, dt, WM_EPI_RESID, O16, D, W16(h, p + "attn.proj.weight"), D, X, D, F(h, p + "attn.proj.bias"), F(h, p + "ls1.gamma"), M, D, D, &ex, -1, &fused);
     if (st) return st;
-    if (!fused) {
+    if (!fused && !fc1_def) {
+      ++g_ln_launches;
       st = layernorm(c, X, D, A16, D, F(h, p + "norm2.weight"), F(h, p + "norm2.bias"), D, eps, 1, M, 0, 0, 0, 0, 0, dt);
       if (st) return st;
     }
   }
   const int Hd = c.h->cfg.mlp_ratio * D;
-  st = gemm(c, dt, WM_EPI_GELU_T16, A16, D, W16(h, p + "mlp.fc1.weight"), D, H16, Hd, F(h, p + "mlp.fc1.bias"), nullptr, M, Hd, D);
+  if (fc1_def) {
+    WmGemmArgs ex;
+    memset(&ex, 0, sizeof(ex));
+    defer_consumer(ex, fc1_def, eps);
+    st = gemm(c, dt, WM_EPI_GELU_T16, A16, D, fc1_def->wg16, D, H16, Hd, nullptr, nullptr, M, Hd, D, &ex);
+  } else {
+    st = gemm(c, dt, WM_EPI_GELU_T16, A16, D, W16(h, p + "mlp.fc1.weight"), D, H16, Hd, F(h, p + "mlp.fc1.bias"), nullptr, M, Hd, D);
+  }
   if (st) return st;
   WmGemmArgs ex;
   memset(&ex, 0, sizeof(ex));
   ex.C2 = tap_half; ex.ldc2 = 2 * D;
   bool fused = false;
-  if (!next_norm1.empty()) fuse_args(ex, F(h, next_norm1 + "norm1.weight"), F(h, next_norm1 + "norm1.bias"));
+  bool defer_next = false;
+  if (!next_norm1.empty()) {
+    fuse_args(ex, F(h, next_norm1 + "norm1.weight"), F(h, next_norm1 + "norm1.bias"));
+    defer_next = ln1_ready != nullptr && can_defer(next_norm1 + "attn.qkv.weight", WM_EPI_QKV, Hd) != nullptr;
+    if (defer_next) { ex.a16_out = A16; ex.a16_ld = D; }
+  }
   st = gemm(c, dt, WM_EPI_RESID, H16, Hd, W16(h, p + "mlp.fc2.weight"), Hd, X, D, F(h, p + "mlp.fc2.bias"), F(h, p + "ls2.gamma"), M, D, Hd, &ex, -1, &fused);
-  if (ln1_ready) *ln1_ready = fused;
+  if (ln1_ready) *ln1_ready = fused ? LN1_FUSED : defer_next ? LN1_DEFERRED : LN1_NONE;
   return st;
 }
 
@@ -1450,7 +1574,7 @@
   }
   LCHK(c, wm_launch_dino_tokens(nullptr, F(h, dn + "cls_token"), F(h, dn + "register_tokens"), B<float>(h, "dino_pos"), Xd, n, d.hw, d.R, D, s));
   {
-    bool ln1 = false;
+    int ln1 = LN1_NONE;
     for (int i = 0; i < cf.dino_depth; ++i) {
       const std::string nxt = i + 1 < cf.dino_depth ? dn + "blocks." + std::to_string(i + 1) + "." : std::string();
       st = backbone_block(c, dn + "blocks." + std::to_string(i) + ".", Xd, d.Md, d.Td, cf.dino_heads, 1e-6f, false, false, d.Td, 0, false, nullptr, ln1, nxt, &ln1);
@@ -1495,7 +1619,7 @@
   LCHK(c, wm_launch_vgt_special(Xv, F(h, v + "cam_token"), F(h, v + "reg_token"), pose_tok, ray_tok, n, d.P, d.R, D, cf.enable_cond, first_view, s));
 
   int tap_i = 0;
-  bool vgt_ln1 = false;
+  int vgt_ln1 = LN1_NONE;
   for (int i = 0; i < cf.depth; ++i) {
     const bool is_tap = tap_i < 4 && i == cf.intermediate_idxs[tap_i];
     float* tap = is_tap ? B<float>(h, ("tap" + std::to_string(tap_i)).c_str()) : nullptr;
@@ -1703,6 +1827,48 @@
   if (wm_launch_gemm(a, (hipStream_t)stream) != hipSuccess) return WM_ERR_HIP;
   if (fuse && wm_launch_gemm_ln_fallback(a, (hipStream_t)stream) != hipSuccess) return WM_ERR_HIP;
   return WM_OK;
+}
+extern "C" long long wm_layernorm_launch_count(int reset) {
+  const long long v = g_ln_launches;
+  if (reset) g_ln_launches = 0;
+  return v;
+}
+extern "C" wm_status wm_op_gemm_resid_defer(int dtype, const void* A, const void* Wp, float* X, const float* bias, const float* gamma, float* c2,
+                                            void* a16_out, float* stats, int M, int N, int K, int* deferred_out, void* stream) {
+  WmGemmArgs a;
+  memset(&a, 0, sizeof(a));
+  a.A = A; a.W = Wp; a.C = X; a.bias = bias; a.gamma = gamma; a.M = M; a.N = N; a.K = K; a.lda = K; a.ldw = K; a.ldc = N;
+  a.dtype = dtype; a.epi = WM_EPI_RESID; a.C2 = c2; a.ldc2 = 2 * N;
+  a.a16_out = a16_out; a.a16_ld = N; a.ln_stats = stats;
+  if (deferred_out) *deferred_out = wm_gemm_defers_ln(a) ? 1 : 0;
+  return wm_launch_gemm(a, (hipStream_t)stream) == hipSuccess ? WM_OK : WM_ERR_HIP;
+}
+extern "C" wm_status wm_op_gemm_deferred_ln(int dtype, int epi, const void* A, const void* Wg, void* C, const float* stats, const float* ln_s,
+                                            const float* ln_c, float ln_eps, int M, int N, int K, void* stream) {
+  WmGemmArgs a;
+  memset(&a, 0, sizeof(a));
+  a.A = A; a.W = Wg; a.C = C; a.M = M; a.N = N; a.K = K; a.lda = K; a.ldw = K; a.ldc = N; a.dtype = dtype; a.epi = epi;
+  a.ln_stats = const_cast<float*>(stats); a.ln_s = ln_s; a.ln_c = ln_c; a.ln_eps = ln_eps;
+  if (!ln_s || !wm_gemm_takes_deferred_ln(a)) return WM_ERR_INVALID;
+  return wm_launch_gemm(a, (hipStream_t)stream) == hipSuccess ? WM_OK : WM_ERR_HIP;
+}
+extern "C" wm_status wm_op_gemm_qkv_deferred_ln(int dtype, const void* A, const void* Wg, const float* stats, const float* ln_s, const float* ln_c,
+                                                float ln_eps, void* q, void* k, void* v, const float* qn_w, const float* qn_b, const float* kn_w,
+                                                const float* kn_b, const float* rope_cos, const float* rope_sin, int M, int H, int K,
+                                                int tokens_per_view, int patch_start, int grid_w, float q_scale, void* stream) {
+  WmGemmArgs a;
+  memset(&a, 0, sizeof(a));
+  a.A = A; a.W = Wg; a.M = M; a.N = 3 * H * 64; a.K = K; a.lda = K; a.ldw = K; a.dtype = dtype; a.epi = WM_EPI_QKV;
+  a.qkv.q = q; a.qkv.k = k; a.qkv.v = v; a.qkv.qn_w = qn_w; a.qkv.qn_b = qn_b; a.qkv.kn_w = kn_w; a.qkv.kn_b = kn_b;
+  a.qkv.rope_cos = rope_cos; a.qkv.rope_sin = rope_sin; a.qkv.M = M; a.qkv.H = H; a.qkv.head_stride = M;
+  a.qkv.tokens_per_view = tokens_per_view; a.qkv.patch_start = patch_start; a.qkv.grid_w = grid_w; a.qkv.q_scale = q_scale; a.qkv.dtype = dtype;
+  a.ln_stats = const_cast<float*>(stats); a.ln_s = ln_s; a.ln_c = ln_c; a.ln_eps = ln_eps;
+  if (!ln_s || !wm_gemm_takes_deferred_ln(a)) return WM_ERR_INVALID;
+  return wm_launch_gemm(a, (hipStream_t)stream) == hipSuccess ? WM_OK : WM_ERR_HIP;
+}
+extern "C" wm_status wm_op_fold_ln(const float* W32, const float* ln_w, const float* ln_b, const float* bias, void* wg16, float* s, float* c, int N,
+                                   int K, void* stream) {
+  return wm_launch_fold_ln(W32, ln_w, ln_b, bias, wg16, s, c, N, K, (hipStream_t)stream) == hipSuccess ? WM_OK : WM_ERR_HIP;
 }
 extern "C" wm_status wm_op_gemm_qkv(int dtype, const void* A, const void* Wp, const float* bias, void* q, void* k, void* v,
                                     const float* qn_w, const float* qn_b, const float* kn_w, const float* kn_b, const float* rope_cos,
diff --git a/include/wm_hip.h b/include/wm_hip.h
--- a/include/wm_hip.h
+++ b/include/wm_hip.h
@@ -85,6 +85,17 @@
 wm_status wm_op_gemm_resid_ln(int dtype, const void* A, const void* W, float* X, const float* bias, const float* gamma, const float* ln_w,
                               const float* ln_b, float ln_eps, void* ln_out, float* stats, int* sync, int M, int N, int K, int* fused_out,
                               void* stream);
+wm_status wm_op_fold_ln(const float* W32, const float* ln_w, const float* ln_b, const float* bias, void* wg16, float* s, float* c, int N, int K,
+                        void* stream);
+wm_status wm_op_gemm_resid_defer(int dtype, const void* A, const void* W, float* X, const float* bias, const float* gamma, float* c2,
+                                 void* a16_out, float* stats, int M, int N, int K, int* deferred_out, void* stream);
+wm_status wm_op_gemm_deferred_ln(int dtype, int epi, const void* A, const void* Wg, void* C, const float* stats, const float* ln_s,
+                                 const float* ln_c, float ln_eps, int M, int N, int K, void* stream);
+wm_status wm_op_gemm_qkv_deferred_ln(int dtype, const void* A, const void* Wg, const float* stats, const float* ln_s, const float* ln_c,
+                                     float ln_eps, void* q, void* k, void* v, const float* qn_w, const float* qn_b, const float* kn_w,
+                                     const float* kn_b, const float* rope_cos, const float* rope_sin, int M, int H, int K,
+                                     int tokens_per_view, int patch_start, int grid_w, float q_scale, void* stream);
+long long wm_layernorm_launch_count(int reset);
 wm_status wm_op_attention(int dtype, const void* Q, const void* K, const void* V, void* O, int H, int q_rows, int seq_len,
                           int kv_chunks, int kv_rows_per_chunk, void* stream);
 wm_status wm_op_attention_split(int dtype, const void* Q, const void* K, const void* V, void* O, int H, int q_rows, int seq_len,
```

Result: slower. 158.7 views/s (-1.1%).
